# gonewest818/raytrace-clj

Measured on NVIDIA B200. Metric: samples_per_sec, higher is better.
Workload: dtype f32

## Files before the change

### raytrace_clj_b200/csrc/rt_api.cu

```cuda
#include "../../include/raytrace_b200.h"

#include <cuda_runtime.h>
#include <dlfcn.h>
#include <math_constants.h>
#include <nccl.h>

#include <algorithm>
#include <cmath>
#include <cstdio>
#include <cstdlib>
#include <cstring>
#include <atomic>
#include <mutex>
#include <thread>
#include <string>
#include <vector>

#include "rt_bvh_build.cuh"
#include "rt_kernels.cuh"

using namespace rt;

namespace {

constexpr int kR = 4;
constexpr int kBlock = 256;
constexpr int kMinBlocks = 1;
constexpr int kTileCap = 4096;

thread_local std::string g_create_error;

struct DeviceBuffers {
    int dev = 0;
    cudaStream_t stream = nullptr;
    cudaEvent_t ev0 = nullptr, ev1 = nullptr, ev_done = nullptr;
    void* scene_blob = nullptr;
    void* scene_stage = nullptr;
    size_t scene_bytes = 0;
    DevScene sc{};
    float* d_sum = nullptr;
    float* d_mean = nullptr;
    uint8_t* d_rgb8 = nullptr;
    size_t frame_px = 0;
    unsigned long long* d_counters = nullptr;
    struct WaveLane {
        float4* queue = nullptr;
        unsigned long long* best = nullptr;
        uint2* pairs = nullptr;
        uint2* cands = nullptr;
        double* cand_t = nullptr;
        unsigned* cand_count = nullptr;
        WaveState* state = nullptr;
        LaneStatus* h_status = nullptr;
        LaneStatus* d_status = nullptr;
        cudaEvent_t ev_done = nullptr;
        cudaStream_t stream = nullptr;
        cudaStream_t stage_stream = nullptr;
        cudaEvent_t ev_culled = nullptr, ev_shaded = nullptr;
        size_t entries = 0;
        bool best_clean = false;
    } lanes[kMaxLanes];
    cudaEvent_t ev_lane_start = nullptr;
    TraceRec* d_trace = nullptr;
    struct TraceMeta { const char* kernel; int lane, iter; };
    std::vector<TraceMeta> trace_meta;
    void* scratch = nullptr;
    size_t scratch_bytes = 0;
    int sm_count = 0, clock_khz = 0;
    char name[64] = {0};
    float last_ms = 0.f;
    bool timed = false;
    float4* bvh_nodes = nullptr;
    size_t bvh_cap = 0;
    int bvh_builder = 0, bvh_depth = 0;
    long long bvh_build_ns = 0;
    void* bvh_scratch = nullptr;
    size_t bvh_scratch_bytes = 0;
    int* h_bvh_depth = nullptr;
    cudaEvent_t ev_b0 = nullptr, ev_b1 = nullptr;
    void* h_stage = nullptr;
    size_t h_stage_bytes = 0;
    cudaEvent_t ev_r0 = nullptr, ev_r1 = nullptr;
    cudaEvent_t ev_chunk[4] = {};
};

struct NcclApi {
    void* handle = nullptr;
    ncclResult_t (*CommInitAll)(ncclComm_t*, int, const int*) = nullptr;
    ncclResult_t (*CommDestroy)(ncclComm_t) = nullptr;
    ncclResult_t (*Reduce)(const void*, void*, size_t, ncclDataType_t, ncclRedOp_t, int, ncclComm_t, cudaStream_t) = nullptr;
    ncclResult_t (*GroupStart)() = nullptr;
    ncclResult_t (*GroupEnd)() = nullptr;
    const char* (*GetErrorString)(ncclResult_t) = nullptr;
    std::vector<ncclComm_t> comms;
};

}

struct Options {
    int wave_lanes = 2;
    long long wave_capacity = 1ll << 24;
    int cull_claims = 2;
    int cull_ctas_per_sm = 4;
    int cull_shape = 0;
    int light_block = 128;
    long long tail_entries = 1 << 19;
    int tail_ctas_per_sm = 0;
    int tile_records = 1024;
    int direct_spheres = 1;
    int common_origin = 1;
    int reduce = 0;
    int rows = 0;
    int tail_block = 256;
    int tail_rays = 1;
    int tail_solo = 24;
    int tail_lpp = 32;
    int mega_regcap = 0;
    int wave_depth = 2;
    int cull_tc = 1;
    int tc_tiles_per_cta = 0;
    int tc_ctas = 0;
    int bvh_build = 1;
};

struct rt_ctx {
    std::mutex mu;
    std::string err;
    std::vector<DeviceBuffers> devs;
    Options opt;
    bool has_scene = false, has_cam = false;
    int n_spheres = 0;
    int n_total = 0;
    int n_list = 0, n_cull = 0;
    int cull_cap = 0, preloaded = 0;
    int tc_tiles = 0;
    std::vector<std::vector<float>> tc_scratch_rows;
    std::vector<int> tc_row_k;
    int generic = 0;
    int accel = RT_ACCEL_BRUTE_FORCE;
    bool bvh_dirty = true;
    double win_lo = 0.0, win_hi = 0.0;
    std::vector<float> h_c0r, h_c1, h_t0t1;
    std::vector<unsigned> h_flags;
    std::vector<double> h_bs_c0, h_bs_c1, h_bs_r;
    DevCamera cam{};
    std::atomic<uint64_t> n_launches{0};
    std::mutex err_mu;
    bool profile = false;
    double stage_ms[4] = {0, 0, 0, 0};
    double reduce_ms = 0.0;
    std::vector<bool> peer_ok;
    NcclApi nccl;
};

namespace {

int fail(rt_ctx* ctx, int code, const std::string& msg) {
    if (ctx) {
        std::lock_guard<std::mutex> lk(ctx->err_mu);
        ctx->err = msg;
    } else {
        g_create_error = msg;
    }
    return code;
}

#define RT_CUDA(ctx, expr)                                                                          \
    do {                                                                                            \
        cudaError_t e__ = (expr);                                                                   \
        if (e__ != cudaSuccess)                                                                     \
            return fail(ctx, RT_ERR_CUDA, std::string(#expr) + ": " + cudaGetErrorString(e__));     \
    } while (0)

int ensure_scratch(rt_ctx* ctx, DeviceBuffers& d, size_t bytes) {
    if (d.scratch_bytes >= bytes) return RT_OK;
    if (d.scratch) cudaFree(d.scratch);
    d.scratch = nullptr;
    d.scratch_bytes = 0;
    RT_CUDA(ctx, cudaMalloc(&d.scratch, bytes));
    d.scratch_bytes = bytes;
    return RT_OK;
}

int ensure_frame(rt_ctx* ctx, DeviceBuffers& d, size_t px) {
    if (d.frame_px >= px) return RT_OK;
    if (d.d_sum) cudaFree(d.d_sum);
    if (d.d_mean) cudaFree(d.d_mean);
    if (d.d_rgb8) cudaFree(d.d_rgb8);
    d.d_sum = d.d_mean = nullptr;
    d.d_rgb8 = nullptr;
    d.frame_px = 0;
    RT_CUDA(ctx, cudaMalloc(&d.d_sum, px * 3 * sizeof(float)));
    RT_CUDA(ctx, cudaMalloc(&d.d_mean, px * 3 * sizeof(float)));
    RT_CUDA(ctx, cudaMalloc(&d.d_rgb8, px * 3));
    d.frame_px = px;
    return RT_OK;
}


void free_lane(DeviceBuffers::WaveLane& L) {
    if (L.queue) cudaFree(L.queue);
    if (L.best) cudaFree(L.best);
    if (L.pairs) cudaFree(L.pairs);
    if (L.cands) cudaFree(L.cands);
    if (L.cand_t) cudaFree(L.cand_t);
    if (L.cand_count) cudaFree(L.cand_count);
    L.queue = nullptr; L.best = nullptr; L.pairs = nullptr; L.cands = nullptr; L.cand_t = nullptr; L.cand_count = nullptr;
    L.entries = 0;
}

void free_wave(DeviceBuffers& d) {
    for (auto& L : d.lanes) {
        free_lane(L);
        if (L.state) cudaFree(L.state);
        if (L.h_status) cudaFreeHost(L.h_status);
        if (L.ev_done) cudaEventDestroy(L.ev_done);
        if (L.stream) cudaStreamDestroy(L.stream);
        if (L.stage_stream) cudaStreamDestroy(L.stage_stream);
        if (L.ev_culled) cudaEventDestroy(L.ev_culled);
        if (L.ev_shaded) cudaEventDestroy(L.ev_shaded);
        L = DeviceBuffers::WaveLane();
    }
    if (d.ev_lane_start) cudaEventDestroy(d.ev_lane_start);
    d.ev_lane_start = nullptr;
    if (d.d_trace) cudaFree(d.d_trace);
    d.d_trace = nullptr;
}

int ensure_lane(rt_ctx* ctx, DeviceBuffers& d, int lane, size_t entries) {
    DeviceBuffers::WaveLane& L = d.lanes[lane];
    if (!L.state) {
        RT_CUDA(ctx, cudaMalloc(&L.state, sizeof(WaveState)));
        RT_CUDA(ctx, cudaHostAlloc(&L.h_status, sizeof(LaneStatus), cudaHostAllocMapped));
        RT_CUDA(ctx, cudaHostGetDevicePointer((void**)&L.d_status, L.h_status, 0));
        RT_CUDA(ctx, cudaEventCreateWithFlags(&L.ev_done, cudaEventDisableTiming));
        if (lane > 0) RT_CUDA(ctx, cudaStreamCreateWithFlags(&L.stream, cudaStreamNonBlocking));
        int prio_least = 0, prio_greatest = 0;
        RT_CUDA(ctx, cudaDeviceGetStreamPriorityRange(&prio_least, &prio_greatest));
        RT_CUDA(ctx, cudaStreamCreateWithPriority(&L.stage_stream, cudaStreamNonBlocking, prio_greatest));
        RT_CUDA(ctx, cudaEventCreateWithFlags(&L.ev_culled, cudaEventDisableTiming));
        RT_CUDA(ctx, cudaEventCreateWithFlags(&L.ev_shaded, cudaEventDisableTiming));
        if (!d.ev_lane_start) RT_CUDA(ctx, cudaEventCreateWithFlags(&d.ev_lane_start, cudaEventDisableTiming));
    }
    if (L.entries >= entries) return RT_OK;
    free_lane(L);
    RT_CUDA(ctx, cudaMalloc(&L.queue, entries * 2 * 3 * sizeof(float4)));
    RT_CUDA(ctx, cudaMalloc(&L.best, entries * 2 * sizeof(unsigned long long)));
    RT_CUDA(ctx, cudaMalloc(&L.pairs, entries * kPairsPerEntry * sizeof(uint2)));
    const size_t cand_slots = entries * kPairsPerEntry + (size_t)d.sm_count * 8 * 8 * 32;
    RT_CUDA(ctx, cudaMalloc(&L.cands, cand_slots * sizeof(uint2)));
    RT_CUDA(ctx, cudaMalloc(&L.cand_t, cand_slots * sizeof(double)));
    RT_CUDA(ctx, cudaMalloc(&L.cand_count, (size_t)d.sm_count * 8 * 8 * sizeof(unsigned)));
    L.entries = entries;
    L.best_clean = false;
    return RT_OK;
}

size_t align_up(size_t x, size_t a) { return (x + a - 1) / a * a; }

float round_up_f32(double x) {
    float f = (float)x;
    if ((double)f < x) f = nextafterf(f, INFINITY);
    return f;
}

size_t mega_smem_bytes(int cull_cap) { return (size_t)cull_cap * sizeof(float4) + Culler<kR, kBlock>::LIST_BYTES; }

template <typename Kern>
int configure_kernel(rt_ctx* ctx, Kern kern, size_t smem, int* blocks_per_sm) {
    RT_CUDA(ctx, cudaFuncSetAttribute(kern, cudaFuncAttributeMaxDynamicSharedMemorySize, (int)smem));
    int b = 0;
    RT_CUDA(ctx, cudaOccupancyMaxActiveBlocksPerMultiprocessor(&b, kern, kBlock, smem));
    if (b < 1) return fail(ctx, RT_ERR_CUDA, "kernel does not fit on an SM");
    *blocks_per_sm = b;
    return RT_OK;
}

long long env_ll(const char* name, long long dflt) {
    const char* v = getenv(name);
    return (v && *v) ? atoll(v) : dflt;
}
int env_int(const char* name, int dflt) { return (int)env_ll(name, dflt); }

Options options_from_env() {
    Options o;
    o.wave_lanes = env_int("RT_WAVE_LANES", o.wave_lanes);
    o.wave_capacity = env_ll("RT_WAVE_CAPACITY", o.wave_capacity);
    o.cull_claims = env_int("RT_CULL_CLAIMS", o.cull_claims);
    o.cull_ctas_per_sm = env_int("RT_CULL_CTAS_PER_SM", o.cull_ctas_per_sm);
    const char* shape = getenv("RT_CULL_SHAPE");
    if (shape && !strcmp(shape, "128x6")) o.cull_shape = 1;
    if (shape && !strcmp(shape, "256x2")) o.cull_shape = 2;
    o.light_block = env_int("RT_LIGHT_BLOCK", o.light_block);
    o.tail_entries = env_ll("RT_TAIL_ENTRIES", o.tail_entries);
    o.tail_ctas_per_sm = env_int("RT_TAIL_CTAS_PER_SM", o.tail_ctas_per_sm);
    o.tile_records = env_int("RT_TILE_RECORDS", o.tile_records);
    o.direct_spheres = env_int("RT_DIRECT_SPHERES", o.direct_spheres);
    o.common_origin = env_int("RT_COMMON_ORIGIN", o.common_origin);
    o.reduce = env_int("RT_REDUCE", o.reduce);
    o.rows = env_int("RT_ROWS", o.rows);
    o.wave_depth = env_int("RT_WAVE_DEPTH", o.wave_depth);
    o.tail_rays = env_int("RT_TAIL_RAYS", o.tail_rays);
    o.tail_solo = env_int("RT_TAIL_SOLO", o.tail_solo);
    o.tail_lpp = env_int("RT_TAIL_LPP", o.tail_lpp);
    o.tail_block = env_int("RT_TAIL_BLOCK", o.tail_block);
    o.cull_tc = env_int("RT_CULL_TC", o.cull_tc);
    o.tc_tiles_per_cta = env_int("RT_TC_TILES_PER_CTA", o.tc_tiles_per_cta);
    o.tc_ctas = env_int("RT_TC_CTAS", o.tc_ctas);
    o.bvh_build = env_int("RT_BVH_BUILD", o.bvh_build);
    return o;
}

template <int BLOCK, int MINB>
int cull_config(rt_ctx* ctx, size_t* smem, int* bps, void (**kern)(const WaveParams)) {
    *kern = wf_cull<kR, BLOCK, MINB>;
    *smem = (ctx->preloaded ? 2 : 1) * (size_t)ctx->cull_cap * sizeof(float4) + Culler<kR, BLOCK>::LIST_BYTES;
    RT_CUDA(ctx, cudaFuncSetAttribute(*kern, cudaFuncAttributeMaxDynamicSharedMemorySize, (int)*smem));
    RT_CUDA(ctx, cudaOccupancyMaxActiveBlocksPerMultiprocessor(bps, *kern, BLOCK, *smem));
    if (*bps < 1) return fail(ctx, RT_ERR_CUDA, "cull kernel does not fit on an SM");
    return RT_OK;
}

int launch_wave(rt_ctx* ctx, DeviceBuffers& d, const RenderParams& P, unsigned long long, cudaStream_t stream) {
    const Options& opt = ctx->opt;
    void (*cull)(const WaveParams) = nullptr;
    size_t smem = 0;
    int bps = 0, cull_block = 256, rc;
    if (opt.cull_shape == 2) rc = cull_config<256, 2>(ctx, &smem, &bps, &cull);
    else if (opt.cull_shape == 1) { rc = cull_config<128, 6>(ctx, &smem, &bps, &cull); cull_block = 128; }
    else { rc = cull_config<128, 5>(ctx, &smem, &bps, &cull); cull_block = 128; }
    if (rc) return rc;
    const int cull_ctas_env = opt.cull_ctas_per_sm;
    if (cull_ctas_env > 0) bps = std::min(bps, cull_ctas_env);
    const size_t cap_env = (size_t)std::max<long long>(64, opt.wave_capacity);
    const int lanes_env = std::max(1, std::min(kMaxLanes, opt.wave_lanes));
    const int n_lanes = (ctx->profile || P.total_work < 65536) ? 1 : lanes_env;
    const size_t capacity = align_up((size_t)std::min<unsigned long long>(cap_env / n_lanes, (P.total_work + n_lanes - 1) / n_lanes), 32);

    bool done[kMaxLanes] = {};
    const unsigned tail_entries = (unsigned)std::max<long long>(0, opt.tail_entries);
    const bool gen = ctx->generic != 0;
    const bool tail4 = opt.tail_rays == 4;
    const int tail_block = (gen || tail4) ? 256 : (opt.tail_block == 32 || opt.tail_block == 64 || opt.tail_block == 128 ? opt.tail_block : 256);
    const size_t tail_smem = (size_t)ctx->cull_cap * sizeof(float4) +
                             (tail4 ? Culler<4, 256>::LIST_BYTES : (size_t)Culler<1, 256>::LIST_WORDS * tail_block * sizeof(uint32_t));
    int tail_bps = 0;
    void (*k_tail)(const WaveParams) = gen ? wf_tail<256, true, 1> : (tail4 ? wf_tail<256, false, 4> : wf_tail<256, false, 1>);
    if (tail_block == 128) k_tail = wf_tail<128, false, 1>;
    if (tail_block == 64) k_tail = wf_tail<64, false, 1>;
    if (tail_block == 32) k_tail = wf_tail<32, false, 1>;
    void (*k_refine)(const WaveParams) = gen ? wf_refine<true> : wf_refine<false>;
    void (*k_shade)(const WaveParams) = gen ? wf_shade<true> : wf_shade<false>;
    RT_CUDA(ctx, cudaFuncSetAttribute(k_tail, cudaFuncAttributeMaxDynamicSharedMemorySize, (int)tail_smem));
    RT_CUDA(ctx, cudaOccupancyMaxActiveBlocksPerMultiprocessor(&tail_bps, k_tail, tail_block, tail_smem));
    const int tail_auto = (n_lanes > 1 ? 1 : std::max(1, std::min((int)(tail_bps * tail_block / 256), 2))) * (256 / tail_block);
    const int tail_grid = d.sm_count * (opt.tail_ctas_per_sm > 0 ? opt.tail_ctas_per_sm : tail_auto);
    const bool bvh = ctx->accel == RT_ACCEL_BVH;
    void (*k_bvh)(const WaveParams) = gen ? wf_bvh<true> : wf_bvh<false>;
    const bool tail_ok = tail_bps >= 1 && tail_entries > 0 && !ctx->profile && !bvh;
    const bool use_tc = opt.cull_tc != 0 && ctx->tc_tiles > 0 && !bvh && ((ctx->n_list >= tc::MIN_LEAVES && !ctx->generic) || opt.cull_tc == 3);
    const int tc_launch_tiles = std::min(ctx->tc_tiles, (int)tc::MAX_TILES);
    const int tc_slots = tc::slots_for(tc_launch_tiles, 227 * 1024);
    const size_t tc_smem = tc::smem_bytes(tc_launch_tiles, tc_slots);
    if (use_tc) RT_CUDA(ctx, cudaFuncSetAttribute(wf_cull_tc, cudaFuncAttributeMaxDynamicSharedMemorySize, (int)tc_smem));
    const int tc_per_cta = std::max(0, opt.tc_tiles_per_cta);
    const int tc_grid = opt.tc_ctas > 0 ? std::min(opt.tc_ctas, 4 * d.sm_count) : d.sm_count;
    auto launch_tc = [&](const WaveParams& Wl, int per_cta, unsigned ctas, cudaStream_t s_) {
        WaveParams Wt = Wl;
        Wt.claims_per_warp = per_cta;
        Wt.tc_slots = tc_slots;
        for (int t0 = 0, pass = 0; t0 < ctx->tc_tiles; t0 += tc::MAX_TILES, ++pass) {
            Wt.tc_tile0 = t0;
            Wt.tc_launch_tiles = std::min((int)tc::MAX_TILES, ctx->tc_tiles - t0);
            Wt.tc_pass = pass;
            wf_cull_tc<<<ctas, tc::THREADS, tc_smem, s_>>>(Wt);
            if (pass) ctx->n_launches += 1;
        }
    };

    const int light_block = std::max(64, std::min(256, opt.light_block / 32 * 32));
    const int light_grid = d.sm_count * 8 * 256 / light_block;
    const int cull_grid = d.sm_count * bps;
    const int claims_env = std::max(0, opt.cull_claims);
    const int claims = (ctx->profile || !ctx->preloaded || n_lanes < 2 || bvh) ? 0 : claims_env;
    const int cull_warps = cull_block / 32, resident_warps = cull_grid * cull_warps;
    unsigned n_bound[kMaxLanes];
    WaveParams W[kMaxLanes];
    cudaStream_t st[kMaxLanes];
    unsigned long long first = 0;
    for (int l = 0; l < n_lanes; ++l) {
        if ((rc = ensure_lane(ctx, d, l, capacity))) return rc;
        DeviceBuffers::WaveLane& L = d.lanes[l];
        W[l] = WaveParams{};
        W[l].base = P;
        W[l].queue[0] = L.queue;
        W[l].queue[1] = L.queue + 3 * capacity;
        W[l].best_t = L.best;
        W[l].best_key = L.best + L.entries;
        W[l].pairs = L.pairs;
        W[l].cands = L.cands;
        W[l].cand_t = L.cand_t;
        W[l].cand_count = L.cand_count;
        W[l].st = L.state;
        W[l].capacity = (int)capacity;
        W[l].pair_cap = (unsigned)std::min<size_t>(capacity * kPairsPerEntry, 0xfffffff0u);
        W[l].cur = 0;
        W[l].claims_per_warp = claims;
        W[l].resident_warps = claims ? resident_warps : 0;
        W[l].tail_solo = (unsigned)std::max(0, opt.tail_solo);
        W[l].tail_lpp = opt.tail_lpp == 8 ? 8u : (opt.tail_lpp == 16 ? 16u : 32u);
        st[l] = l == 0 ? stream : L.stream;
    }
    static const char* trace_path = getenv("RT_TRACE");
    constexpr int kTraceMax = 8192;
    const bool tracing = trace_path && *trace_path;
    if (tracing) {
        if (!d.d_trace) RT_CUDA(ctx, cudaMalloc(&d.d_trace, kTraceMax * sizeof(TraceRec)));
        static const std::vector<TraceRec> init((size_t)kTraceMax, TraceRec{~0ull, 0ull});
        RT_CUDA(ctx, cudaMemcpyAsync(d.d_trace, init.data(), init.size() * sizeof(TraceRec), cudaMemcpyHostToDevice, stream));
        d.trace_meta.clear();
    }
    auto trace_slot = [&](const char* kernel, int lane, int iter) -> TraceRec* {
        if (!tracing || (int)d.trace_meta.size() >= kTraceMax) return nullptr;
        d.trace_meta.push_back({kernel, lane, iter});
        return d.d_trace + (d.trace_meta.size() - 1);
    };
    int iter_no[kMaxLanes] = {};
    static const bool debug_sync = getenv("RT_DEBUG_SYNC") && *getenv("RT_DEBUG_SYNC") == '1';
    auto dbg = [&](const char* what, int lane, int it) -> int {
        if (!debug_sync) return RT_OK;
        cudaError_t e = cudaDeviceSynchronize();
        if (e != cudaSuccess) return fail(ctx, RT_ERR_CUDA, std::string(what) + " (lane " + std::to_string(lane) + ", iteration " + std::to_string(it) + "): " + cudaGetErrorString(e));
        return RT_OK;
    };
    unsigned count0[kMaxLanes];
    unsigned long long total0 = 0;
    for (int l = 0; l < n_lanes; ++l) {
        count0[l] = (unsigned)std::min<unsigned long long>(capacity, P.total_work - total0);
        total0 += count0[l];
        n_bound[l] = count0[l];
    }
    InitParams I{};
    I.n_lanes = n_lanes;
    I.work_counter = P.work_counter;
    I.counters = P.counters;
    I.total0 = total0;
    I.total_work = P.total_work;
    for (int l = 0; l < n_lanes; ++l) {
        DeviceBuffers::WaveLane& L = d.lanes[l];
        I.st[l] = L.state;
        I.first[l] = first;
        I.count[l] = count0[l];
        first += count0[l];
        if (!L.best_clean) {
            wf_fill_best<<<d.sm_count * 4, 256, 0, stream>>>(L.best, L.best + L.entries, L.entries);
            ctx->n_launches += 1;
        }
        L.best_clean = false;
    }
    wf_init<<<1, 1, 0, stream>>>(I);
    ctx->n_launches += 1;
    RT_CUDA(ctx, cudaGetLastError());
    RT_CUDA(ctx, cudaEventRecord(d.ev_lane_start, stream));
    for (int l = 1; l < n_lanes; ++l) RT_CUDA(ctx, cudaStreamWaitEvent(st[l], d.ev_lane_start, 0));

    const int depth = std::max(1, std::min(16, opt.wave_depth));
    int enq[kMaxLanes] = {}, seen[kMaxLanes] = {};
    bool tailed[kMaxLanes] = {};
    for (int l = 0; l < n_lanes; ++l) {
        DeviceBuffers::WaveLane& L = d.lanes[l];
        memset(L.h_status, 0, sizeof(LaneStatus));
        W[l].status = L.d_status;
        if (count0[l] == 0) done[l] = true;
    }
    std::vector<cudaEvent_t> evs;
    unsigned idle_spins = 0;
    for (;;) {
        bool progressed = false, all_done = true;
        for (int l = 0; l < n_lanes; ++l) {
            if (done[l]) continue;
            all_done = false;
            DeviceBuffers::WaveLane& L = d.lanes[l];
            while (!tailed[l] && enq[l] - seen[l] < depth) {
                cudaEvent_t e[5] = {nullptr, nullptr, nullptr, nullptr, nullptr};
                if (ctx->profile)
                    for (auto& x : e) { RT_CUDA(ctx, cudaEventCreate(&x)); evs.push_back(x); }
                if (ctx->profile) cudaEventRecord(e[0], st[l]);
                W[l].iter = (unsigned)(enq[l] + 1);
                const bool tc_now = use_tc && !(enq[l] == 0 && P.common_origin && opt.cull_tc == 2);
                if (bvh) {
                    W[l].trace = trace_slot("bvh", l, iter_no[l]);
                    k_bvh<<<light_grid, 128, 0, st[l]>>>(W[l]);
                    if (ctx->profile) { cudaEventRecord(e[1], st[l]); cudaEventRecord(e[2], st[l]); cudaEventRecord(e[3], st[l]); }
                    W[l].trace = trace_slot("shade", l, iter_no[l]);
                    k_shade<<<light_grid, light_block, 0, st[l]>>>(W[l]);
                    if (ctx->profile) cudaEventRecord(e[4], st[l]);
                    ctx->n_launches -= 2;
                } else if (claims) {
                    W[l].trace = trace_slot("cull", l, iter_no[l]);
                    if (debug_sync) {
                        WaveState hs{};
                        cudaMemcpy(&hs, W[l].st, sizeof hs, cudaMemcpyDeviceToHost);
                        fprintf(stderr, "lane %d iteration %d cur %d: in flight %u fresh %u | other queue %u %u | mode %u exhausted %u npairs %u\n", l, enq[l], W[l].cur,
                                hs.cnt[W[l].cur][0], hs.cnt[W[l].cur][1], hs.cnt[W[l].cur ^ 1][0], hs.cnt[W[l].cur ^ 1][1], hs.mode, hs.exhausted, hs.npairs);
                    }
                    if (tc_now) {
                        const unsigned tiles = (n_bound[l] + tc::TILE_M - 1) / tc::TILE_M;
                        const unsigned ctas = tc_per_cta ? (tiles + (unsigned)tc_per_cta - 1u) / (unsigned)tc_per_cta : (unsigned)tc_grid;
                        launch_tc(W[l], tc_per_cta, std::max(1u, ctas), st[l]);
                    } else {
                    const unsigned items = n_bound[l] / (32u * kR) + 2u * (unsigned)resident_warps + 8u;
                    const unsigned ctas = (items + (unsigned)(cull_warps * claims) - 1u) / (unsigned)(cull_warps * claims);
                    cull<<<ctas, cull_block, smem, st[l]>>>(W[l]);
                    }
                    if ((rc = dbg(tc_now ? "wf_cull_tc" : "wf_cull", l, enq[l]))) return rc;
                    RT_CUDA(ctx, cudaEventRecord(L.ev_culled, st[l]));
                    RT_CUDA(ctx, cudaStreamWaitEvent(L.stage_stream, L.ev_culled, 0));
                    W[l].trace = trace_slot("refine", l, iter_no[l]);
                    k_refine<<<light_grid, light_block, 0, L.stage_stream>>>(W[l]);
                    if ((rc = dbg("wf_refine", l, enq[l]))) return rc;
                    W[l].trace = trace_slot("tiebreak", l, iter_no[l]);
                    wf_tiebreak<<<light_grid, light_block, 0, L.stage_stream>>>(W[l]);
                    if ((rc = dbg("wf_tiebreak", l, enq[l]))) return rc;
                    W[l].trace = trace_slot("shade", l, iter_no[l]);
                    k_shade<<<light_grid, light_block, 0, L.stage_stream>>>(W[l]);
                    if ((rc = dbg("wf_shade", l, enq[l]))) return rc;
                    RT_CUDA(ctx, cudaEventRecord(L.ev_shaded, L.stage_stream));
                    RT_CUDA(ctx, cudaStreamWaitEvent(st[l], L.ev_shaded, 0));
                } else {
                    W[l].trace = trace_slot("cull", l, iter_no[l]);
                    if (tc_now) {
                        launch_tc(W[l], 0, (unsigned)tc_grid, st[l]);
                    } else {
                        cull<<<cull_grid, cull_block, smem, st[l]>>>(W[l]);
                    }
                    if (ctx->profile) cudaEventRecord(e[1], st[l]);
                    W[l].trace = trace_slot("refine", l, iter_no[l]);
                    k_refine<<<light_grid, light_block, 0, st[l]>>>(W[l]);
                    if (ctx->profile) cudaEventRecord(e[2], st[l]);
                    W[l].trace = trace_slot("tiebreak", l, iter_no[l]);
                    wf_tiebreak<<<light_grid, light_block, 0, st[l]>>>(W[l]);
                    if (ctx->profile) cudaEventRecord(e[3], st[l]);
                    W[l].trace = trace_slot("shade", l, iter_no[l]);
                    k_shade<<<light_grid, light_block, 0, st[l]>>>(W[l]);
                    if (ctx->profile) cudaEventRecord(e[4], st[l]);
                }
                RT_CUDA(ctx, cudaGetLastError());
                W[l].cur ^= 1;
                ++iter_no[l];
                ctx->n_launches += 4;
                ++enq[l];
                progressed = true;
            }
        }
        if (all_done) break;
        for (int l = 0; l < n_lanes; ++l) {
            if (done[l]) continue;
            DeviceBuffers::WaveLane& L = d.lanes[l];
            const volatile LaneStatus* hs = L.h_status;
            const unsigned seq = hs->seq;
            if ((int)seq == seen[l] && hs->mode != MODE_DONE) continue;
            std::atomic_thread_fence(std::memory_order_acquire);
            const unsigned n_next = hs->n_next, n_fresh = hs->n_fresh, exhausted = hs->exhausted, mode = hs->mode;
            if (hs->seq != seq) continue;
            seen[l] = (int)seq;
            progressed = true;
            if (exhausted) n_bound[l] = std::min(n_bound[l], n_next);
            if (mode == MODE_DONE) { done[l] = true; continue; }
            if (tail_ok && !tailed[l] && exhausted && n_fresh == 0 && n_next <= tail_entries) {
                W[l].iter = (unsigned)(enq[l] + 1);
                W[l].trace = trace_slot("tail", l, iter_no[l]);
                k_tail<<<tail_grid, tail_block, tail_smem, st[l]>>>(W[l]);
                if ((rc = dbg("wf_tail", l, enq[l]))) return rc;
                RT_CUDA(ctx, cudaGetLastError());
                ctx->n_launches += 1;
                tailed[l] = true;
            }
        }
        if (!progressed) {
            if (++idle_spins > 200) {
                if (cudaSuccess != cudaPeekAtLastError()) RT_CUDA(ctx, cudaGetLastError());
                if (idle_spins > 20000 && (idle_spins % 1000) == 0) {
                    for (int l = 0; l < n_lanes; ++l)
                        if (!done[l] && cudaStreamQuery(st[l]) == cudaSuccess && d.lanes[l].h_status->seq == (unsigned)seen[l] &&
                            enq[l] > seen[l])
                            return fail(ctx, RT_ERR_CUDA, "wavefront lane finished its queue without reporting status");
                }
                std::this_thread::yield();
            }
        } else {
            idle_spins = 0;
        }
    }
    for (int l = 1; l < n_lanes; ++l) {
        RT_CUDA(ctx, cudaEventRecord(d.lanes[l].ev_done, st[l]));
        RT_CUDA(ctx, cudaStreamWaitEvent(stream, d.lanes[l].ev_done, 0));
    }
    for (int l = 0; l < n_lanes; ++l) d.lanes[l].best_clean = true;
    if (ctx->profile) {
        RT_CUDA(ctx, cudaStreamSynchronize(stream));
        for (size_t i = 0; i + 4 < evs.size(); i += 5)
            for (int sgi = 0; sgi < 4; ++sgi) {
                float ms = 0.f;
                if (cudaEventElapsedTime(&ms, evs[i + sgi], evs[i + sgi + 1]) == cudaSuccess) ctx->stage_ms[sgi] += ms;
            }
        for (auto x : evs) cudaEventDestroy(x);
    }
    return RT_OK;
}

int launch_params(rt_ctx* ctx, DeviceBuffers& d, RenderParams& P, int variant, cudaStream_t stream);

int launch_render(rt_ctx* ctx, DeviceBuffers& d, int nx, int ny, int sample_begin, int sample_count, int row_offset,
                  int row_stride, int max_depth, uint64_t seed, int variant, float* d_sum, cudaStream_t stream) {
    RenderParams P{};
    P.sc = d.sc;
    P.cam = ctx->cam;
    P.nx = nx;
    P.ny = ny;
    P.sample_begin = sample_begin;
    P.sample_count = sample_count;
    P.row_offset = row_offset;
    P.row_stride = row_stride;
    P.rows_in_shard = (ny - row_offset + row_stride - 1) / row_stride;
    P.max_depth = max_depth;
    P.key = make_uint2((uint32_t)seed, (uint32_t)(seed >> 32));
    P.sum = d_sum;
    P.counters = d.d_counters;
    P.work_counter = d.d_counters + DC_COUNT;
    P.total_work = (unsigned long long)sample_count * (unsigned long long)nx * (unsigned long long)P.rows_in_shard;
    if ((sample_begin + sample_count) >= (1 << 24)) return fail(ctx, RT_ERR_ARG, "sample index must stay below 2^24");
    return launch_params(ctx, d, P, variant, stream);
}

int launch_params(rt_ctx* ctx, DeviceBuffers& d, RenderParams& P, int variant, cudaStream_t stream) {
    if (variant != RT_VARIANT_MEGAKERNEL && variant != RT_VARIANT_WAVEFRONT)
        return fail(ctx, RT_ERR_ARG, "unknown render variant");
    if (variant == RT_VARIANT_WAVEFRONT && P.max_depth > 255)
        return fail(ctx, RT_ERR_ARG, "the wavefront variant packs the depth in 8 bits: max_depth <= 255");
    P.sc = d.sc;
    P.cam = ctx->cam;
    P.counters = d.d_counters;
    P.work_counter = d.d_counters + DC_COUNT;
    P.cull_cap = ctx->cull_cap;
    P.preloaded = ctx->preloaded;
    P.common_origin = (ctx->opt.common_origin && (ctx->cam.type == CAM_PINHOLE || ctx->cam.lens_radius == 0.f)) ? 1 : 0;
    RT_CUDA(ctx, cudaMemsetAsync(P.work_counter, 0, sizeof(unsigned long long), stream));
    if (P.total_work == 0) return RT_OK;
    size_t smem = mega_smem_bytes(ctx->cull_cap);
    unsigned long long want = (P.total_work + (unsigned long long)kBlock * kR - 1) / ((unsigned long long)kBlock * kR);
    int bps = 0;
    if (variant == RT_VARIANT_MEGAKERNEL) {
        void (*kern)(const RenderParams) = ctx->generic ? mega_kernel<kR, kBlock, kMinBlocks, true>
                                           : (ctx->opt.mega_regcap ? mega_kernel<kR, kBlock, 2, false> : mega_kernel<kR, kBlock, kMinBlocks, false>);
        int rc = configure_kernel(ctx, kern, smem, &bps);
        if (rc) return rc;
        int grid = (int)std::min<unsigned long long>((unsigned long long)d.sm_count * bps, want);
        if (grid < 1) grid = 1;
        kern<<<grid, kBlock, smem, stream>>>(P);
        RT_CUDA(ctx, cudaGetLastError());
        ctx->n_launches += 1;
        return RT_OK;
    }
    return launch_wave(ctx, d, P, want, stream);
}

void build_cull_records(rt_ctx* ctx, double win_lo, double win_hi, float* cull_all, float* tc_out) {
    const double eps = std::ldexp(1.0, -20), u = std::ldexp(1.0, -24);
    for (int i = 0; i < ctx->n_spheres; ++i) {
        float* cull_a = i < ctx->n_list ? cull_all : cull_all + 4 * (size_t)(ctx->n_cull - ctx->n_list);
        double r = std::fabs(ctx->h_bs_r[(size_t)i]);
        double mid[3], half2 = 0.0, cmax = 0.0;
        const bool moving = (ctx->h_flags[i] & RT_SPHERE_MOVING) != 0;
        for (int c = 0; c < 3; ++c) {
            double p0 = ctx->h_bs_c0[3 * (size_t)i + c];
            if (moving) {
                double p1 = ctx->h_bs_c1[3 * (size_t)i + c], t0 = ctx->h_t0t1[2 * i], t1 = ctx->h_t0t1[2 * i + 1];
                double fa = (win_lo - t0) / (t1 - t0), fb = (win_hi - t0) / (t1 - t0);
                double pa = p0 * (1.0 - fa) + p1 * fa, pb = p0 * (1.0 - fb) + p1 * fb;
                mid[c] = 0.5 * (pa + pb);
                half2 += 0.25 * (pb - pa) * (pb - pa);
            } else {
                mid[c] = p0;
            }
            cmax = std::max(cmax, std::fabs(mid[c]));
        }
        double rb = r + std::sqrt(half2);
        double e = (moving || ctx->generic) ? std::ldexp(1.0, -21) * (cmax + rb) : 0.0;
        double cc = 0.0;
        for (int c = 0; c < 3; ++c) {
            const float neg = (float)(-mid[c]);
            cull_a[4 * i + c] = neg;
            cc += (double)neg * (double)neg;
        }
        double re = rb + e;
        double r2i = re * re * (1.0 + eps) + 48.0 * u * cc + 8.0 * u * re * re;
        cull_a[4 * i + 3] = round_up_f32(r2i - cc);
        if (tc_out && i < ctx->n_list) {
            const double c[3] = {-(double)cull_a[4 * i], -(double)cull_a[4 * i + 1], -(double)cull_a[4 * i + 2]};
            const double Wtc = re * re * (1.0 + eps) + 96.0 * u * cc + 24.0 * u * re * re - cc;
            float row[tc::KTOT];
            tc::sphere_slots(c, Wtc, row);
            ctx->tc_scratch_rows[(size_t)i].assign(row, row + tc::KTOT);
        }
    }
    for (int k = ctx->n_list; k < ctx->n_cull; ++k) {
        cull_all[4 * k] = cull_all[4 * k + 1] = cull_all[4 * k + 2] = 0.f;
        cull_all[4 * k + 3] = -INFINITY;
    }
    if (tc_out) {
        float pad[tc::KTOT];
        tc::padding_slots(pad);
        for (int p = 0; p < ctx->tc_tiles * tc::TILE_N; ++p) {
            const int k = ctx->tc_row_k[(size_t)p];
            const float* row = k >= 0 ? ctx->tc_scratch_rows[(size_t)k].data() : pad;
            float* tile = tc_out + (size_t)(p / tc::TILE_N) * (tc::B_TILE_BYTES / 4);
            for (int q = 0; q < tc::KTOT; ++q) tile[tc::canon_off(tc::TILE_N, p % tc::TILE_N, q) / 4] = row[q];
        }
    }
}

int ensure_window(rt_ctx* ctx, double lo, double hi) {
    if (lo >= ctx->win_lo && hi <= ctx->win_hi) return RT_OK;
    if (!(lo <= hi) || !std::isfinite(lo) || !std::isfinite(hi)) return fail(ctx, RT_ERR_ARG, "ray time is not finite");
    ctx->win_lo = std::min(ctx->win_lo, lo);
    ctx->win_hi = std::max(ctx->win_hi, hi);
    bool any_moving = false;
    for (unsigned f : ctx->h_flags) any_moving |= (f & RT_SPHERE_MOVING) != 0;
    if (!any_moving) return RT_OK;
    ctx->bvh_dirty = true;
    std::vector<float> cull((size_t)(ctx->n_cull + ctx->n_spheres - ctx->n_list) * 4);
    std::vector<float> tcr((size_t)ctx->tc_tiles * (tc::B_TILE_BYTES / 4));
    build_cull_records(ctx, ctx->win_lo, ctx->win_hi, cull.data(), tcr.empty() ? nullptr : tcr.data());
    if (cull.empty()) return RT_OK;
    for (auto& d : ctx->devs) {
        RT_CUDA(ctx, cudaSetDevice(d.dev));
        RT_CUDA(ctx, cudaDeviceSynchronize());
        RT_CUDA(ctx, cudaMemcpy((void*)d.sc.cull_a, cull.data(), cull.size() * sizeof(float), cudaMemcpyHostToDevice));
        if (!tcr.empty()) RT_CUDA(ctx, cudaMemcpy((void*)d.sc.cull_tc, tcr.data(), tcr.size() * sizeof(float), cudaMemcpyHostToDevice));
    }
    cudaSetDevice(ctx->devs[0].dev);
    return RT_OK;
}

struct BuildLeaf {
    float lo[3], hi[3];
    float c[3];
    int k;
};
int bvh_build_node(std::vector<BuildLeaf>& L, int begin, int end, std::vector<float>& nodes, float lo[3], float hi[3], int depth,
                   int* max_depth) {
    if (end - begin == 1) {
        for (int a = 0; a < 3; ++a) { lo[a] = L[(size_t)begin].lo[a]; hi[a] = L[(size_t)begin].hi[a]; }
        *max_depth = std::max(*max_depth, depth);
        return ~L[(size_t)begin].k;
    }
    float cmin[3] = {INFINITY, INFINITY, INFINITY}, cmax[3] = {-INFINITY, -INFINITY, -INFINITY};
    for (int i = begin; i < end; ++i)
        for (int a = 0; a < 3; ++a) { cmin[a] = std::min(cmin[a], L[(size_t)i].c[a]); cmax[a] = std::max(cmax[a], L[(size_t)i].c[a]); }
    int axis = 0;
    for (int a = 1; a < 3; ++a) if (cmax[a] - cmin[a] > cmax[axis] - cmin[axis]) axis = a;
    const int mid = begin + (end - begin + 1) / 2;
    std::nth_element(L.begin() + begin, L.begin() + mid, L.begin() + end,
                     [axis](const BuildLeaf& x, const BuildLeaf& y) { return x.c[axis] < y.c[axis]; });
    const size_t me = nodes.size() / 16;
    nodes.resize(nodes.size() + 16, 0.f);
    float llo[3], lhi[3], rlo[3], rhi[3];
    const int left = bvh_build_node(L, begin, mid, nodes, llo, lhi, depth + 1, max_depth);
    const int right = bvh_build_node(L, mid, end, nodes, rlo, rhi, depth + 1, max_depth);
    float* N = nodes.data() + 16 * me;
    N[0] = llo[0]; N[1] = llo[1]; N[2] = llo[2]; N[3] = lhi[0]; N[4] = lhi[1]; N[5] = lhi[2];
    N[6] = rlo[0]; N[7] = rlo[1]; N[8] = rlo[2]; N[9] = rhi[0]; N[10] = rhi[1]; N[11] = rhi[2];
    memcpy(&N[12], &left, 4);
    memcpy(&N[13], &right, 4);
    for (int a = 0; a < 3; ++a) { lo[a] = std::min(llo[a], rlo[a]); hi[a] = std::max(lhi[a], rhi[a]); }
    return (int)me;
}

int ensure_bvh_nodes(rt_ctx* ctx, DeviceBuffers& d, size_t bytes) {
    if (d.bvh_cap >= bytes) return RT_OK;
    if (d.bvh_nodes) cudaFree(d.bvh_nodes);
    d.bvh_nodes = nullptr;
    d.bvh_cap = 0;
    RT_CUDA(ctx, cudaMalloc(&d.bvh_nodes, bytes));
    d.bvh_cap = bytes;
    return RT_OK;
}

int bvh_build_host(rt_ctx* ctx) {
    const int n = ctx->n_list;
    std::vector<BuildLeaf> L((size_t)n);
    for (int k = 0; k < n; ++k) {
        BuildLeaf& b = L[(size_t)k];
        b.k = k;
        const bool moving = (ctx->h_flags[(size_t)k] & RT_SPHERE_MOVING) != 0;
        const double r = std::fabs(ctx->h_bs_r[(size_t)k]);
        for (int a = 0; a < 3; ++a) {
            double pa = ctx->h_bs_c0[3 * (size_t)k + a], pb = pa;
            if (moving) {
                const double p0 = ctx->h_bs_c0[3 * (size_t)k + a], p1 = ctx->h_bs_c1[3 * (size_t)k + a];
                const double t0 = ctx->h_t0t1[2 * k], t1 = ctx->h_t0t1[2 * k + 1];
                const double fa = (ctx->win_lo - t0) / (t1 - t0), fb = (ctx->win_hi - t0) / (t1 - t0);
                pa = p0 * (1.0 - fa) + p1 * fa;
                pb = p0 * (1.0 - fb) + p1 * fb;
            }
            const double lo = std::min(pa, pb) - r, hi = std::max(pa, pb) + r;
            const double m = 1e-6 * (std::fabs(lo) + std::fabs(hi) + r) + 1e-30;
            b.lo[a] = nextafterf((float)(lo - m), -INFINITY);
            b.hi[a] = nextafterf((float)(hi + m), INFINITY);
            b.c[a] = (float)(0.5 * (lo + hi));
        }
    }
    std::vector<float> nodes;
    nodes.reserve(16 * (size_t)std::max(1, n));
    float lo[3], hi[3];
    int depth = 1;
    if (n == 1) {
        nodes.assign(16, 0.f);
        for (int a = 0; a < 3; ++a) { nodes[(size_t)a] = nodes[6 + (size_t)a] = L[0].lo[a]; nodes[3 + (size_t)a] = nodes[9 + (size_t)a] = L[0].hi[a]; }
        const int leaf = ~0;
        memcpy(&nodes[12], &leaf, 4);
        memcpy(&nodes[13], &leaf, 4);
    } else {
        const int root = bvh_build_node(L, 0, n, nodes, lo, hi, 0, &depth);
        if (root != 0) return fail(ctx, RT_ERR_STATE, "BVH build: the root is not node 0");
    }
    for (auto& d : ctx->devs) {
        RT_CUDA(ctx, cudaSetDevice(d.dev));
        RT_CUDA(ctx, cudaDeviceSynchronize());
        const size_t bytes = nodes.size() * sizeof(float);
        if (int rc = ensure_bvh_nodes(ctx, d, bytes)) return rc;
        RT_CUDA(ctx, cudaMemcpy(d.bvh_nodes, nodes.data(), bytes, cudaMemcpyHostToDevice));
        d.sc.bvh = d.bvh_nodes;
        d.sc.bvh_nodes = (int)(nodes.size() / 16);
        d.bvh_builder = 0;
        d.bvh_depth = depth;
        d.bvh_build_ns = 0;
    }
    cudaSetDevice(ctx->devs[0].dev);
    return RT_OK;
}

int bvh_enqueue_device(rt_ctx* ctx, DeviceBuffers& d) {
    const int n = ctx->n_list;
    const int n_nodes = std::max(1, n - 1);
    RT_CUDA(ctx, cudaSetDevice(d.dev));
    RT_CUDA(ctx, cudaDeviceSynchronize());
    if (int rc = ensure_bvh_nodes(ctx, d, (size_t)n_nodes * 4 * sizeof(float4))) return rc;
    size_t sort_bytes = 0;
    RT_CUDA(ctx, cub::DeviceRadixSort::SortPairs(nullptr, sort_bytes, (const unsigned long long*)nullptr, (unsigned long long*)nullptr,
                                                 (const int*)nullptr, (int*)nullptr, n, 0, 3 * (int)kMortonAxisBits, d.stream));
    size_t off = 0;
    auto take = [&](size_t bytes) { const size_t o = off; off = align_up(off + bytes, 256); return o; };
    const size_t n_ = (size_t)n;
    const size_t o_c0 = take(n_ * 3 * 8), o_c1 = take(n_ * 3 * 8), o_r = take(n_ * 8), o_t = take(n_ * 2 * 4), o_fl = take(n_ * 4);
    const size_t o_box = take(n_ * 6 * 4), o_cb = take(6 * 4), o_code = take(n_ * 8), o_code2 = take(n_ * 8);
    const size_t o_leaf = take(n_ * 4), o_leaf2 = take(n_ * 4), o_par = take((2 * n_ - 1) * 4), o_arr = take((size_t)n_nodes * 4);
    const size_t o_h = take((size_t)n_nodes * 4), o_depth = take(4), o_sort = take(sort_bytes);
    if (d.bvh_scratch_bytes < off) {
        if (d.bvh_scratch) cudaFree(d.bvh_scratch);
        d.bvh_scratch = nullptr;
        d.bvh_scratch_bytes = 0;
        RT_CUDA(ctx, cudaMalloc(&d.bvh_scratch, off));
        d.bvh_scratch_bytes = off;
    }
    if (!d.h_bvh_depth) {
        RT_CUDA(ctx, cudaHostAlloc(&d.h_bvh_depth, sizeof(int), cudaHostAllocDefault));
        RT_CUDA(ctx, cudaEventCreate(&d.ev_b0));
        RT_CUDA(ctx, cudaEventCreate(&d.ev_b1));
    }
    char* S = (char*)d.bvh_scratch;
    const cudaStream_t st = d.stream;
    BvhLeafInput in{(const double*)(S + o_c0), (const double*)(S + o_c1), (const double*)(S + o_r), (const float*)(S + o_t),
                    (const unsigned*)(S + o_fl)};
    float* boxes = (float*)(S + o_box);
    unsigned* cb = (unsigned*)(S + o_cb);
    int* depth = (int*)(S + o_depth);
    RT_CUDA(ctx, cudaEventRecord(d.ev_b0, st));
    RT_CUDA(ctx, cudaMemcpyAsync(S + o_c0, ctx->h_bs_c0.data(), n_ * 3 * 8, cudaMemcpyHostToDevice, st));
    RT_CUDA(ctx, cudaMemcpyAsync(S + o_c1, ctx->h_bs_c1.data(), n_ * 3 * 8, cudaMemcpyHostToDevice, st));
    RT_CUDA(ctx, cudaMemcpyAsync(S + o_r, ctx->h_bs_r.data(), n_ * 8, cudaMemcpyHostToDevice, st));
    RT_CUDA(ctx, cudaMemcpyAsync(S + o_t, ctx->h_t0t1.data(), n_ * 2 * 4, cudaMemcpyHostToDevice, st));
    RT_CUDA(ctx, cudaMemcpyAsync(S + o_fl, ctx->h_flags.data(), n_ * 4, cudaMemcpyHostToDevice, st));
    RT_CUDA(ctx, cudaMemsetAsync(cb, 0xff, 3 * 4, st));
    RT_CUDA(ctx, cudaMemsetAsync(cb + 3, 0, 3 * 4, st));
    const int grid = (n + 255) / 256;
    bvh_leaf_boxes<<<grid, 256, 0, st>>>(in, n, ctx->win_lo, ctx->win_hi, boxes, cb);
    if (n == 1) {
        bvh_single_leaf<<<1, 32, 0, st>>>(boxes, d.bvh_nodes, depth);
    } else {
        unsigned long long* code = (unsigned long long*)(S + o_code);
        unsigned long long* code2 = (unsigned long long*)(S + o_code2);
        int* leaf = (int*)(S + o_leaf);
        int* leaf2 = (int*)(S + o_leaf2);
        int* parent = (int*)(S + o_par);
        bvh_morton<<<grid, 256, 0, st>>>(boxes, n, cb, code, leaf);
        RT_CUDA(ctx, cub::DeviceRadixSort::SortPairs(S + o_sort, sort_bytes, code, code2, leaf, leaf2, n, 0, 3 * (int)kMortonAxisBits, st));
        RT_CUDA(ctx, cudaMemsetAsync(S + o_arr, 0, (size_t)n_nodes * 4, st));
        bvh_hierarchy<<<(n - 1 + 255) / 256, 256, 0, st>>>(code2, leaf2, n, d.bvh_nodes, parent);
        bvh_fit<<<grid, 256, 0, st>>>(boxes, parent, n, d.bvh_nodes, (unsigned*)(S + o_arr), (int*)(S + o_h), depth);
    }
    RT_CUDA(ctx, cudaGetLastError());
    RT_CUDA(ctx, cudaMemcpyAsync(d.h_bvh_depth, depth, sizeof(int), cudaMemcpyDeviceToHost, st));
    RT_CUDA(ctx, cudaEventRecord(d.ev_b1, st));
    d.sc.bvh_nodes = n_nodes;
// ... 751 lines not shown
        int bad = RT_OK;
        for (int g = 0; g < G; ++g)
            if (rcs[(size_t)g] && !bad) bad = rcs[(size_t)g];
        if (bad) {
            for (auto& dv : ctx->devs) { cudaSetDevice(dv.dev); cudaDeviceSynchronize(); }
            cudaSetDevice(ctx->devs[0].dev);
            return bad;
        }
    }
    DeviceBuffers& root = ctx->devs[0];
    RT_CUDA(ctx, cudaSetDevice(root.dev));
    ResolveParams P{};
    P.sum = root.d_sum; P.n_peers = 0; P.nx = nx; P.ny = ny; P.nr = nsamples;
    P.rgb8 = out_rgb8 ? root.d_rgb8 : nullptr;
    P.mean = out_linear_rgb ? root.d_mean : nullptr;
    P.sum_out = nullptr;
    const int total = nx * ny * 3;
    if (use_nccl) {
        NcclApi& N = ctx->nccl;
        for (int g = 1; g < G; ++g) RT_CUDA(ctx, cudaStreamWaitEvent(root.stream, ctx->devs[g].ev_done, 0));
        RT_CUDA(ctx, cudaEventRecord(root.ev_r0, root.stream));
        ncclResult_t nr = N.GroupStart();
        for (int g = 0; g < G && nr == ncclSuccess; ++g)
            nr = N.Reduce(ctx->devs[g].d_sum, ctx->devs[g].d_sum, (size_t)total, ncclFloat, ncclSum, 0, N.comms[(size_t)g], ctx->devs[g].stream);
        const ncclResult_t ge = N.GroupEnd();
        if (nr == ncclSuccess) nr = ge;
        if (nr != ncclSuccess) {
            for (auto& dv : ctx->devs) { cudaSetDevice(dv.dev); cudaDeviceSynchronize(); }
            cudaSetDevice(root.dev);
            return fail(ctx, RT_ERR_NCCL, std::string("ncclReduce: ") + N.GetErrorString(nr));
        }
        RT_CUDA(ctx, cudaSetDevice(root.dev));
        RT_CUDA(ctx, cudaEventRecord(root.ev_r1, root.stream));
        resolve_kernel<<<(total + 255) / 256, 256, 0, root.stream>>>(P);
    } else {
        for (int g = 1; g < G; ++g) {
            DeviceBuffers& d = ctx->devs[g];
            RT_CUDA(ctx, cudaStreamWaitEvent(root.stream, d.ev_done, 0));
            if (ctx->peer_ok[g]) {
                P.peers[P.n_peers++] = d.d_sum;
            } else {
                if ((rc = ensure_scratch(ctx, root, (size_t)(G - 1) * px * 3 * sizeof(float)))) return rc;
                float* stage = (float*)root.scratch + (size_t)(g - 1) * px * 3;
                RT_CUDA(ctx, cudaMemcpyPeerAsync(stage, root.dev, d.d_sum, d.dev, px * 3 * sizeof(float), root.stream));
                P.peers[P.n_peers++] = stage;
            }
        }
        RT_CUDA(ctx, cudaEventRecord(root.ev_r0, root.stream));
        resolve_kernel<<<(total + 255) / 256, 256, 0, root.stream>>>(P);
        RT_CUDA(ctx, cudaEventRecord(root.ev_r1, root.stream));
    }
    RT_CUDA(ctx, cudaGetLastError());
    ctx->n_launches += 1;
    auto host_pinned = [](const void* p) {
        cudaPointerAttributes at{};
        if (cudaPointerGetAttributes(&at, p) != cudaSuccess) { cudaGetLastError(); return false; }
        return at.type == cudaMemoryTypeHost;
    };
    const size_t b_lin = out_linear_rgb ? align_up(px * 3 * sizeof(float), 256) : 0, b_rgb = out_rgb8 ? px * 3 : 0;
    if (b_lin + b_rgb) {
        if ((rc = ensure_stage(ctx, root, b_lin + b_rgb))) return rc;
        constexpr int NCH = 4;
        for (auto& e : root.ev_chunk)
            if (!e) RT_CUDA(ctx, cudaEventCreateWithFlags(&e, cudaEventDisableTiming));
        struct Part { char* dst; const char* src; char* stage; size_t bytes; };
        const Part parts[2] = {{(char*)out_linear_rgb, (const char*)root.d_mean, (char*)root.h_stage, out_linear_rgb ? px * 3 * sizeof(float) : 0},
                               {(char*)out_rgb8, (const char*)root.d_rgb8, (char*)root.h_stage + b_lin, b_rgb}};
        for (const Part& pt : parts) {
            if (!pt.bytes) continue;
            if (host_pinned(pt.dst)) {
                RT_CUDA(ctx, cudaMemcpyAsync(pt.dst, pt.src, pt.bytes, cudaMemcpyDeviceToHost, root.stream));
                continue;
            }
            const size_t step = align_up((pt.bytes + NCH - 1) / NCH, 4096);
            for (int c = 0; c < NCH; ++c) {
                const size_t off = std::min(pt.bytes, (size_t)c * step), len = std::min(pt.bytes - off, step);
                if (len) RT_CUDA(ctx, cudaMemcpyAsync(pt.stage + off, pt.src + off, len, cudaMemcpyDeviceToHost, root.stream));
                RT_CUDA(ctx, cudaEventRecord(root.ev_chunk[c], root.stream));
            }
            for (int c = 0; c < NCH; ++c) {
                const size_t off = std::min(pt.bytes, (size_t)c * step), len = std::min(pt.bytes - off, step);
                RT_CUDA(ctx, cudaEventSynchronize(root.ev_chunk[c]));
                if (len) memcpy(pt.dst + off, pt.stage + off, len);
            }
        }
    }
    RT_CUDA(ctx, cudaStreamSynchronize(root.stream));
    for (int g = 1; g < G; ++g) {
        RT_CUDA(ctx, cudaSetDevice(ctx->devs[g].dev));
        RT_CUDA(ctx, cudaStreamSynchronize(ctx->devs[g].stream));
    }
    cudaSetDevice(root.dev);
    if (G > 1) {
        float ms = 0.f;
        if (cudaEventElapsedTime(&ms, root.ev_r0, root.ev_r1) == cudaSuccess) ctx->reduce_ms += ms;
        cudaGetLastError();
    }
    return RT_OK;
}

int rt_host_alloc(rt_ctx* ctx, size_t bytes, void** out) {
    if (!out || bytes == 0) return ctx ? fail(ctx, RT_ERR_ARG, "rt_host_alloc: bad arguments") : RT_ERR_ARG;
    *out = nullptr;
    if (ctx && !ctx->devs.empty()) cudaSetDevice(ctx->devs[0].dev);
    const cudaError_t e = cudaHostAlloc(out, bytes, cudaHostAllocPortable);
    if (e != cudaSuccess) {
        cudaGetLastError();
        return fail(ctx, RT_ERR_CUDA, std::string("cudaHostAlloc: ") + cudaGetErrorString(e));
    }
    return RT_OK;
}

int rt_host_free(rt_ctx* ctx, void* p) {
    if (!p) return RT_OK;
    const cudaError_t e = cudaFreeHost(p);
    if (e != cudaSuccess) {
        cudaGetLastError();
        return fail(ctx, RT_ERR_CUDA, std::string("cudaFreeHost: ") + cudaGetErrorString(e));
    }
    return RT_OK;
}

int rt_trace_paths(rt_ctx* ctx, int nx, int ny, int n, const int32_t* pixel, const int32_t* sample, int max_depth, uint64_t seed,
                   int variant, float* out_radiance, int32_t* out_nrays, int32_t* out_term, int log_bounces, rt_path_bounce* out_log) {
    int rc = check_ready(ctx);
    if (rc) return rc;
    std::lock_guard<std::mutex> lk(ctx->mu);
    if ((rc = check_camera_times(ctx))) return rc;
    if (nx <= 0 || ny <= 0 || n < 0 || max_depth < 0 || log_bounces < 0 || (n > 0 && (!pixel || !sample || !out_radiance || !out_nrays || !out_term)) ||
        (log_bounces > 0 && n > 0 && !out_log))
        return fail(ctx, RT_ERR_ARG, "bad trace_paths arguments");
    if ((long long)nx * ny > 0x7fffffffLL / 3) return fail(ctx, RT_ERR_ARG, "image too large");
    if (n == 0) return RT_OK;
    for (int q = 0; q < n; ++q)
        if (pixel[q] < 0 || pixel[q] >= nx * ny || sample[q] < 0 || sample[q] >= (1 << 24))
            return fail(ctx, RT_ERR_ARG, "pixel / sample index out of range");
    static_assert(sizeof(rt_path_bounce) == sizeof(PathBounce) && sizeof(PathBounce) == 40, "rt_path_bounce layout");
    DeviceBuffers& d = ctx->devs[0];
    RT_CUDA(ctx, cudaSetDevice(d.dev));
    const size_t b_i = align_up((size_t)n * 4, 256), b_f = align_up((size_t)n * 12, 256), b_l = align_up((size_t)n * log_bounces * sizeof(PathBounce), 256);
    char* buf = nullptr;
    RT_CUDA(ctx, cudaMalloc(&buf, 4 * b_i + b_f + b_l + 256));
    int* d_pix = (int*)buf;
    int* d_smp = (int*)(buf + b_i);
    int* d_nr = (int*)(buf + 2 * b_i);
    int* d_term = (int*)(buf + 3 * b_i);
    float* d_rad = (float*)(buf + 4 * b_i);
    PathBounce* d_log = log_bounces > 0 ? (PathBounce*)(buf + 4 * b_i + b_f) : nullptr;
    auto cleanup = [&](int code) { cudaStreamSynchronize(d.stream); cudaFree(buf); return code; };
    cudaError_t e;
    if ((e = cudaMemcpyAsync(d_pix, pixel, (size_t)n * 4, cudaMemcpyHostToDevice, d.stream)) != cudaSuccess ||
        (e = cudaMemcpyAsync(d_smp, sample, (size_t)n * 4, cudaMemcpyHostToDevice, d.stream)) != cudaSuccess ||
        (e = cudaMemsetAsync(d_nr, 0, 2 * b_i + b_f, d.stream)) != cudaSuccess ||
        (d_log && (e = cudaMemsetAsync(d_log, 0xff, (size_t)n * log_bounces * sizeof(PathBounce), d.stream)) != cudaSuccess))
        return cleanup(fail(ctx, RT_ERR_CUDA, std::string("trace_paths upload: ") + cudaGetErrorString(e)));
    RenderParams P{};
    P.nx = nx; P.ny = ny;
    P.sample_begin = 0; P.sample_count = 1;
    P.row_offset = 0; P.row_stride = 1; P.rows_in_shard = ny;
    P.max_depth = max_depth;
    P.key = make_uint2((uint32_t)seed, (uint32_t)(seed >> 32));
    P.sum = d_rad;
    P.total_work = (unsigned long long)n;
    P.path_pixel = d_pix; P.path_sample = d_smp; P.path_nrays = d_nr; P.path_term = d_term;
    P.path_log = d_log; P.path_log_n = log_bounces;
    if ((rc = launch_params(ctx, d, P, variant, d.stream))) return cleanup(rc);
    if ((e = cudaMemcpyAsync(out_radiance, d_rad, (size_t)n * 12, cudaMemcpyDeviceToHost, d.stream)) != cudaSuccess ||
        (e = cudaMemcpyAsync(out_nrays, d_nr, (size_t)n * 4, cudaMemcpyDeviceToHost, d.stream)) != cudaSuccess ||
        (e = cudaMemcpyAsync(out_term, d_term, (size_t)n * 4, cudaMemcpyDeviceToHost, d.stream)) != cudaSuccess ||
        (d_log && (e = cudaMemcpyAsync(out_log, d_log, (size_t)n * log_bounces * sizeof(PathBounce), cudaMemcpyDeviceToHost, d.stream)) != cudaSuccess) ||
        (e = cudaStreamSynchronize(d.stream)) != cudaSuccess)
        return cleanup(fail(ctx, RT_ERR_CUDA, std::string("trace_paths: ") + cudaGetErrorString(e)));
    if (out_log)
        for (size_t q = 0; q < (size_t)n * log_bounces; ++q)
            if (out_log[q].hit_id == -1 && std::isnan(out_log[q].t)) { memset(&out_log[q], 0, sizeof(rt_path_bounce)); out_log[q].hit_id = -2; }
    d.timed = false;
    return cleanup(RT_OK);
}

int rt_sample_device(rt_ctx* ctx, int kind, int n, uint64_t seed, float* out) {
    if (!ctx) return RT_ERR_ARG;
    std::lock_guard<std::mutex> lk(ctx->mu);
    if ((kind != 0 && kind != 1) || n < 0 || (n > 0 && !out)) return fail(ctx, RT_ERR_ARG, "bad sample_device arguments");
    if (n == 0) return RT_OK;
    DeviceBuffers& d = ctx->devs[0];
    RT_CUDA(ctx, cudaSetDevice(d.dev));
    const int dim = kind == 0 ? 3 : 2;
    int rc;
    if ((rc = ensure_scratch(ctx, d, (size_t)n * dim * 4))) return rc;
    sampler_kernel<<<(n + 255) / 256, 256, 0, d.stream>>>(kind, n, make_uint2((uint32_t)seed, (uint32_t)(seed >> 32)), (float*)d.scratch);
    RT_CUDA(ctx, cudaGetLastError());
    RT_CUDA(ctx, cudaMemcpyAsync(out, d.scratch, (size_t)n * dim * 4, cudaMemcpyDeviceToHost, d.stream));
    RT_CUDA(ctx, cudaStreamSynchronize(d.stream));
    return RT_OK;
}

int rt_trace_primary(rt_ctx* ctx, int n, const float* origins, const float* dirs, const float* times, double tmin,
                     double tmax, double* out_t, int32_t* out_id) {
    int rc = check_ready(ctx);
    if (rc) return rc;
    std::lock_guard<std::mutex> lk(ctx->mu);
    if (n < 0 || (n > 0 && (!origins || !dirs || !out_t || !out_id))) return fail(ctx, RT_ERR_ARG, "bad trace arguments");
    if (!(tmin >= 0.0)) return fail(ctx, RT_ERR_ARG, "tmin must be >= 0: the cull discards spheres behind the origin");
    if (n == 0) return RT_OK;
    {
        double lo = 0.0, hi = 0.0;
        if (times) {
            lo = INFINITY; hi = -INFINITY;
            for (int i = 0; i < n; ++i) { lo = std::min(lo, (double)times[i]); hi = std::max(hi, (double)times[i]); }
        }
        if ((rc = ensure_window(ctx, lo, hi))) return rc;
    }
    DeviceBuffers& d = ctx->devs[0];
    RT_CUDA(ctx, cudaSetDevice(d.dev));
    size_t b_o = align_up((size_t)n * 12, 256), b_t = align_up((size_t)n * 4, 256), b_ot = align_up((size_t)n * 8, 256);
    if ((rc = ensure_scratch(ctx, d, 2 * b_o + 2 * b_t + b_ot))) return rc;
    char* base = (char*)d.scratch;
    float* d_o = (float*)base;
    float* d_d = (float*)(base + b_o);
    float* d_tm = (float*)(base + 2 * b_o);
    int* d_id = (int*)(base + 2 * b_o + b_t);
    double* d_t = (double*)(base + 2 * b_o + 2 * b_t);
    RT_CUDA(ctx, cudaMemcpyAsync(d_o, origins, (size_t)n * 12, cudaMemcpyHostToDevice, d.stream));
    RT_CUDA(ctx, cudaMemcpyAsync(d_d, dirs, (size_t)n * 12, cudaMemcpyHostToDevice, d.stream));
    if (times) RT_CUDA(ctx, cudaMemcpyAsync(d_tm, times, (size_t)n * 4, cudaMemcpyHostToDevice, d.stream));
    if (ctx->accel == RT_ACCEL_BVH) {
        if ((rc = ensure_bvh(ctx))) return rc;
        TraceParamsB B{};
        B.sc = d.sc; B.n = n; B.origins = d_o; B.dirs = d_d; B.times = times ? d_tm : nullptr;
        B.tmin = tmin; B.tmax = tmax; B.out_t = d_t; B.out_id = d_id;
        B.stats = nullptr;
        if (ctx->generic) trace_bvh_kernel<true><<<(n + 127) / 128, 128, 0, d.stream>>>(B);
        else trace_bvh_kernel<false><<<(n + 127) / 128, 128, 0, d.stream>>>(B);
        RT_CUDA(ctx, cudaGetLastError());
        RT_CUDA(ctx, cudaMemcpyAsync(out_t, d_t, (size_t)n * 8, cudaMemcpyDeviceToHost, d.stream));
        RT_CUDA(ctx, cudaMemcpyAsync(out_id, d_id, (size_t)n * 4, cudaMemcpyDeviceToHost, d.stream));
        RT_CUDA(ctx, cudaStreamSynchronize(d.stream));
        return RT_OK;
    }
    TraceParams P{};
    P.sc = d.sc; P.n = n; P.origins = d_o; P.dirs = d_d; P.times = times ? d_tm : nullptr;
    P.tmin = tmin; P.tmax = tmax; P.out_t = d_t; P.out_id = d_id; P.cull_cap = ctx->cull_cap; P.preloaded = ctx->preloaded;
    void (*kern)(const TraceParams) = ctx->generic ? trace_kernel<kR, kBlock, true> : trace_kernel<kR, kBlock, false>;
    size_t smem = mega_smem_bytes(ctx->cull_cap);
    int bps = 0;
    if ((rc = configure_kernel(ctx, kern, smem, &bps))) return rc;
    int want = (int)(((long long)n + kBlock * kR - 1) / (kBlock * kR));
    int grid = std::max(1, std::min(d.sm_count * bps, want));
    kern<<<grid, kBlock, smem, d.stream>>>(P);
    RT_CUDA(ctx, cudaGetLastError());
    RT_CUDA(ctx, cudaMemcpyAsync(out_t, d_t, (size_t)n * 8, cudaMemcpyDeviceToHost, d.stream));
    RT_CUDA(ctx, cudaMemcpyAsync(out_id, d_id, (size_t)n * 4, cudaMemcpyDeviceToHost, d.stream));
    RT_CUDA(ctx, cudaStreamSynchronize(d.stream));
    return RT_OK;
}

int rt_cull_check(rt_ctx* ctx, int n, const float* origins, const float* dirs, const float* times, double tmin, double tmax,
                  uint64_t out[3]) {
    int rc = check_ready(ctx);
    if (rc) return rc;
    std::lock_guard<std::mutex> lk(ctx->mu);
    if (n < 0 || !out || (n > 0 && (!origins || !dirs))) return fail(ctx, RT_ERR_ARG, "bad cull_check arguments");
    if (!(tmin >= 0.0)) return fail(ctx, RT_ERR_ARG, "tmin must be >= 0: the cull discards spheres behind the origin");
    out[0] = out[1] = out[2] = 0;
    if (n == 0) return RT_OK;
    {
        double lo = 0.0, hi = 0.0;
        if (times) {
            lo = INFINITY; hi = -INFINITY;
            for (int i = 0; i < n; ++i) { lo = std::min(lo, (double)times[i]); hi = std::max(hi, (double)times[i]); }
        }
        if ((rc = ensure_window(ctx, lo, hi))) return rc;
    }
    DeviceBuffers& d = ctx->devs[0];
    RT_CUDA(ctx, cudaSetDevice(d.dev));
    size_t b_o = align_up((size_t)n * 12, 256), b_t = align_up((size_t)n * 4, 256);
    if ((rc = ensure_scratch(ctx, d, 2 * b_o + b_t + 256))) return rc;
    char* base = (char*)d.scratch;
    float* d_o = (float*)base;
    float* d_d = (float*)(base + b_o);
    float* d_tm = (float*)(base + 2 * b_o);
    unsigned long long* d_out = (unsigned long long*)(base + 2 * b_o + b_t);
    RT_CUDA(ctx, cudaMemcpyAsync(d_o, origins, (size_t)n * 12, cudaMemcpyHostToDevice, d.stream));
    RT_CUDA(ctx, cudaMemcpyAsync(d_d, dirs, (size_t)n * 12, cudaMemcpyHostToDevice, d.stream));
    if (times) RT_CUDA(ctx, cudaMemcpyAsync(d_tm, times, (size_t)n * 4, cudaMemcpyHostToDevice, d.stream));
    RT_CUDA(ctx, cudaMemsetAsync(d_out, 0, 3 * sizeof(unsigned long long), d.stream));
    if (ctx->opt.cull_tc && ctx->tc_tiles > 0) {
        const size_t cap = align_up(std::max<size_t>((size_t)n, 1u << 18), 128);
        if ((rc = ensure_lane(ctx, d, 0, cap))) return rc;
        DeviceBuffers::WaveLane& L = d.lanes[0];
        L.best_clean = false;
        const int words = (ctx->n_cull + 31) / 32;
        unsigned* d_mask = nullptr;
        RT_CUDA(ctx, cudaMalloc(&d_mask, (size_t)n * words * sizeof(unsigned)));
        RT_CUDA(ctx, cudaMemsetAsync(d_mask, 0, (size_t)n * words * sizeof(unsigned), d.stream));
        WaveParams W{};
        W.base.sc = d.sc;
        W.base.cam = ctx->cam;
        W.base.counters = d.d_counters;
        W.base.work_counter = d.d_counters + DC_COUNT;
        W.base.max_depth = 1;
        W.queue[0] = L.queue;
        W.queue[1] = L.queue + 3 * L.entries;
        W.best_t = L.best;
        W.best_key = L.best + L.entries;
        W.pairs = L.pairs;
        W.cands = L.cands;
        W.cand_t = L.cand_t;
        W.cand_count = L.cand_count;
        W.st = L.state;
        W.capacity = (int)L.entries;
        W.pair_cap = (unsigned)std::min<size_t>(L.entries * kPairsPerEntry, 0xfffffff0u);
        wf_fill_best<<<d.sm_count * 4, 256, 0, d.stream>>>(L.best, L.best + L.entries, L.entries);
#ifdef RT_TC_CHECK
        RT_CUDA(ctx, cudaMemsetAsync(L.pairs, 0xDD, (size_t)W.pair_cap * sizeof(uint2), d.stream));
#endif
        tc_check_fill<<<(n + 127) / 128, 128, 0, d.stream>>>(W, n, d_o, d_d, times ? d_tm : nullptr);
        const int launch_tiles = std::min(ctx->tc_tiles, (int)tc::MAX_TILES);
        W.tc_slots = tc::slots_for(launch_tiles, 227 * 1024);
        const size_t tc_smem = tc::smem_bytes(launch_tiles, W.tc_slots);
        RT_CUDA(ctx, cudaFuncSetAttribute(wf_cull_tc, cudaFuncAttributeMaxDynamicSharedMemorySize, (int)tc_smem));
        for (int t0 = 0, pass = 0; t0 < ctx->tc_tiles; t0 += tc::MAX_TILES, ++pass) {
            W.tc_tile0 = t0;
            W.tc_launch_tiles = std::min((int)tc::MAX_TILES, ctx->tc_tiles - t0);
            W.tc_pass = pass;
            wf_cull_tc<<<d.sm_count, tc::THREADS, tc_smem, d.stream>>>(W);
        }
        tc_check_mark<<<d.sm_count * 4, 256, 0, d.stream>>>(W, d_mask, words);
        tc_check_compare<<<(n + 127) / 128, 128, 0, d.stream>>>(W, n, tmin, tmax, d_mask, words, d_out);
        cudaError_t e = cudaStreamSynchronize(d.stream);
        cudaFree(d_mask);
        if (e != cudaSuccess) return fail(ctx, RT_ERR_CUDA, std::string("tensor-core cull check: ") + cudaGetErrorString(e));
    } else {
        cull_check_kernel<<<(n + 127) / 128, 128, 0, d.stream>>>(d.sc, n, d_o, d_d, times ? d_tm : nullptr, tmin, tmax, d_out);
    }
    RT_CUDA(ctx, cudaGetLastError());
    unsigned long long h[3];
    RT_CUDA(ctx, cudaMemcpyAsync(h, d_out, sizeof(h), cudaMemcpyDeviceToHost, d.stream));
    RT_CUDA(ctx, cudaStreamSynchronize(d.stream));
    for (int i = 0; i < 3; ++i) out[i] = h[i];
    return RT_OK;
}

int rt_generate_rays(rt_ctx* ctx, int n, int nx, int ny, const int32_t* ij, const int32_t* s, uint64_t seed,
                     float* out_origin, float* out_dir, float* out_time, float* out_rand) {
    if (!ctx) return RT_ERR_ARG;
    std::lock_guard<std::mutex> lk(ctx->mu);
    if (!ctx->has_cam) return fail(ctx, RT_ERR_STATE, "rt_set_camera has not been called");
    if (n < 0 || nx <= 0 || ny <= 0 || (n > 0 && (!ij || !s || !out_origin || !out_dir || !out_time)))
        return fail(ctx, RT_ERR_ARG, "bad generate_rays arguments");
    if (n == 0) return RT_OK;
    DeviceBuffers& d = ctx->devs[0];
    RT_CUDA(ctx, cudaSetDevice(d.dev));
    size_t b_ij = align_up((size_t)n * 8, 256), b_s = align_up((size_t)n * 4, 256), b_v = align_up((size_t)n * 12, 256),
           b_r = align_up((size_t)n * 20, 256);
    int rc;
    if ((rc = ensure_scratch(ctx, d, b_ij + 2 * b_s + 2 * b_v + b_r))) return rc;
    char* base = (char*)d.scratch;
    int* d_ij = (int*)base;
    int* d_s = (int*)(base + b_ij);
    float* d_o = (float*)(base + b_ij + b_s);
    float* d_d = (float*)(base + b_ij + b_s + b_v);
    float* d_t = (float*)(base + b_ij + b_s + 2 * b_v);
    float* d_r = (float*)(base + b_ij + 2 * b_s + 2 * b_v);
    RT_CUDA(ctx, cudaMemcpyAsync(d_ij, ij, (size_t)n * 8, cudaMemcpyHostToDevice, d.stream));
    RT_CUDA(ctx, cudaMemcpyAsync(d_s, s, (size_t)n * 4, cudaMemcpyHostToDevice, d.stream));
    genrays_kernel<<<(n + 255) / 256, 256, 0, d.stream>>>(ctx->cam, n, nx, ny, d_ij, d_s,
                                                         make_uint2((uint32_t)seed, (uint32_t)(seed >> 32)), d_o, d_d, d_t,
                                                         out_rand ? d_r : nullptr);
    RT_CUDA(ctx, cudaGetLastError());
    RT_CUDA(ctx, cudaMemcpyAsync(out_origin, d_o, (size_t)n * 12, cudaMemcpyDeviceToHost, d.stream));
    RT_CUDA(ctx, cudaMemcpyAsync(out_dir, d_d, (size_t)n * 12, cudaMemcpyDeviceToHost, d.stream));
    RT_CUDA(ctx, cudaMemcpyAsync(out_time, d_t, (size_t)n * 4, cudaMemcpyDeviceToHost, d.stream));
    if (out_rand) RT_CUDA(ctx, cudaMemcpyAsync(out_rand, d_r, (size_t)n * 20, cudaMemcpyDeviceToHost, d.stream));
    RT_CUDA(ctx, cudaStreamSynchronize(d.stream));
    return RT_OK;
}

int rt_shade_batch(rt_ctx* ctx, int n, const float* origins, const float* dirs, const float* times, const int32_t* hit_id,
                   const double* hit_t, const float* ball, const float* u01v, float* out_origin, float* out_dir,
                   float* out_atten, float* out_emitted, int32_t* out_flags) {
    int rc = check_ready(ctx);
    if (rc) return rc;
    std::lock_guard<std::mutex> lk(ctx->mu);
    if (n < 0 || (n > 0 && (!origins || !dirs || !hit_id || !hit_t || !ball || !u01v || !out_origin || !out_dir ||
                            !out_atten || !out_emitted || !out_flags)))
        return fail(ctx, RT_ERR_ARG, "bad shade_batch arguments");
    if (n == 0) return RT_OK;
    DeviceBuffers& d = ctx->devs[0];
    RT_CUDA(ctx, cudaSetDevice(d.dev));
    size_t b3 = align_up((size_t)n * 12, 256), b1 = align_up((size_t)n * 4, 256), b8 = align_up((size_t)n * 8, 256);
    if ((rc = ensure_scratch(ctx, d, 7 * b3 + 4 * b1 + b8))) return rc;
    char* p = (char*)d.scratch;
    float* d_o = (float*)p; p += b3;
    float* d_d = (float*)p; p += b3;
    float* d_ball = (float*)p; p += b3;
    float* d_oo = (float*)p; p += b3;
    float* d_od = (float*)p; p += b3;
    float* d_oa = (float*)p; p += b3;
    float* d_oe = (float*)p; p += b3;
    float* d_tm = (float*)p; p += b1;
    float* d_u = (float*)p; p += b1;
    int* d_id = (int*)p; p += b1;
    int* d_fl = (int*)p; p += b1;
    double* d_ht = (double*)p;
    RT_CUDA(ctx, cudaMemcpyAsync(d_o, origins, (size_t)n * 12, cudaMemcpyHostToDevice, d.stream));
    RT_CUDA(ctx, cudaMemcpyAsync(d_d, dirs, (size_t)n * 12, cudaMemcpyHostToDevice, d.stream));
    RT_CUDA(ctx, cudaMemcpyAsync(d_ball, ball, (size_t)n * 12, cudaMemcpyHostToDevice, d.stream));
    if (times) RT_CUDA(ctx, cudaMemcpyAsync(d_tm, times, (size_t)n * 4, cudaMemcpyHostToDevice, d.stream));
    RT_CUDA(ctx, cudaMemcpyAsync(d_u, u01v, (size_t)n * 4, cudaMemcpyHostToDevice, d.stream));
    RT_CUDA(ctx, cudaMemcpyAsync(d_id, hit_id, (size_t)n * 4, cudaMemcpyHostToDevice, d.stream));
    RT_CUDA(ctx, cudaMemcpyAsync(d_ht, hit_t, (size_t)n * 8, cudaMemcpyHostToDevice, d.stream));
    shade_kernel<<<(n + 255) / 256, 256, 0, d.stream>>>(d.sc, n, d_o, d_d, times ? d_tm : nullptr, d_id, d_ht, d_ball, d_u,
                                                       d_oo, d_od, d_oa, d_oe, d_fl);
    RT_CUDA(ctx, cudaGetLastError());
    RT_CUDA(ctx, cudaMemcpyAsync(out_origin, d_oo, (size_t)n * 12, cudaMemcpyDeviceToHost, d.stream));
    RT_CUDA(ctx, cudaMemcpyAsync(out_dir, d_od, (size_t)n * 12, cudaMemcpyDeviceToHost, d.stream));
    RT_CUDA(ctx, cudaMemcpyAsync(out_atten, d_oa, (size_t)n * 12, cudaMemcpyDeviceToHost, d.stream));
    RT_CUDA(ctx, cudaMemcpyAsync(out_emitted, d_oe, (size_t)n * 12, cudaMemcpyDeviceToHost, d.stream));
    RT_CUDA(ctx, cudaMemcpyAsync(out_flags, d_fl, (size_t)n * 4, cudaMemcpyDeviceToHost, d.stream));
    RT_CUDA(ctx, cudaStreamSynchronize(d.stream));
    return RT_OK;
}

int rt_measure_fp32_peak(rt_ctx* ctx, double* out_ffma_tflops, double* out_ffma2_tflops) {
    if (!ctx) return RT_ERR_ARG;
    std::lock_guard<std::mutex> lk(ctx->mu);
    DeviceBuffers& d = ctx->devs[0];
    RT_CUDA(ctx, cudaSetDevice(d.dev));
    const int blocks = d.sm_count * 8, threads = 256, iters = 1 << 15;
    int rc;
    if ((rc = ensure_scratch(ctx, d, (size_t)blocks * threads * 4))) return rc;
    float* out = (float*)d.scratch;
    double best[2] = {0, 0};
    for (int variant = 0; variant < 2; ++variant) {
        for (int rep = 0; rep < 4; ++rep) {
            RT_CUDA(ctx, cudaEventRecord(d.ev0, d.stream));
            if (variant == 0) ffma_peak_kernel<false><<<blocks, threads, 0, d.stream>>>(out, iters, 1.0000001f, 1e-7f);
            else ffma_peak_kernel<true><<<blocks, threads, 0, d.stream>>>(out, iters, 1.0000001f, 1e-7f);
            RT_CUDA(ctx, cudaGetLastError());
            RT_CUDA(ctx, cudaEventRecord(d.ev1, d.stream));
            RT_CUDA(ctx, cudaEventSynchronize(d.ev1));
            float ms = 0;
            RT_CUDA(ctx, cudaEventElapsedTime(&ms, d.ev0, d.ev1));
            double flops = 2.0 * 16.0 * (double)iters * (double)blocks * threads;
            if (rep > 0) best[variant] = std::max(best[variant], flops / (ms * 1e-3) / 1e12);
        }
    }
    if (out_ffma_tflops) *out_ffma_tflops = best[0];
    if (out_ffma2_tflops) *out_ffma2_tflops = best[1];
    d.timed = false;
    return RT_OK;
}

int rt_get_counters(rt_ctx* ctx, uint64_t out[RT_CTR_COUNT]) {
    if (!ctx || !out) return RT_ERR_ARG;
    std::lock_guard<std::mutex> lk(ctx->mu);
    unsigned long long dc[DC_COUNT];
    uint64_t total[DC_COUNT] = {0};
    float max_ms = 0.f;
    for (auto& d : ctx->devs) {
        RT_CUDA(ctx, cudaSetDevice(d.dev));
        RT_CUDA(ctx, cudaDeviceSynchronize());
        RT_CUDA(ctx, cudaMemcpy(dc, d.d_counters, sizeof(dc), cudaMemcpyDeviceToHost));
        for (int i = 0; i < DC_COUNT; ++i) total[i] += dc[i];
        if (!d.trace_meta.empty() && d.d_trace && getenv("RT_TRACE")) {
            std::vector<TraceRec> rec(d.trace_meta.size());
            RT_CUDA(ctx, cudaMemcpy(rec.data(), d.d_trace, rec.size() * sizeof(TraceRec), cudaMemcpyDeviceToHost));
            unsigned long long t0 = ~0ull;
            for (auto& r : rec) if (r.t_end) t0 = std::min(t0, r.t_start);
            if (FILE* f = fopen(getenv("RT_TRACE"), "a")) {
                fprintf(f, "# device %d, %zu launches: kernel lane iteration start_us end_us duration_us (%%globaltimer, relative to the first kernel)\n", d.dev, rec.size());
                for (size_t i = 0; i < rec.size(); ++i) {
                    if (!rec[i].t_end) continue;
                    fprintf(f, "%-9s %d %3d %10.1f %10.1f %9.1f\n", d.trace_meta[i].kernel, d.trace_meta[i].lane, d.trace_meta[i].iter,
                            (rec[i].t_start - t0) * 1e-3, (rec[i].t_end - t0) * 1e-3, (rec[i].t_end - rec[i].t_start) * 1e-3);
                }
                fclose(f);
            }
            d.trace_meta.clear();
        }
        if (d.timed) {
            float ms = 0.f;
            if (cudaEventElapsedTime(&ms, d.ev0, d.ev1) == cudaSuccess) d.last_ms = ms;
            cudaGetLastError();
        }
        max_ms = std::max(max_ms, d.last_ms);
    }
    cudaSetDevice(ctx->devs[0].dev);
    memset(out, 0, sizeof(uint64_t) * RT_CTR_COUNT);
    out[RT_CTR_RAYS] = total[DC_RAYS];
    out[RT_CTR_SPHERE_TESTS] = total[DC_RAYS] * (uint64_t)ctx->n_spheres;
    out[RT_CTR_SAMPLES] = total[DC_SAMPLES];
    out[RT_CTR_TERM_LIGHT] = total[DC_TERM_LIGHT];
    out[RT_CTR_TERM_ABSORB] = total[DC_TERM_ABSORB];
    out[RT_CTR_TERM_DEPTH] = total[DC_TERM_DEPTH];
    out[RT_CTR_TERM_MISS] = total[DC_TERM_MISS];
    out[RT_CTR_KERNEL_NS] = (uint64_t)((double)max_ms * 1e6);
    out[RT_CTR_CANDIDATES] = total[DC_CANDIDATES];
    out[RT_CTR_DIRECT_TESTS] = total[DC_DIRECT];
    out[RT_CTR_BVH_NODE_TESTS] = total[DC_BVH_NODES];
    if (ctx->accel == RT_ACCEL_BVH) out[RT_CTR_SPHERE_TESTS] = total[DC_CANDIDATES] + total[DC_DIRECT];
    out[RT_CTR_KERNEL_LAUNCHES] = ctx->n_launches.load();
    out[RT_CTR_CULL_NS] = (uint64_t)(ctx->stage_ms[0] * 1e6);
    out[RT_CTR_REFINE_NS] = (uint64_t)(ctx->stage_ms[1] * 1e6);
    out[RT_CTR_TIEBREAK_NS] = (uint64_t)(ctx->stage_ms[2] * 1e6);
    out[RT_CTR_SHADE_NS] = (uint64_t)(ctx->stage_ms[3] * 1e6);
    out[RT_CTR_REDUCE_NS] = (uint64_t)(ctx->reduce_ms * 1e6);
    return RT_OK;
}

int rt_reset_counters(rt_ctx* ctx) {
    if (!ctx) return RT_ERR_ARG;
    std::lock_guard<std::mutex> lk(ctx->mu);
    for (auto& d : ctx->devs) {
        RT_CUDA(ctx, cudaSetDevice(d.dev));
        RT_CUDA(ctx, cudaDeviceSynchronize());
        RT_CUDA(ctx, cudaMemset(d.d_counters, 0, (DC_COUNT + 1) * sizeof(unsigned long long)));
    }
    cudaSetDevice(ctx->devs[0].dev);
    ctx->n_launches = 0;
    for (double& x : ctx->stage_ms) x = 0.0;
    ctx->reduce_ms = 0.0;
    return RT_OK;
}

int rt_set_profile(rt_ctx* ctx, int on) {
    if (!ctx) return RT_ERR_ARG;
    std::lock_guard<std::mutex> lk(ctx->mu);
    ctx->profile = on != 0;
    return RT_OK;
}

}
```

### raytrace_clj_b200/csrc/rt_cull_tc.cuh

```cuda

namespace tc {

constexpr int EW = 16;
constexpr int PG = 1;
constexpr int PW = 4 * PG;
constexpr int THREADS = (EW + 1 + PW) * 32;
constexpr int MAX_SLOTS = 4;
constexpr int TILE_M = 128;
constexpr int TILE_N = 256;
constexpr int KTOT = 32;
constexpr int A_BYTES = TILE_M * KTOT * 4;
constexpr int B_TILE_BYTES = TILE_N * KTOT * 4;
constexpr int MAX_TILES = 4;
constexpr int MIN_LEAVES = 160;
constexpr int CAND_CAP = 256;
constexpr int PAIR_CHUNK = 64;
constexpr float RAY_DEFLATE = 1.0f - 5.0e-6f;
constexpr float DEAD = -1.0e30f;

__host__ __device__ inline size_t canon_off(int rows, int r, int k) {
    return (size_t)(k / 4) * ((size_t)rows * 16) + (size_t)(r / 8) * 128 + (size_t)(r % 8) * 16 + (size_t)(k % 4) * 4;
}
inline size_t smem_bytes(int tiles, int slots) {
    return (size_t)tiles * B_TILE_BYTES + (size_t)tiles * TILE_N * (16 + 4) + (size_t)slots * (A_BYTES + TILE_M * 32) + (size_t)EW * CAND_CAP * 4 + 1024;
}
inline int slots_for(int tiles, size_t smem_limit) {
    int s = MAX_SLOTS;
    while (s > 2 && smem_bytes(tiles, s) > smem_limit) --s;
    return s;
}

__device__ __forceinline__ uint32_t smem_u32(const void* p) { return (uint32_t)__cvta_generic_to_shared(p); }
__device__ __forceinline__ void mbar_init(uint64_t* bar, int count) {
    asm volatile("mbarrier.init.shared::cta.b64 [%0], %1;" ::"r"(smem_u32(bar)), "r"(count) : "memory");
}
__device__ __forceinline__ void mbar_arrive(uint64_t* bar) {
    asm volatile("mbarrier.arrive.shared::cta.b64 _, [%0];" ::"r"(smem_u32(bar)) : "memory");
}
__device__ __forceinline__ bool mbar_try_wait(uint64_t* bar, uint32_t parity) {
    uint32_t ok;
    asm volatile("{\n .reg .pred p;\n mbarrier.try_wait.parity.shared::cta.b64 p, [%1], %2;\n selp.u32 %0, 1, 0, p;\n}"
                 : "=r"(ok) : "r"(smem_u32(bar)), "r"(parity) : "memory");
    return ok != 0;
}
__device__ __forceinline__ void mbar_wait(uint64_t* bar, uint32_t parity) {
    for (unsigned spin = 0; spin < 0x40000000u; ++spin)
        if (mbar_try_wait(bar, parity)) return;
    __trap();
}
__device__ __forceinline__ uint64_t make_desc(uint32_t saddr, uint32_t lbo_bytes, uint32_t sbo_bytes) {
    return (uint64_t)((saddr >> 4) & 0x3fffu) | ((uint64_t)((lbo_bytes >> 4) & 0x3fffu) << 16) | ((uint64_t)((sbo_bytes >> 4) & 0x3fffu) << 32) |
           (1ull << 46);
}
#ifndef RT_TC_NBLK
#define RT_TC_NBLK 1
#endif
constexpr int NBLK = RT_TC_NBLK;
constexpr int BLOCK_N = TILE_N / NBLK;
constexpr int BLOCK_WARPS = EW / NBLK;
constexpr uint32_t IDESC = (1u << 4) | (2u << 7) | (2u << 10) | ((uint32_t)(BLOCK_N >> 3) << 17) | ((uint32_t)(TILE_M >> 4) << 24);
__device__ __forceinline__ void mma_tf32(uint32_t d_tmem, uint64_t adesc, uint64_t bdesc, uint32_t accumulate) {
    asm volatile("{\n .reg .pred p;\n setp.ne.b32 p, %4, 0;\n tcgen05.mma.cta_group::1.kind::tf32 [%0], %1, %2, %3, p;\n}"
                 ::"r"(d_tmem), "l"(adesc), "l"(bdesc), "r"(IDESC), "r"(accumulate) : "memory");
}
__device__ __forceinline__ void mma_commit(uint64_t* bar) {
    asm volatile("tcgen05.commit.cta_group::1.mbarrier::arrive::one.shared::cluster.b64 [%0];" ::"r"(smem_u32(bar)) : "memory");
}
#define RT_TMEM_LD32(taddr, v)                                                                                                \
    asm volatile("tcgen05.ld.sync.aligned.32x32b.x32.b32 "                                                                   \
                 "{%0, %1, %2, %3, %4, %5, %6, %7, %8, %9, %10, %11, %12, %13, %14, %15, "                                   \
                 "%16, %17, %18, %19, %20, %21, %22, %23, %24, %25, %26, %27, %28, %29, %30, %31}, [%32];"                   \
                 : "=r"(v[0]), "=r"(v[1]), "=r"(v[2]), "=r"(v[3]), "=r"(v[4]), "=r"(v[5]), "=r"(v[6]), "=r"(v[7]),           \
                   "=r"(v[8]), "=r"(v[9]), "=r"(v[10]), "=r"(v[11]), "=r"(v[12]), "=r"(v[13]), "=r"(v[14]), "=r"(v[15]),     \
                   "=r"(v[16]), "=r"(v[17]), "=r"(v[18]), "=r"(v[19]), "=r"(v[20]), "=r"(v[21]), "=r"(v[22]), "=r"(v[23]),   \
                   "=r"(v[24]), "=r"(v[25]), "=r"(v[26]), "=r"(v[27]), "=r"(v[28]), "=r"(v[29]), "=r"(v[30]), "=r"(v[31])    \
                 : "r"(taddr))
__device__ __forceinline__ void tmem_wait_ld() { asm volatile("tcgen05.wait::ld.sync.aligned;" ::: "memory"); }
__device__ __forceinline__ void fence_before() { asm volatile("tcgen05.fence::before_thread_sync;" ::: "memory"); }
__device__ __forceinline__ void fence_after() { asm volatile("tcgen05.fence::after_thread_sync;" ::: "memory"); }
__device__ __forceinline__ void fence_async_smem() { asm volatile("fence.proxy.async.shared::cta;" ::: "memory"); }

__host__ __device__ inline float tf32_rn(float x) {
#ifdef __CUDA_ARCH__
    return __uint_as_float((__float_as_uint(x) + 0x1000u) & 0xffffe000u);
#else
    uint32_t b; memcpy(&b, &x, 4); b = (b + 0x1000u) & 0xffffe000u; memcpy(&x, &b, 4); return x;
#endif
}
__device__ __forceinline__ void split2(float x, float& hi, float& lo) {
    hi = tf32_rn(x);
    lo = tf32_rn(x - hi);
}

inline void sphere_slots(const double c[3], double W, float out[KTOT]) {
    auto sp2 = [](double x, float& hi, float& lo) { hi = tf32_rn((float)x); lo = tf32_rn((float)(x - (double)hi)); };
    float wh = tf32_rn((float)W), wl = tf32_rn((float)(W - (double)wh)), wl2 = tf32_rn((float)(W - (double)wh - (double)wl));
    float ch[3], cl[3], dh[3], dl[3], eh[3], el[3];
    for (int i = 0; i < 3; ++i) { sp2(c[i], ch[i], cl[i]); sp2(c[i] * c[i], dh[i], dl[i]); }
    sp2(2.0 * c[0] * c[1], eh[0], el[0]); sp2(2.0 * c[0] * c[2], eh[1], el[1]); sp2(2.0 * c[1] * c[2], eh[2], el[2]);
    const float s[KTOT] = {1.f, 1.f, wh, wl, ch[0], cl[0], ch[0], wl2, ch[1], cl[1], ch[1], el[2], ch[2], cl[2], ch[2], eh[2],
                           dh[0], dl[0], dh[0], dh[1], dl[1], dh[1], dh[2], dl[2], dh[2], eh[0], el[0], eh[0], eh[1], el[1], eh[1], eh[2]};
    for (int k = 0; k < KTOT; ++k) out[k] = s[k];
}
inline void padding_slots(float out[KTOT]) {
    for (int k = 0; k < KTOT; ++k) out[k] = 0.f;
    out[0] = 1.f;
    out[2] = DEAD;
}

struct Smem {
    float* B;
    float4* rec;
    int* row_k;
    unsigned char* A0;
    float4* ray0;
    uint32_t* cand;
    uint64_t* a_ready;
    uint64_t* a_free;
    uint64_t* ray_free;
    uint64_t* d_full;
    uint64_t* d_empty;
    int* tile_of;
    uint32_t* tmem_base;
    unsigned* cand_n;
    __device__ __forceinline__ float* A(unsigned s) const { return reinterpret_cast<float*>(A0 + (size_t)s * A_BYTES); }
    __device__ __forceinline__ float4* ray(unsigned s) const { return ray0 + (size_t)s * TILE_M * 2; }
};
__device__ __forceinline__ Smem carve(unsigned char* base, int tiles, int slots) {
    Smem S;
    S.B = reinterpret_cast<float*>(base);
    unsigned char* p = base + (size_t)tiles * B_TILE_BYTES;
    S.rec = reinterpret_cast<float4*>(p);
    p += (size_t)tiles * TILE_N * 16;
    S.row_k = reinterpret_cast<int*>(p);
    p += (size_t)tiles * TILE_N * 4;
    S.A0 = p;
    p += (size_t)slots * A_BYTES;
    S.ray0 = reinterpret_cast<float4*>(p);
    p += (size_t)slots * TILE_M * 32;
    S.cand = reinterpret_cast<uint32_t*>(p);
    p += (size_t)EW * CAND_CAP * 4;
    uint64_t* bars = reinterpret_cast<uint64_t*>(p);
    S.a_ready = bars; S.a_free = bars + MAX_SLOTS; S.ray_free = bars + 2 * MAX_SLOTS;
    S.d_full = bars + 3 * MAX_SLOTS; S.d_empty = bars + 3 * MAX_SLOTS + 2 * NBLK;
    int* ints = reinterpret_cast<int*>(bars + 3 * MAX_SLOTS + 4 * NBLK);
    S.tile_of = ints;
    S.tmem_base = reinterpret_cast<uint32_t*>(ints + MAX_SLOTS);
    S.cand_n = reinterpret_cast<unsigned*>(ints + MAX_SLOTS + 4);
    return S;
}

}

#ifdef RT_TC_CHECK
#define TC_CHECK(cond, what, a, b) do { if (!(cond)) { printf("wf_cull_tc check failed: %s (%u, %u) block %u thread %u\n", what, (unsigned)(a), (unsigned)(b), blockIdx.x, threadIdx.x); __trap(); } } while (0)
#else
#define TC_CHECK(cond, what, a, b)
#endif

__device__ __forceinline__ void tc_produce_ray(const WaveParams& W, const tc::Smem& S, int slot, int rl, bool live, unsigned v, unsigned n_g,
                                               unsigned p0, unsigned long long gen_base, int cur) {
    const RenderParams& P = W.base;
    float f[tc::KTOT];
    float4 r0, r1;
    if (live) {
        float4* qc = cur ? W.queue[1] : W.queue[0];
        float4 a, b;
        if (v >= n_g && W.tc_pass != 0) {
            const size_t e = (size_t)(p0 + (v - n_g));
            a = qc[3 * e];
            b = qc[3 * e + 1];
        } else if (v >= n_g) {
            float4 c;
            float4* q = qc + 3 * (size_t)(p0 + (v - n_g));
            TC_CHECK(p0 + (v - n_g) < (unsigned)W.capacity, "fresh entry", p0 + (v - n_g), W.capacity);
            TC_CHECK(gen_base + (v - n_g) < P.total_work, "work item", (unsigned)(gen_base + (v - n_g)), (unsigned)P.total_work);
            make_path(P, gen_base + (v - n_g), a, b, c);
            q[0] = a; q[1] = b; q[2] = c;
        } else {
            TC_CHECK(v < (unsigned)W.capacity, "entry in flight", v, W.capacity);
            a = qc[3 * (size_t)v];
            b = qc[3 * (size_t)v + 1];
        }
        const float aa = fmaf(b.z, b.z, fmaf(b.y, b.y, b.x * b.x));
        const float inv = rsqrtf(aa);
        const float qq = fmaf(a.z, a.z, fmaf(a.y, a.y, a.x * a.x));
        {
            const float s = inv * ((1.0f + 0.5f * CULL_EPS) * 0.70710678118654752f);
            const float hx = b.x * s, hy = b.y * s, hz = b.z * s;
            r0 = make_float4(hx, hy, hz, fmaf(a.z, hz, fmaf(a.y, hy, a.x * hx)));
            r1 = make_float4(-2.0f * a.x, -2.0f * a.y, -2.0f * a.z, qq * RAY_DEFLATE);
        }
        const float s = inv * (1.0f + 0.5f * CULL_EPS);
        const float hx = b.x * s, hy = b.y * s, hz = b.z * s;
        const float Pd = fmaf(a.z, hz, fmaf(a.y, hy, a.x * hx));
        const float g0 = fmaf(Pd, Pd, -(qq * tc::RAY_DEFLATE));
        const float gx = 2.0f * fmaf(-Pd, hx, a.x), gy = 2.0f * fmaf(-Pd, hy, a.y), gz = 2.0f * fmaf(-Pd, hz, a.z);
        float h_, l_;
        tc::split2(g0, h_, l_); f[0] = h_; f[1] = l_;
        f[2] = 1.f; f[3] = 1.f; f[7] = 1.f;
        tc::split2(gx, h_, l_); f[4] = h_; f[5] = h_; f[6] = l_;
        tc::split2(gy, h_, l_); f[8] = h_; f[9] = h_; f[10] = l_;
        tc::split2(gz, h_, l_); f[12] = h_; f[13] = h_; f[14] = l_;
        tc::split2(hx * hx, h_, l_); f[16] = h_; f[17] = h_; f[18] = l_;
        tc::split2(hy * hy, h_, l_); f[19] = h_; f[20] = h_; f[21] = l_;
        tc::split2(hz * hz, h_, l_); f[22] = h_; f[23] = h_; f[24] = l_;
        tc::split2(hx * hy, h_, l_); f[25] = h_; f[26] = h_; f[27] = l_;
        tc::split2(hx * hz, h_, l_); f[28] = h_; f[29] = h_; f[30] = l_;
        tc::split2(hy * hz, h_, l_); f[31] = h_; f[11] = h_; f[15] = l_;
    } else {
#pragma unroll
        for (int k = 0; k < tc::KTOT; ++k) f[k] = 0.f;
        f[0] = tc::DEAD;
        f[2] = 1.f;
        r0 = make_float4(1.f, 0.f, 0.f, 0.f);
        r1 = make_float4(0.f, 0.f, 0.f, CUDART_INF_F);
    }
    unsigned char* Ab = reinterpret_cast<unsigned char*>(S.A((unsigned)slot)) + (size_t)(rl >> 3) * 128 + (size_t)(rl & 7) * 16;
#pragma unroll
    for (int kc = 0; kc < tc::KTOT / 4; ++kc)
        *reinterpret_cast<float4*>(Ab + (size_t)kc * (tc::TILE_M * 16)) = make_float4(f[4 * kc], f[4 * kc + 1], f[4 * kc + 2], f[4 * kc + 3]);
    S.ray((unsigned)slot)[2 * rl] = r0;
    S.ray((unsigned)slot)[2 * rl + 1] = r1;
}

struct TcEmit {
    unsigned pos, end;
    unsigned next;
    bool ahead;
    unsigned pads;
};
__device__ __forceinline__ void tc_pad(const WaveParams& W, TcEmit& E, unsigned from, unsigned to, unsigned lane) {
    TC_CHECK(to <= W.pair_cap, "pad", from, to);
#ifdef RT_TC_CHECK
    for (unsigned i = from + lane; i < to; i += 32) W.pairs[i] = make_uint2(PAIR_NULL, (blockIdx.x << 8) | (threadIdx.x >> 5));
#else
    for (unsigned i = from + lane; i < to; i += 32) W.pairs[i] = make_uint2(PAIR_NULL, 0u);
#endif
    if (to > from) E.pads += to - from;
}
__device__ __forceinline__ void tc_request(const WaveParams& W, TcEmit& E, unsigned lane) {
    unsigned b = 0;
    if (lane == 0) b = atomicAdd(&W.st->npairs, (unsigned)tc::PAIR_CHUNK);
    E.next = b;
    E.ahead = true;
}

__device__ __forceinline__ void tc_emit(const WaveParams& W, TcEmit& E, bool emit, unsigned entry, unsigned k, unsigned lane) {
    const unsigned bal = __ballot_sync(0xffffffffu, emit);
    const unsigned total = __popc(bal);
    if (total == 0) return;
    if (E.pos + total > E.end) {
        tc_pad(W, E, E.pos, E.end, lane);
        if (!E.ahead) tc_request(W, E, lane);
        const unsigned b = __shfl_sync(0xffffffffu, E.next, 0);
        E.pos = min(b, W.pair_cap);
        E.end = min(b + (unsigned)tc::PAIR_CHUNK, W.pair_cap);
        tc_request(W, E, lane);
    }
    if (emit) {
        const unsigned w = E.pos + __popc(bal & ((1u << lane) - 1u));
        TC_CHECK(entry < (unsigned)W.capacity && k < (unsigned)W.base.sc.n_list, "pair", entry, k);
        if (w < E.end) W.pairs[w] = make_uint2(entry, k);
        else W.best_key[entry] = BEST_KEY_OVERFLOW;
    }
    E.pos = min(E.pos + total, E.end);
}

__device__ __forceinline__ bool tc_confirm(const tc::Smem& S, float4 r0, float4 r1, unsigned row, int& kk) {
    const float4 R = S.rec[row];
    kk = S.row_k[row];
    const float cc = fmaf(R.x, r0.x, fmaf(R.y, r0.y, fmaf(R.z, r0.z, r0.w)));
    const float s = fmaf(R.x, r1.x, fmaf(R.y, r1.y, fmaf(R.z, r1.z, R.w)));
    const float key = fmaf(-cc, fabsf(cc), fmaf(cc, cc, s - r1.w));
    return (__float_as_uint(key) >> 31) == 0u && kk >= 0;
}

__device__ __noinline__ void tc_redo_fp32(const WaveParams& W, const tc::Smem& S, int slot, unsigned tile, unsigned n, unsigned n_g, unsigned n_p,
                                          int tiles, unsigned cb, unsigned rl) {
    if (tile * tc::TILE_M + rl >= n) return;
    const float4 r0 = S.ray((unsigned)slot)[2 * rl], r1 = S.ray((unsigned)slot)[2 * rl + 1];
    const unsigned entry = wf_entry(tile * tc::TILE_M + rl, n_g, n_p, (unsigned)W.capacity);
    for (int j = 0; j < tiles; ++j)
        for (unsigned q = 0; q < 64u; ++q) {
            int kk;
            if (!tc_confirm(S, r0, r1, (unsigned)j * tc::TILE_N + cb * 64u + q, kk)) continue;
            const unsigned w = atomicAdd(&W.st->npairs, 1u);
            if (w < W.pair_cap) W.pairs[w] = make_uint2(entry, (unsigned)kk);
            else W.best_key[entry] = BEST_KEY_OVERFLOW;
        }
}

__device__ __forceinline__ void tc_drain(const WaveParams& W, const tc::Smem& S, int slot, unsigned tile, unsigned n_g, unsigned n_p,
                                         const uint32_t* cand, unsigned ncand, TcEmit& E, unsigned lane) {
    for (unsigned base = 0; base < ncand; base += 32) {
        const unsigned idx = base + lane;
        bool emit = false;
        unsigned k = 0, entry = 0;
        if (idx < ncand) {
            const uint32_t c = cand[idx];
            const unsigned rl = c >> 20, row = c & 0xfffffu;
            TC_CHECK(rl < 128u && row < (unsigned)W.tc_launch_tiles * 256u, "candidate", c, ncand);
            int kk;
            emit = tc_confirm(S, S.ray((unsigned)slot)[2 * rl], S.ray((unsigned)slot)[2 * rl + 1], row, kk);
            k = (unsigned)kk;
            entry = wf_entry(tile * tc::TILE_M + rl, n_g, n_p, (unsigned)W.capacity);
        }
        tc_emit(W, E, emit, entry, k, lane);
    }
}

#ifdef RT_TC_TIMING
#define TC_T(var) const long long var = clock64()
#define TC_ACC(slot, since) tacc[slot] += clock64() - (since)
#else
#define TC_T(var)
#define TC_ACC(slot, since)
#endif
__global__ void __launch_bounds__(tc::THREADS, 1) wf_cull_tc(const __grid_constant__ WaveParams W) {
    TraceScope trace(W.trace);
    const RenderParams& P = W.base;
    extern __shared__ __align__(1024) unsigned char tc_smem[];
    if (W.st->mode != MODE_RUN) return;
    const unsigned n_g = W.st->cnt[W.cur][0], n_p = W.st->cnt[W.cur][1], n = n_g + n_p;
    if (n == 0) return;
    const unsigned long long gen_base = W.st->gen_base[W.cur];
    const unsigned p0 = (unsigned)W.capacity - n_p;
    const int tiles = W.tc_launch_tiles;
    const unsigned slots = (unsigned)W.tc_slots;
    const tc::Smem S = tc::carve(tc_smem, tiles, (int)slots);
    const unsigned tid = threadIdx.x, warp = tid >> 5, lane = tid & 31u;
    if (blockIdx.x == 0 && tid == 0 && W.tc_pass == 0) atomicAdd(&P.counters[DC_RAYS], (unsigned long long)n);

    const unsigned total_tiles = (n + tc::TILE_M - 1) / tc::TILE_M;
    const unsigned per_cta = W.claims_per_warp > 0 ? (unsigned)W.claims_per_warp : (total_tiles + gridDim.x - 1) / gridDim.x;
    const unsigned first = blockIdx.x * per_cta, last = min(first + per_cta, total_tiles);
    if (first >= last) return;

    if (tid == 0) {
        for (unsigned i = 0; i < slots; ++i) {
            tc::mbar_init(&S.a_ready[i], tc::TILE_M);
            tc::mbar_init(&S.a_free[i], 1);
            tc::mbar_init(&S.ray_free[i], tc::EW);
        }
        for (int i = 0; i < 2 * tc::NBLK; ++i) {
            tc::mbar_init(&S.d_full[i], 1);
            tc::mbar_init(&S.d_empty[i], tc::BLOCK_WARPS);
        }
        asm volatile("fence.mbarrier_init.release.cluster;" ::: "memory");
    }
    if (warp == tc::EW) {
        asm volatile("tcgen05.alloc.cta_group::1.sync.aligned.shared::cta.b32 [%0], %1;" ::"r"(tc::smem_u32(S.tmem_base)), "r"(512) : "memory");
        asm volatile("tcgen05.relinquish_alloc_permit.cta_group::1.sync.aligned;" ::: "memory");
    }
    if (tid < tc::EW) S.cand_n[tid] = 0u;
    {
        const float4* src = reinterpret_cast<const float4*>(P.sc.cull_tc) + (size_t)W.tc_tile0 * (tc::B_TILE_BYTES / 16);
        float4* dst = reinterpret_cast<float4*>(S.B);
        const int n4 = tiles * (tc::B_TILE_BYTES / 16);
        for (int i = (int)tid; i < n4; i += tc::THREADS) dst[i] = __ldg(&src[i]);
        for (int i = (int)tid; i < tiles * tc::TILE_N; i += tc::THREADS) {
            const int k = __ldg(&P.sc.tc_row_k[(size_t)W.tc_tile0 * tc::TILE_N + i]);
            S.row_k[i] = k;
            S.rec[i] = k >= 0 ? __ldg(&P.sc.cull_a[k]) : make_float4(0.f, 0.f, 0.f, -CUDART_INF_F);
        }
    }
    tc::fence_async_smem();
    tc::fence_before();
    __syncthreads();
    tc::fence_after();
    const uint32_t tmem = *S.tmem_base;
    const unsigned n_it = last - first;
#ifdef RT_TC_TIMING
    long long tacc[6] = {0, 0, 0, 0, 0, 0};
    const long long t_begin = clock64();
#endif

    if (warp > tc::EW) {
        const unsigned pt = tid - (tc::EW + 1) * 32, rl = pt & (tc::TILE_M - 1), q = pt / tc::TILE_M;
        for (unsigned it = q; it <= n_it; it += tc::PG) {
            const unsigned s = it % slots, ph = (it / slots) & 1u;
            TC_T(t0);
            if (it >= slots) {
                tc::mbar_wait(&S.a_free[s], ph ^ 1u);
                TC_ACC(0, t0);
                TC_T(t1);
                tc::mbar_wait(&S.ray_free[s], ph ^ 1u);
                TC_ACC(1, t1);
            }
            TC_T(t2);
            if (it < n_it) {
                const unsigned v = (first + it) * tc::TILE_M + rl;
                tc_produce_ray(W, S, (int)s, (int)rl, v < n, v, n_g, p0, gen_base, W.cur);
            }
            TC_ACC(2, t2);
            if (rl == 0) S.tile_of[s] = it < n_it ? (int)(first + it) : -1;
            tc::fence_async_smem();
            tc::mbar_arrive(&S.a_ready[s]);
        }
    } else if (warp == tc::EW) {
        if (lane == 0) {
            const unsigned total = n_it * (unsigned)tiles;
            unsigned gi[tc::NBLK];
#pragma unroll
            for (int c = 0; c < tc::NBLK; ++c) gi[c] = 0;
            unsigned ready_tiles = 0, freed_tiles = 0;
            const uint32_t b_base = tc::smem_u32(S.B);
            for (unsigned idle = 0;;) {
                bool left = false, progressed = false;
#pragma unroll
                for (int c = 0; c < tc::NBLK; ++c) {
                    const unsigned gq = gi[c];
                    if (gq >= total) continue;
                    left = true;
                    const unsigned it = gq / (unsigned)tiles, jt = gq - it * (unsigned)tiles, s = it % slots, b = gq & 1u;
                    if (it >= ready_tiles) {
                        if (!tc::mbar_try_wait(&S.a_ready[s], (it / slots) & 1u)) continue;
                        ready_tiles = it + 1;
                    }
                    if (!tc::mbar_try_wait(&S.d_empty[b * tc::NBLK + c], ((gq >> 1) & 1u) ^ 1u)) continue;
                    tc::fence_after();
                    const uint32_t a_addr = tc::smem_u32(S.A(s));
                    const uint32_t b_addr = b_base + jt * tc::B_TILE_BYTES + (uint32_t)c * (tc::BLOCK_N / 8) * 128;
#pragma unroll
                    for (int kk = 0; kk < tc::KTOT / 8; ++kk)
                        tc::mma_tf32(tmem + b * tc::TILE_N + (uint32_t)c * tc::BLOCK_N, tc::make_desc(a_addr + kk * 2 * tc::TILE_M * 16, tc::TILE_M * 16, 128),
                                     tc::make_desc(b_addr + kk * 2 * tc::TILE_N * 16, tc::TILE_N * 16, 128), kk > 0);
                    tc::mma_commit(&S.d_full[b * tc::NBLK + c]);
                    gi[c] = gq + 1;
                    progressed = true;
                }
                unsigned mn = gi[0];
#pragma unroll
                for (int c = 1; c < tc::NBLK; ++c) mn = min(mn, gi[c]);
                for (const unsigned done = mn / (unsigned)tiles; freed_tiles < done; ++freed_tiles) tc::mma_commit(&S.a_free[freed_tiles % slots]);
                if (!left) break;
                if (progressed) idle = 0;
                else if (++idle > 0x20000000u) __trap();
            }
            tc::mbar_wait(&S.a_free[(n_it - 1) % slots], ((n_it - 1) / slots) & 1u);
        }
        __syncwarp();
    } else {
        const unsigned rl = (warp & 3u) * 32u + lane;
        const unsigned cb = warp >> 2;
        const unsigned blk = warp / tc::BLOCK_WARPS;
        const uint32_t t_lane = ((warp & 3u) * 32u) << 16;
        uint32_t* cand = S.cand + warp * tc::CAND_CAP;
        unsigned* cand_n = S.cand_n + warp;
        TcEmit E{0u, 0u, 0u, false, 0u};
        unsigned g = 0;
        for (unsigned it = 0; it < n_it; ++it) {
            const unsigned s = it % slots, a_ph = (it / slots) & 1u, tile = first + it;
            for (int j = 0; j < tiles; ++j, ++g) {
                const unsigned b = g & 1u;
                TC_T(t0);
                tc::mbar_wait(&S.d_full[b * tc::NBLK + blk], (g >> 1) & 1u);
                TC_ACC(0, t0);
                tc::fence_after();
                const uint32_t taddr = tmem + t_lane + b * tc::TILE_N + cb * 64u;
                unsigned m0, m1;
                TC_T(t1);
                {
                    uint32_t v0[32], v1[32];
                    RT_TMEM_LD32(taddr, v0);
                    RT_TMEM_LD32(taddr + 32u, v1);
                    tc::tmem_wait_ld();
                    tc::fence_before();
                    __syncwarp();
                    if (lane == 0) tc::mbar_arrive(&S.d_empty[b * tc::NBLK + blk]);
                    unsigned w0 = 0u, w1 = 0u;
#pragma unroll
                    for (int q = 0; q < 32; ++q) { w0 = __funnelshift_l(v0[q], w0, 1); w1 = __funnelshift_l(v1[q], w1, 1); }
                    const bool live_ray = tile * tc::TILE_M + rl < n;
                    m0 = live_ray ? ~w0 : 0u; m1 = live_ray ? ~w1 : 0u;
                }
                TC_ACC(1, t1);
                TC_T(t2);
                const unsigned row0 = (unsigned)j * tc::TILE_N + cb * 64u;
#ifdef RT_TC_CHECK
                {
                    const unsigned char* Ab = reinterpret_cast<const unsigned char*>(S.A(s));
                    const unsigned char* Bb = reinterpret_cast<const unsigned char*>(S.B) + (size_t)j * tc::B_TILE_BYTES;
                    for (int q = 0; q < 64; ++q) {
                        double acc = 0.0, mag = 0.0;
                        for (int k = 0; k < tc::KTOT; ++k) {
                            const double x = (double)*reinterpret_cast<const float*>(Ab + tc::canon_off(tc::TILE_M, (int)rl, k)) *
                                             (double)*reinterpret_cast<const float*>(Bb + tc::canon_off(tc::TILE_N, (int)(cb * 64u) + q, k));
                            acc += x; mag += fabs(x);
                        }
                        const unsigned culled = ((q < 32 ? ~m0 : ~m1) >> (31 - (q & 31))) & 1u;
                        if (acc > 1e-4 * mag && culled && mag < 1e20)
                            printf("TMEM mismatch: tile %u ray %u col %u (row %u) double %g (mag %g) but sign bit set; block %u warp %u buffer %u g %u\n", tile, rl, (unsigned)q, row0 + q,
                                   acc, mag, blockIdx.x, warp, b, g);
                        if (acc < -1e-4 * mag && !culled)
                            printf("TMEM mismatch: tile %u ray %u col %u (row %u) double %g (mag %g) but sign bit clear; block %u warp %u buffer %u g %u\n", tile, rl, (unsigned)q, row0 + q,
                                   acc, mag, blockIdx.x, warp, b, g);
                    }
                }
#endif
#pragma unroll
                for (int h = 0; h < 2; ++h) {
                    unsigned mm = h ? m1 : m0;
                    while (mm != 0u) {
                        const int bit = 31 - __clz((int)mm);
                        mm &= ~(1u << bit);
                        const unsigned pos = atomicAdd(cand_n, 1u);
                        if (pos < (unsigned)tc::CAND_CAP) cand[pos] = (rl << 20) | (row0 + (unsigned)h * 32u + (unsigned)(31 - bit));
                    }
                }
                TC_ACC(2, t2);
            }
            TC_T(t3);
            __syncwarp();
            const unsigned raw = *cand_n;
            const bool overflowed = raw > (unsigned)tc::CAND_CAP;
            const unsigned ncand = overflowed ? 0u : raw;
            if (overflowed) {
                tc::mbar_wait(&S.a_ready[s], a_ph);
                tc_redo_fp32(W, S, (int)s, tile, n, n_g, n_p, tiles, cb, rl);
                __syncwarp();
            }
#ifdef RT_TC_CHECK
            if (lane == 0 && ncand > 48u && n < 300u)
                printf("big candidate list: block %u warp %u tile %u it %u ncand %u raw %u first %x %x %x %x last %x\n", blockIdx.x, warp, tile, it, ncand, raw, cand[0], cand[1], cand[2], cand[3], cand[ncand - 1]);
#endif
            if (ncand) {
                tc::mbar_wait(&S.a_ready[s], a_ph);
                tc_drain(W, S, (int)s, tile, n_g, n_p, cand, ncand, E, lane);
            }
            __syncwarp();
            if (lane == 0) {
                *cand_n = 0u;
                tc::mbar_arrive(&S.ray_free[s]);
            }
            __syncwarp();
            TC_ACC(3, t3);
        }
        tc_pad(W, E, E.pos, E.end, lane);
        if (E.ahead) {
            const unsigned b = __shfl_sync(0xffffffffu, E.next, 0);
            tc_pad(W, E, min(b, W.pair_cap), min(b + (unsigned)tc::PAIR_CHUNK, W.pair_cap), lane);
            if (lane == 0 && E.pads) atomicAdd(&W.st->pad, E.pads);
        }
    }
#ifdef RT_TC_TIMING
    if (blockIdx.x == 0 && lane == 0 && n_it > 8)
        printf("tc warp %2u (%s) tiles %u total %lld : %lld %lld %lld %lld cycles per tile\n", warp, warp < tc::EW ? "epi: d_full wait, ld+shf, cand, drain" : (warp == tc::EW ? "mma: a_ready wait, d_empty wait, issue" : "prod: a_free wait, ray_free wait, produce"),
               n_it, (clock64() - t_begin) / n_it, tacc[0] / n_it, tacc[1] / n_it, tacc[2] / n_it, tacc[3] / n_it);
#endif
    tc::fence_before();
    __syncthreads();
    if (warp == tc::EW) asm volatile("tcgen05.dealloc.cta_group::1.sync.aligned.b32 %0, %1;" ::"r"(tmem), "r"(512) : "memory");
}

__global__ void tc_check_fill(const __grid_constant__ WaveParams W, int n, const float* origins, const float* dirs, const float* times) {
    const int i = blockIdx.x * blockDim.x + threadIdx.x;
    if (i == 0) {
        WaveState* st = W.st;
        st->cnt[0][0] = (unsigned)n; st->cnt[0][1] = 0; st->cnt[1][0] = 0; st->cnt[1][1] = 0;
        st->gen_base[0] = 0; st->gen_base[1] = 0;
        st->batch = 0; st->npairs = 0; st->exhausted = 1; st->done = 0; st->mode = MODE_RUN; st->pad = 0;
    }
    if (i >= n) return;
    float4* q = W.queue[0] + 3 * (size_t)i;
    q[0] = make_float4(origins[3 * i], origins[3 * i + 1], origins[3 * i + 2], times ? times[i] : 0.f);
    q[1] = make_float4(dirs[3 * i], dirs[3 * i + 1], dirs[3 * i + 2], 0.f);
    q[2] = make_float4(0.f, 0.f, 0.f, 0.f);
}
__global__ void tc_check_mark(const __grid_constant__ WaveParams W, unsigned* mask, int words) {
    const unsigned npairs = min(W.st->npairs, W.pair_cap);
#ifdef RT_TC_CHECK
    if (blockIdx.x == 0 && threadIdx.x == 0 && W.st->cnt[0][0] < 300u) {
        for (unsigned c0 = 0; c0 < npairs; c0 += 64) {
            unsigned never = 0, real = 0, tag0 = 0xffffffffu, tags = 0;
            for (unsigned i = c0; i < min(c0 + 64u, npairs); ++i) {
                const uint2 pr = W.pairs[i];
                if (pr.x == 0xddddddddu) ++never;
                else if (pr.x == PAIR_NULL) { if (pr.y != tag0) { ++tags; tag0 = pr.y; } }
                else ++real;
            }
            if (never || tags > 1 || real)
                printf("chunk %u: never written %u, real %u, pad-tag changes %u (last tag block %u warp %u)  first entries (%x %x) (%x %x) (%x %x) ... (%x %x)\n", c0, never, real, tags,
                       tag0 >> 8, tag0 & 255u, W.pairs[c0].x, W.pairs[c0].y, W.pairs[c0 + 1].x, W.pairs[c0 + 1].y, W.pairs[c0 + 2].x, W.pairs[c0 + 2].y, W.pairs[c0 + 63].x, W.pairs[c0 + 63].y);
        }
        printf("npairs %u pad counter %u\n", W.st->npairs, W.st->pad);
    }
#endif
    for (unsigned i = blockIdx.x * blockDim.x + threadIdx.x; i < npairs; i += gridDim.x * blockDim.x) {
        const uint2 pr = W.pairs[i];
        if (pr.x != PAIR_NULL && pr.x < (unsigned)W.capacity) atomicOr(&mask[(size_t)pr.x * words + (pr.y >> 5)], 1u << (pr.y & 31u));
    }
}
__global__ void __launch_bounds__(128) tc_check_compare(const __grid_constant__ WaveParams W, int n, double tmin, double tmax, const unsigned* mask,
                                                        int words, unsigned long long* out) {
    const DevScene& sc = W.base.sc;
    const int idx = blockIdx.x * blockDim.x + threadIdx.x;
    unsigned long long lost = 0, surv = 0, cand = 0;
    if (idx < n) {
        const float4 a = W.queue[0][3 * (size_t)idx], b = W.queue[0][3 * (size_t)idx + 1];
        const bool overflow = W.best_key[idx] == BEST_KEY_OVERFLOW;
        for (int k = 0; k < sc.n_list; ++k) {
            const bool kept = overflow || ((mask[(size_t)idx * words + (k >> 5)] >> (k & 31)) & 1u);
            const double t = sc.generic ? refine_leaf<true>(&W.base.sc, k, a.x, a.y, a.z, b.x, b.y, b.z, a.w, tmin, tmax, false, make_uint2(0u, 0u), 0u, 0u, 0u)
                                        : refine_leaf<false>(&W.base.sc, k, a.x, a.y, a.z, b.x, b.y, b.z, a.w, tmin, tmax, false, make_uint2(0u, 0u), 0u, 0u, 0u);
            surv += kept ? 1u : 0u;
            if (t < CUDART_INF) {
                cand++;
                lost += kept ? 0u : 1u;
#ifdef RT_TC_CHECK
                if (!kept) printf("lost pair: ray %d leaf %d t %.9g  o (%.9g %.9g %.9g) d (%.9g %.9g %.9g)\n", idx, k, t, a.x, a.y, a.z, b.x, b.y, b.z);
#endif
            }
        }
    }
    if (lost) atomicAdd(&out[0], lost);
    if (surv) atomicAdd(&out[1], surv);
    if (cand) atomicAdd(&out[2], cand);
}
```

### raytrace_clj_b200/csrc/rt_kernels.cuh

```cuda
#pragma once

#include "rt_device.cuh"

namespace rt {

#define RT_FOR_R _Pragma("unroll") for (int r = 0; r < R; ++r)

struct PathBounce {
    float o[3];
    float time;
    float d[3];
    int hit_id;
    double t;
};

struct RenderParams {
    DevScene sc;
    DevCamera cam;
    int nx, ny;
    int sample_begin, sample_count;
    int row_offset, row_stride, rows_in_shard;
    int max_depth;
    uint2 key;
    float* sum;
// ... 29 lines not shown
        P.path_term[slot] = reason;
    }
}

template <bool GEN>
__device__ __forceinline__ double refine_leaf(const DevScene* sc, int k, float ox, float oy, float oz, float dx, float dy, float dz,
                                              float time, double tmin, double tmax, bool has_ctx, uint2 key, uint32_t pixel,
                                              uint32_t sample, uint32_t bounce) {
    if (!GEN)
        return refine_candidate(sc->ex_c0r, sc->ex_c1, sc->ex_t0t1, sc->flags, k, ox, oy, oz, dx, dy, dz, time, tmin, tmax);
    float mu = 0.5f;
    if (has_ctx && __ldg(&sc->prim_type[k]) == PRIM_MEDIUM) mu = medium_uniform(key, pixel, sample, bounce, __ldg(&sc->orig_id[k]));
    return refine_generic(sc, k, ox, oy, oz, dx, dy, dz, time, tmin, tmax, mu);
}

__device__ __forceinline__ float4 lds128(unsigned addr) {
    float4 v;
    asm("ld.shared.v4.f32 {%0, %1, %2, %3}, [%4];" : "=f"(v.x), "=f"(v.y), "=f"(v.z), "=f"(v.w) : "r"(addr));
    return v;
}
__device__ __forceinline__ unsigned smem_addr(const void* p) {
    unsigned a = (unsigned)__cvta_generic_to_shared(p);
    asm volatile("" : "+r"(a));
    return a;
}

__device__ __forceinline__ int slice_lo(int n, int part, int parts) { return (int)(((long long)n * part) / parts); }

constexpr int GROUP = 32;
constexpr int CHUNK_GROUPS = 16;
constexpr int CHUNK = GROUP * CHUNK_GROUPS;
constexpr int CULL_PAD = 8;
constexpr float RAY_DEFLATE = 1.0f - 3.2e-6f;

template <int R, int BLOCK, bool COMMON = false>
struct Culler {
    float hx[R], hy[R], hz[R];
    float mx[R], my[R], mz[R];
    float P[R];
    float Q[R];
    float cox, coy, coz;

    static constexpr int LIST_WORDS = CHUNK_GROUPS * R;
    static constexpr size_t LIST_BYTES = (size_t)LIST_WORDS * BLOCK * sizeof(uint32_t);

    __device__ __forceinline__ void set_ray(int r, float o_x, float o_y, float o_z, float d_x, float d_y, float d_z) {
        float a = fmaf(d_z, d_z, fmaf(d_y, d_y, d_x * d_x));
        float s = rsqrtf(a) * ((1.0f + 0.5f * CULL_EPS) * 0.70710678118654752f);
        hx[r] = d_x * s; hy[r] = d_y * s; hz[r] = d_z * s;
        mx[r] = -2.0f * o_x; my[r] = -2.0f * o_y; mz[r] = -2.0f * o_z;
        P[r] = fmaf(o_z, hz[r], fmaf(o_y, hy[r], o_x * hx[r]));
        Q[r] = fmaf(o_z, o_z, fmaf(o_y, o_y, o_x * o_x)) * RAY_DEFLATE;
    }
    __device__ __forceinline__ void kill(int r) {
        hx[r] = 1.f; hy[r] = 0.f; hz[r] = 0.f;
        mx[r] = my[r] = mz[r] = 0.f;
        P[r] = 0.f;
        Q[r] = CUDART_INF_F;
    }

    __device__ __forceinline__ void pin() {
        if (COMMON) {
            RT_FOR_R asm volatile("" : "+f"(hx[r]), "+f"(hy[r]), "+f"(hz[r]), "+f"(P[r]));
        } else {
            RT_FOR_R asm volatile("" : "+f"(hx[r]), "+f"(hy[r]), "+f"(hz[r]), "+f"(mx[r]), "+f"(my[r]), "+f"(mz[r]), "+f"(P[r]), "+f"(Q[r]));
        }
    }

    static __device__ __forceinline__ unsigned list_begin(const uint32_t* list) {
        return (unsigned)__cvta_generic_to_shared(list + threadIdx.x);
    }
    static __device__ __forceinline__ unsigned word(const uint32_t* list, int g, int r) {
        return list[(g * R + r) * BLOCK + threadIdx.x];
    }

    static __device__ __forceinline__ float4 common_record(float4 S, float o_x, float o_y, float o_z) {
        const float m_x = -2.0f * o_x, m_y = -2.0f * o_y, m_z = -2.0f * o_z;
        const float q = fmaf(o_z, o_z, fmaf(o_y, o_y, o_x * o_x)) * RAY_DEFLATE;
        S.w = fmaf(S.x, m_x, fmaf(S.y, m_y, fmaf(S.z, m_z, S.w))) - q;
        return S;
    }

    __device__ __forceinline__ unsigned key_bits(const float4 S, int r) const {
        float c = fmaf(S.x, hx[r], fmaf(S.y, hy[r], fmaf(S.z, hz[r], P[r])));
        if (COMMON) return __float_as_uint(fmaf(-c, fabsf(c), fmaf(c, c, S.w)));
        float s = fmaf(S.x, mx[r], fmaf(S.y, my[r], fmaf(S.z, mz[r], S.w)));
        return __float_as_uint(fmaf(-c, fabsf(c), fmaf(c, c, s - Q[r])));
    }

    __device__ __forceinline__ unsigned long long cull_chunk(unsigned sa, int count, uint32_t* list) const {
        unsigned la = list_begin(list);
        unsigned nzr[R];
        RT_FOR_R nzr[r] = 0u;
        const int full = count / GROUP;
        for (int g = 0; g < full; ++g, la += R * BLOCK * 4) {
            unsigned acc[R];
            RT_FOR_R acc[r] = 0u;
#pragma unroll 8
            for (int u = 0; u < GROUP; ++u, sa += 16) {
                const float4 S = lds128(sa);
                RT_FOR_R acc[r] = __funnelshift_l(key_bits(S, r), acc[r], 1);
            }
            RT_FOR_R {
                asm volatile("st.shared.u32 [%0], %1;" ::"r"(la + (unsigned)(r * BLOCK * 4)), "r"(acc[r]) : "memory");
                nzr[r] |= (acc[r] != 0xffffffffu ? 1u : 0u) << g;
            }
        }
        const int rem = count - full * GROUP;
        if (rem) {
            unsigned acc[R];
            RT_FOR_R acc[r] = 0xffffffffu;
            for (int u = 0; u < rem; u += CULL_PAD) {
#pragma unroll
                for (int v = 0; v < CULL_PAD; ++v, sa += 16) {
                    const float4 S = lds128(sa);
                    RT_FOR_R acc[r] = __funnelshift_l(key_bits(S, r), acc[r], 1);
                }
            }
            RT_FOR_R {
                asm volatile("st.shared.u32 [%0], %1;" ::"r"(la + (unsigned)(r * BLOCK * 4)), "r"(acc[r]) : "memory");
                nzr[r] |= (acc[r] != 0xffffffffu ? 1u : 0u) << full;
            }
        }
        unsigned long long nz = 0ull;
        RT_FOR_R nz |= (unsigned long long)nzr[r] << (16 * r);
        return nz;
    }

    template <class Sink>
    __device__ __forceinline__ void run_range(const float4* s_cull, int s0, int s1, int kbase, uint32_t* list, Sink& sink) {
        for (int c0 = s0; c0 < s1; c0 += CHUNK) {
            const int cc = min(CHUNK, s1 - c0);
            const unsigned long long nz = cull_chunk(smem_addr(s_cull + c0), cc, list);
            sink.flush(list, nz, cc, kbase + c0);
        }
    }

    template <class Sink>
    __device__ __forceinline__ void run(const DevScene& sc, float4* s_cull, int cap, bool preloaded, uint32_t* list,
                                        Sink& sink) {
        pin();
        for (int base = 0; base < sc.n_cull; base += cap) {
            const int count = min(cap, sc.n_cull - base);
            if (!preloaded) {
                __syncthreads();
                for (int i = threadIdx.x; i < count; i += BLOCK) {
                    float4 S = __ldg(&sc.cull_a[base + i]);
                    if (COMMON) S = common_record(S, cox, coy, coz);
                    s_cull[i] = S;
                }
                __syncthreads();
            }
            run_range(s_cull, 0, count, base, list, sink);
        }
    }

    template <class Sink>
    __device__ __forceinline__ void run_slice(const DevScene& sc, float4* s_cull, uint32_t* list, Sink& sink, int part,
                                              int parts) {
        pin();
        const int groups = (sc.n_cull + GROUP - 1) / GROUP;
        const int s0 = slice_lo(groups, part, parts) * GROUP, s1 = min(slice_lo(groups, part + 1, parts) * GROUP, sc.n_cull);
        run_range(s_cull, s0, s1, 0, list, sink);
    }
};

__device__ __forceinline__ void preload_scene(const DevScene& sc, float4* s_cull, int block) {
    for (int i = threadIdx.x; i < sc.n_cull; i += block) s_cull[i] = __ldg(&sc.cull_a[i]);
    __syncthreads();
}

template <int R, int BLOCK>
struct SurvivorIter {
    unsigned long long z;
    unsigned sv;
    int g, r, m, full, rem;
    __device__ __forceinline__ void begin(unsigned long long nz, int count) {
        z = nz; sv = 0u; g = 0; r = 0; m = 0;
        full = count / GROUP; rem = count - full * GROUP;
    }
    __device__ __forceinline__ bool next(const uint32_t* list, int& ray, int& k) {
        if (sv == 0u) {
            if (z == 0ull) return false;
            const int i = __ffsll((long long)z) - 1;
            z &= z - 1ull;
            r = i >> 4;
            g = i & 15;
            m = g < full ? GROUP : rem;
            sv = ~Culler<R, BLOCK>::word(list, g, r);
        }
        const int bit = __ffs(sv) - 1;
        sv &= sv - 1u;
        ray = r;
        k = g * GROUP + (m - 1 - bit);
        return true;
    }
};

template <int R, int BLOCK, bool GEN = false>
struct RefineSink {
    float ox[R], oy[R], oz[R];
    float dx[R], dy[R], dz[R];
    float tm[R];
    double best_t[R];
    int best_k[R];
    unsigned best_tie[R];
    unsigned ncand;
    double tmin, tmax;
    const DevScene* sc;
    bool has_ctx;
    uint2 key;
    uint32_t pix[R], smp[R], bounce[R];

    __device__ __forceinline__ void begin() {
        RT_FOR_R {
            best_t[r] = CUDART_INF;
            best_k[r] = -1;
            best_tie[r] = 0xffffffffu;
        }
    }

    __device__ __forceinline__ void refine(int r, int k) {
        float sox = ox[0], soy = oy[0], soz = oz[0], sdx = dx[0], sdy = dy[0], sdz = dz[0], stm = tm[0];
        uint32_t spix = 0, ssmp = 0, sb = 0;
        if (has_ctx) { spix = pix[0]; ssmp = smp[0]; sb = bounce[0]; }
#pragma unroll
        for (int q = 1; q < R; ++q)
            if (r == q) {
                sox = ox[q]; soy = oy[q]; soz = oz[q]; sdx = dx[q]; sdy = dy[q]; sdz = dz[q]; stm = tm[q];
                if (has_ctx) { spix = pix[q]; ssmp = smp[q]; sb = bounce[q]; }
            }
        const double t = refine_leaf<GEN>(sc, k, sox, soy, soz, sdx, sdy, sdz, stm, tmin, tmax, has_ctx, key, spix, ssmp, sb);
        ncand++;
        if (t < CUDART_INF) {
            const unsigned tie = __ldg(&sc->tie_hi[k]);
#pragma unroll
            for (int q = 0; q < R; ++q)
                if (r == q && (t < best_t[q] || (t == best_t[q] && tie < best_tie[q]))) {
                    best_t[q] = t;
                    best_k[q] = k;
                    best_tie[q] = tie;
                }
        }
    }

    __device__ __forceinline__ void flush(const uint32_t* list, unsigned long long nz, int count, int kbase) {
        SurvivorIter<R, BLOCK> it;
        it.begin(nz, count);
        int r, k;
        while (it.next(list, r, k)) refine(r, kbase + k);
    }

    __device__ __forceinline__ unsigned direct(unsigned live) {
        unsigned nd = 0;
        for (int k = sc->n_list; k < sc->n; ++k)
            for (int r = 0; r < R; ++r)
                if ((live >> r) & 1u) { refine(r, k); ++nd; }
        ncand -= nd;
        return nd;
    }
};

struct alignas(8) WaveState {
    unsigned cnt[2][2];
    unsigned long long gen_base[2];
    unsigned batch;
    unsigned npairs;
    unsigned exhausted;
    unsigned done;
    unsigned mode;
    unsigned pad;
};
enum { MODE_RUN = 0, MODE_DONE = 2 };
struct LaneStatus {
    unsigned n_next;
    unsigned n_fresh;
    unsigned exhausted;
    unsigned mode;
    unsigned seq;
    unsigned pad[3];
};
__device__ __forceinline__ unsigned wf_entry(unsigned i, unsigned n_g, unsigned n_p, unsigned capacity) {
    return i < n_g ? i : capacity - n_p + (i - n_g);
}

struct TraceRec {
    unsigned long long t_start, t_end;
};
__device__ __forceinline__ unsigned long long global_timer_ns() {
    unsigned long long t;
    asm volatile("mov.u64 %0, %globaltimer;" : "=l"(t));
    return t;
}
struct TraceScope {
    TraceRec* rec;
    __device__ __forceinline__ explicit TraceScope(TraceRec* r) : rec(r) {
        if (rec && threadIdx.x == 0) atomicMin(&rec->t_start, global_timer_ns());
    }
    __device__ __forceinline__ ~TraceScope() {
        if (rec && threadIdx.x == 0) atomicMax(&rec->t_end, global_timer_ns());
    }
};

struct WaveParams {
    RenderParams base;
    float4* queue[2];
    unsigned long long* best_t;
    unsigned long long* best_key;
    uint2* pairs;
    uint2* cands;
    double* cand_t;
    unsigned* cand_count;
    WaveState* st;
    int capacity;
    unsigned pair_cap;
    int cur;
    int claims_per_warp;
    int resident_warps;
    volatile LaneStatus* status;
    unsigned iter;
    TraceRec* trace;
    int tc_slots;
    int tc_tile0, tc_launch_tiles;
    int tc_pass;
    unsigned tail_solo;
    unsigned tail_lpp;
};
__device__ __forceinline__ void publish_status(const WaveParams& W, unsigned n_next, unsigned n_fresh, unsigned exhausted, unsigned mode,
                                               unsigned seq) {
    if (!W.status) return;
    W.status->n_next = n_next;
    W.status->n_fresh = n_fresh;
    W.status->exhausted = exhausted;
    W.status->mode = mode;
    __threadfence_system();
    W.status->seq = seq;
}

constexpr unsigned long long BEST_T_INIT = 0x7ff0000000000000ull;
constexpr unsigned long long BEST_KEY_MISS = ~0ull;
constexpr unsigned long long BEST_KEY_OVERFLOW = 0ull;
constexpr unsigned PAIR_NULL = 0xffffffffu;

__device__ __forceinline__ unsigned warp_claim(unsigned* counter, bool pred, unsigned lane) {
    unsigned m = __ballot_sync(0xffffffffu, pred);
    unsigned base = 0;
    if (m) {
        int leader = __ffs(m) - 1;
        if ((int)lane == leader) base = atomicAdd(counter, (unsigned)__popc(m));
        base = __shfl_sync(0xffffffffu, base, leader);
    }
    return base + __popc(m & ((1u << lane) - 1u));
}

__device__ __forceinline__ void make_path(const RenderParams& P, unsigned long long w, float4& a, float4& b, float4& c) {
    const unsigned pshard = (unsigned)P.nx * (unsigned)P.rows_in_shard;
    unsigned s_local, q;
    if (P.total_work <= 0xffffffffull) {
        s_local = (unsigned)w / pshard;
        q = (unsigned)w - s_local * pshard;
    } else {
        s_local = (unsigned)(w / pshard);
        q = (unsigned)(w - (unsigned long long)s_local * pshard);
    }
    int row_local = (int)(q / (unsigned)P.nx);
    int i = (int)(q - (unsigned)row_local * (unsigned)P.nx);
    int j = P.row_offset + row_local * P.row_stride;
    uint32_t pix = (uint32_t)j * (uint32_t)P.nx + (uint32_t)i;
    uint32_t smp = (uint32_t)(P.sample_begin + (int)s_local);
    uint32_t slot = pix;
    if (P.path_pixel) {
        pix = (uint32_t)__ldg(&P.path_pixel[w]);
        smp = (uint32_t)__ldg(&P.path_sample[w]);
        j = (int)(pix / (uint32_t)P.nx);
        i = (int)(pix - (uint32_t)j * (uint32_t)P.nx);
        slot = (uint32_t)w;
    }
    float3 o, d;
    float tmv;
    generate_ray(P.cam, P.nx, P.ny, i, j, pix, smp, P.key, o, d, tmv, nullptr);
    a = make_float4(o.x, o.y, o.z, tmv);
    b = make_float4(d.x, d.y, d.z, __uint_as_float(slot));
    c = make_float4(1.f, 1.f, 1.f, __uint_as_float((smp << 8) | (uint32_t)P.max_depth));
}

constexpr int kMaxLanes = 2;
struct InitParams {
    WaveState* st[kMaxLanes];
    unsigned long long first[kMaxLanes];
    unsigned count[kMaxLanes];
    int n_lanes;
    unsigned long long* work_counter;
    unsigned long long* counters;
    unsigned long long total0, total_work;
};
__global__ void wf_init(const InitParams I) {
    for (int l = 0; l < I.n_lanes; ++l) {
        WaveState* st = I.st[l];
        st->cnt[0][0] = 0; st->cnt[0][1] = I.count[l];
        st->cnt[1][0] = 0; st->cnt[1][1] = 0;
        st->gen_base[0] = I.first[l]; st->gen_base[1] = 0;
        st->batch = 0; st->npairs = 0; st->done = 0; st->mode = I.count[l] ? MODE_RUN : MODE_DONE; st->pad = 0;
        st->exhausted = I.total0 >= I.total_work ? 1u : 0u;
    }
    *I.work_counter = I.total0;
    atomicAdd(&I.counters[DC_SAMPLES], I.total0);
}
__global__ void wf_fill_best(unsigned long long* best_t, unsigned long long* best_key, size_t n) {
    for (size_t i = blockIdx.x * (size_t)blockDim.x + threadIdx.x; i < n; i += (size_t)gridDim.x * blockDim.x) {
        best_t[i] = 0x7ff0000000000000ull;
        best_key[i] = ~0ull;
    }
}

template <int R, int BLOCK>
struct PairSink {
    unsigned idx0;
    unsigned n;
    unsigned n_g, p0;
    __device__ __forceinline__ unsigned entry(unsigned v) const { return v < n_g ? v : p0 + (v - n_g); }
    unsigned long long live;
    uint2* pairs;
    unsigned pair_cap;
    unsigned long long* best_key;
    WaveState* st;

    __device__ __forceinline__ void flush(const uint32_t* list, unsigned long long nz, int count, int kbase) {
        nz &= live;
        if (!__any_sync(0xffffffffu, nz != 0ull)) return;
        const unsigned lane = threadIdx.x & 31u;
        unsigned np = 0;
        for (unsigned long long z = nz; z; z &= z - 1ull) {
            const int i = __ffsll((long long)z) - 1;
            np += __popc(~Culler<R, BLOCK>::word(list, i & 15, i >> 4));
        }
        unsigned incl = np;
#pragma unroll
        for (int d = 1; d < 32; d <<= 1) {
            unsigned v = __shfl_up_sync(0xffffffffu, incl, d);
            if ((int)lane >= d) incl += v;
        }
        const unsigned total = __shfl_sync(0xffffffffu, incl, 31);
        unsigned base = 0;
        if (lane == 0) base = atomicAdd(&st->npairs, total);
        base = __shfl_sync(0xffffffffu, base, 0);
        const bool fits = base + total <= pair_cap;
        unsigned w = base + incl - np;
        SurvivorIter<R, BLOCK> it;
        it.begin(nz, count);
        int r, k;
        while (it.next(list, r, k)) {
            const unsigned v = idx0 + 32u * (unsigned)r;
            if (fits) {
                pairs[w] = make_uint2(entry(v), (unsigned)(kbase + k));
            } else {
                if (w < pair_cap) pairs[w] = make_uint2(PAIR_NULL, 0u);
                if (v < n) best_key[entry(v)] = BEST_KEY_OVERFLOW;
            }
            ++w;
        }
    }
};

constexpr unsigned ITEM_NONE = 0xffffffffu;
constexpr unsigned ITEM_STOP = 0xfffffffeu;
struct Scope {
    unsigned bid, nblk;
};
__device__ __forceinline__ Scope grid_scope() { return Scope{blockIdx.x, gridDim.x}; }
template <int R, int BLOCK, bool COMMON>
__device__ __forceinline__ unsigned wf_cull_batches(const WaveParams& W, Scope sc_, int cur, unsigned e0, unsigned e1, unsigned n_g,
                                                    unsigned p0, unsigned long long gen0, int parts, unsigned item0, unsigned claimed,
                                                    int& budget, float4* s_cull, uint32_t* s_list) {
    if (claimed == ITEM_STOP) return ITEM_STOP;
    const RenderParams& P = W.base;
    const unsigned lane = threadIdx.x & 31u, warp = threadIdx.x >> 5, warps = BLOCK / 32;
    const unsigned n_batches = (e1 - e0 + 32 * R - 1) / (32 * R);
    const unsigned n_items = n_batches * (unsigned)parts;
    Culler<R, BLOCK, COMMON> K;
    K.cox = P.cam.origin.x; K.coy = P.cam.origin.y; K.coz = P.cam.origin.z;
    PairSink<R, BLOCK> sink;
    sink.n = e1;
    sink.n_g = n_g;
    sink.p0 = p0;
    sink.pairs = W.pairs;
    sink.pair_cap = W.pair_cap;
    sink.best_key = W.best_key;
    sink.st = W.st;
    unsigned item = sc_.bid * warps + warp;
    const unsigned uniform_end = (n_items + warps - 1) / warps * warps;
    for (;;) {
        if (P.preloaded) {
            if (claimed != ITEM_NONE) {
                item = claimed;
                claimed = ITEM_NONE;
            } else {
                unsigned b = 0;
                if (lane == 0) b = atomicAdd(&W.st->batch, 1u);
                item = __shfl_sync(0xffffffffu, b, 0);
            }
            if (item >= item0 + n_items) return item;
            item -= item0;
        } else {
            if (item - warp >= uniform_end) break;
        }
        const unsigned batch = item / (unsigned)parts, part = item - batch * (unsigned)parts;
        sink.idx0 = e0 + batch * (32 * R) + lane;
        sink.live = 0ull;
        RT_FOR_R {
            const unsigned v = sink.idx0 + 32 * r;
            if (v < e1 && batch < n_batches) {
                float4* qc = cur ? W.queue[1] : W.queue[0];
                float4 a, b;
                if (v >= n_g) {
                    float4 c;
                    float4* q = qc + 3 * (size_t)(p0 + (v - n_g));
                    make_path(P, gen0 + (v - n_g), a, b, c);
                    if (part == 0) { q[0] = a; q[1] = b; q[2] = c; }
                } else {
                    a = qc[3 * (size_t)v];
                    b = qc[3 * (size_t)v + 1];
                }
                K.set_ray(r, a.x, a.y, a.z, b.x, b.y, b.z);
                sink.live |= 0xffffull << (16 * r);
            } else {
                K.kill(r);
            }
        }
        if (parts > 1) K.run_slice(P.sc, s_cull, s_list, sink, (int)part, parts);
        else           K.run(P.sc, s_cull, P.cull_cap, P.preloaded != 0, s_list, sink);
        item += sc_.nblk * warps;
        if (P.preloaded && budget > 0 && --budget == 0) return ITEM_STOP;
    }
    return ITEM_NONE;
}

template <int R, int BLOCK>
__device__ __forceinline__ void wf_cull_body(const WaveParams& W, Scope sc_, int cur, unsigned n_g, unsigned n_p, unsigned long long gen_base,
                                             float4* s_cull, float4* s_cullc, uint32_t* s_list) {
    const RenderParams& P = W.base;
    const unsigned n = n_g + n_p, p0 = (unsigned)W.capacity - n_p;
    if (sc_.bid == 0 && threadIdx.x == 0) atomicAdd(&P.counters[DC_RAYS], (unsigned long long)n);
    const unsigned grid_warps = W.resident_warps > 0 ? (unsigned)W.resident_warps : sc_.nblk * (BLOCK / 32);
    int budget = W.claims_per_warp;
    const unsigned n_c = P.common_origin ? n_p : 0u, n_v = n - n_c;
    const unsigned long long genC = gen_base - p0;
    if (R > 1 && !P.preloaded) {
        if (n_c) wf_cull_batches<R, BLOCK, true>(W, sc_, cur, p0, p0 + n_c, 0u, 0u, genC + 0u, 1, 0u, ITEM_NONE, budget, s_cull, s_list);
        if (n_v) wf_cull_batches<R, BLOCK, false>(W, sc_, cur, 0u, n_v, n_g, p0, gen_base, 1, 0u, ITEM_NONE, budget, s_cull, s_list);
    } else if (R > 1 && n >= grid_warps * 64u) {
        const unsigned tail = grid_warps * 64u, per = 32u * R;
        const unsigned g_rest0 = min(n_v, tail), p_rest0 = min(n_c, tail - g_rest0);
        const unsigned g_bulk = (n_v - g_rest0) / per * per, p_bulk = (n_c - p_rest0) / per * per;
        unsigned items = 0;
        unsigned next = wf_cull_batches<R, BLOCK, true>(W, sc_, cur, p0, p0 + p_bulk, 0u, 0u, genC, 1, items, ITEM_NONE, budget, s_cullc, s_list);
        items += p_bulk / per;
        next = wf_cull_batches<R, BLOCK, false>(W, sc_, cur, 0u, g_bulk, n_g, p0, gen_base, 1, items, next, budget, s_cull, s_list);
        items += g_bulk / per;
        next = wf_cull_batches<1, BLOCK, true>(W, sc_, cur, p0 + p_bulk, p0 + n_c, 0u, 0u, genC, 1, items, next, budget, s_cullc, s_list);
        items += (n_c - p_bulk + 31u) / 32u;
        wf_cull_batches<1, BLOCK, false>(W, sc_, cur, g_bulk, n_v, n_g, p0, gen_base, 1, items, next, budget, s_cull, s_list);
    } else {
        const unsigned b1 = (n + 31) / 32;
        int parts = 1;
        if (P.preloaded)
            while (parts < 16 && b1 * (unsigned)parts * 2u <= grid_warps) parts *= 2;
        unsigned next = ITEM_NONE, items = 0;
        if (n_c) {
            next = wf_cull_batches<1, BLOCK, true>(W, sc_, cur, p0, p0 + n_c, 0u, 0u, genC, parts, 0u, ITEM_NONE, budget, P.preloaded ? s_cullc : s_cull, s_list);
            items = (n_c + 31u) / 32u * (unsigned)parts;
        }
        if (n_v) wf_cull_batches<1, BLOCK, false>(W, sc_, cur, 0u, n_v, n_g, p0, gen_base, parts, items, next, budget, s_cull, s_list);
    }
}

template <int R, int BLOCK, int MINB>
__global__ void __launch_bounds__(BLOCK, MINB) wf_cull(const __grid_constant__ WaveParams W) {
    TraceScope trace(W.trace);
    const RenderParams& P = W.base;
    extern __shared__ float4 smem_f4[];
    float4* s_cull = smem_f4;
    uint32_t* s_list = reinterpret_cast<uint32_t*>(smem_f4 + P.cull_cap);
    float4* s_cullc = reinterpret_cast<float4*>(s_list + Culler<R, BLOCK>::LIST_WORDS * BLOCK);
    if (W.st->mode != MODE_RUN) return;
    const unsigned n_g = W.st->cnt[W.cur][0], n_p = W.st->cnt[W.cur][1];
    if (n_g + n_p == 0) return;
    const unsigned long long gen_base = W.st->gen_base[W.cur];
    if (P.preloaded) {
        preload_scene(P.sc, s_cull, BLOCK);
        if (n_p && P.common_origin)
            for (int i = threadIdx.x; i < P.sc.n_cull; i += BLOCK)
                s_cullc[i] = Culler<R, BLOCK, true>::common_record(s_cull[i], P.cam.origin.x, P.cam.origin.y, P.cam.origin.z);
    }
    __syncthreads();
    wf_cull_body<R, BLOCK>(W, grid_scope(), W.cur, n_g, n_p, gen_base, s_cull, s_cullc, s_list);
}

#include "rt_cull_tc.cuh"

__device__ __forceinline__ unsigned wf_cand_region(const WaveParams& W, unsigned total_warps) {
    return ((W.pair_cap + total_warps * 32u - 1u) / (total_warps * 32u)) * 32u;
}

template <bool GEN>
__device__ __forceinline__ void wf_refine_body(const WaveParams& W, const DevScene* scp, Scope sc_, int cur) {
    const RenderParams& P = W.base;
    const unsigned npairs = min(W.st->npairs, W.pair_cap);
    const unsigned lane = threadIdx.x & 31u;
    if (sc_.bid == 0 && threadIdx.x == 0) {
        W.st->batch = 0;
        W.st->cnt[cur ^ 1][0] = 0;
        W.st->cnt[cur ^ 1][1] = 0;
        atomicAdd(&P.counters[DC_CANDIDATES], (unsigned long long)(npairs - min(npairs, W.st->pad)));
        W.st->pad = 0;
    }
    const unsigned total_warps = sc_.nblk * (blockDim.x >> 5);
    const unsigned warp_id = sc_.bid * (blockDim.x >> 5) + (threadIdx.x >> 5);
    const size_t region = (size_t)warp_id * wf_cand_region(W, total_warps);
    unsigned cnt = 0;
    const unsigned stride = sc_.nblk * blockDim.x;
    const unsigned i_first = sc_.bid * blockDim.x + threadIdx.x;
    uint2 pr_next = i_first < npairs ? W.pairs[i_first] : make_uint2(PAIR_NULL, 0u);
    for (unsigned i0 = i_first - lane; i0 < npairs; i0 += stride) {
        const uint2 pr = pr_next;
        const unsigned i_next = i0 + lane + stride;
        pr_next = i_next < npairs ? W.pairs[i_next] : make_uint2(PAIR_NULL, 0u);
        bool cand = false;
        double t = CUDART_INF;
        if (pr.x != PAIR_NULL) {
            const float4* qc = cur ? W.queue[1] : W.queue[0];
            const float4 a = qc[3 * (size_t)pr.x], b = qc[3 * (size_t)pr.x + 1];
            const unsigned long long seen = __ldcg(&W.best_t[pr.x]);
            if (!GEN) {
                t = refine_candidate(P.sc.ex_c0r, P.sc.ex_c1, P.sc.ex_t0t1, P.sc.flags, (int)pr.y, a.x, a.y, a.z, b.x, b.y, b.z,
                                     a.w, 0.001, (double)FLT_MAX);
            } else {
                uint32_t pixq = 0, smpq = 0, bq = 0;
                if (__ldg(&P.sc.prim_type[pr.y]) == PRIM_MEDIUM) {
                    const uint32_t sd = __float_as_uint(qc[3 * (size_t)pr.x + 2].w);
                    pixq = rng_pixel(P, __float_as_uint(b.w));
                    smpq = sd >> 8;
                    bq = (uint32_t)(P.max_depth - (int)(sd & 255u) + 1);
                }
                t = refine_leaf<true>(scp, (int)pr.y, a.x, a.y, a.z, b.x, b.y, b.z, a.w, 0.001, (double)FLT_MAX, true, P.key, pixq, smpq, bq);
            }
            const unsigned long long tb = (unsigned long long)__double_as_longlong(t);
            if (t < CUDART_INF && tb <= seen) {
                atomicMin(&W.best_t[pr.x], tb);
                cand = true;
            }
        }
        const unsigned m = __ballot_sync(0xffffffffu, cand);
        if (cand) {
            const size_t slot = region + cnt + __popc(m & ((1u << lane) - 1u));
            W.cands[slot] = pr;
            W.cand_t[slot] = t;
        }
        cnt += __popc(m);
    }
    if (lane == 0) W.cand_count[warp_id] = cnt;
}
template <bool GEN>
__global__ void __launch_bounds__(256) wf_refine(const __grid_constant__ WaveParams W) {
    if (W.st->mode != MODE_RUN) return;
    TraceScope trace(W.trace);
    wf_refine_body<GEN>(W, &W.base.sc, grid_scope(), W.cur);
}

__device__ __forceinline__ void wf_tiebreak_body(const WaveParams& W, Scope sc_) {
    const RenderParams& P = W.base;
    const unsigned lane = threadIdx.x & 31u;
    const unsigned total_warps = sc_.nblk * (blockDim.x >> 5);
    const unsigned warp_id = sc_.bid * (blockDim.x >> 5) + (threadIdx.x >> 5);
    const size_t region = (size_t)warp_id * wf_cand_region(W, total_warps);
    const unsigned cnt = W.cand_count[warp_id];
    for (unsigned j = lane; j < cnt; j += 32) {
        const uint2 pr = W.cands[region + j];
        if ((unsigned long long)__double_as_longlong(W.cand_t[region + j]) == W.best_t[pr.x])
            atomicMin(&W.best_key[pr.x], (((unsigned long long)__ldg(&P.sc.tie_hi[pr.y])) << 32) | pr.y);
    }
}
__global__ void __launch_bounds__(256) wf_tiebreak(const __grid_constant__ WaveParams W) {
    if (W.st->mode != MODE_RUN) return;
    TraceScope trace(W.trace);
    wf_tiebreak_body(W, grid_scope());
}

template <bool GEN>
__device__ __noinline__ void exact_closest_hit(const DevScene* sc, float ox, float oy, float oz, float dx, float dy, float dz,
                                               float tm, uint2 key, uint32_t pixel, uint32_t sample, uint32_t bounce, double* out_t,
                                               int* out_k) {
    double best = CUDART_INF;
    int bk = -1;
    unsigned btie = 0xffffffffu;
    for (int k = 0; k < sc->n; ++k) {
        double t = refine_leaf<GEN>(sc, k, ox, oy, oz, dx, dy, dz, tm, 0.001, (double)FLT_MAX, true, key, pixel, sample, bounce);
        if (t < CUDART_INF) {
            unsigned tie = __ldg(&sc->tie_hi[k]);
            if (t < best || (t == best && tie < btie)) { best = t; bk = k; btie = tie; }
        }
    }
    *out_t = best;
    *out_k = bk;
}

template <bool GEN>
__device__ __forceinline__ unsigned wf_shade_body(const WaveParams& W, const DevScene* scp, Scope sc_, int cur, unsigned* s_ctr) {
    const RenderParams& P = W.base;
    const unsigned n_g = W.st->cnt[cur][0], n_p = W.st->cnt[cur][1], n = n_g + n_p;
    const unsigned lane = threadIdx.x & 31u;
    const float4* qc = cur ? W.queue[1] : W.queue[0];
    float4* qn = cur ? W.queue[0] : W.queue[1];
    if (sc_.bid == 0 && threadIdx.x == 0) W.st->npairs = 0;
    unsigned n_direct = 0;
    const unsigned stride = sc_.nblk * blockDim.x;
    for (unsigned idx0 = sc_.bid * blockDim.x + threadIdx.x - lane; idx0 < n; idx0 += stride) {
        const bool have = idx0 + lane < n;
        const unsigned idx = wf_entry(idx0 + lane, n_g, n_p, (unsigned)W.capacity);
        bool cont = false;
        float4 a, b, c;
        if (have) {
            a = qc[3 * (size_t)idx]; b = qc[3 * (size_t)idx + 1]; c = qc[3 * (size_t)idx + 2];
            unsigned long long key = W.best_key[idx];
            const uint32_t slot = __float_as_uint(b.w), sd = __float_as_uint(c.w);
            const uint32_t pix = rng_pixel(P, slot);
            const uint32_t smp = sd >> 8;
            const int depth = (int)(sd & 255u);
            const uint32_t bounce = (uint32_t)(P.max_depth - depth + 1);
            int k = (int)(unsigned)key;
            double td = __longlong_as_double((long long)W.best_t[idx]);
            W.best_key[idx] = BEST_KEY_MISS;
            W.best_t[idx] = BEST_T_INIT;
            if (key == BEST_KEY_OVERFLOW) {
                exact_closest_hit<GEN>(scp, a.x, a.y, a.z, b.x, b.y, b.z, a.w, P.key, pix, smp, bounce, &td, &k);
                key = k < 0 ? BEST_KEY_MISS : 1ull;
            } else {
                for (int kd = P.sc.n_list; kd < P.sc.n; ++kd) {
                    ++n_direct;
                    const double t = refine_leaf<GEN>(scp, kd, a.x, a.y, a.z, b.x, b.y, b.z, a.w, 0.001, (double)FLT_MAX, true, P.key, pix,
                                                      smp, bounce);
                    const unsigned long long kk = (((unsigned long long)__ldg(&P.sc.tie_hi[kd])) << 32) | (unsigned)kd;
                    if (t < td || (t < CUDART_INF && t == td && kk < key)) {
                        td = t;
                        key = kk;
                        k = kd;
                    }
                }
            }
            const bool hit = key != BEST_KEY_MISS;
            if (P.path_pixel) path_log_ray(P, slot, (int)bounce - 1, a, b, hit ? k : -1, hit ? td : CUDART_INF);
            if (!hit) {
                atomicAdd(&s_ctr[DC_TERM_MISS], 1u);
                if (P.path_pixel) path_log_end(P, slot, (int)bounce, TERM_MISS);
            } else {
                float3 o = f3(a.x, a.y, a.z), d = f3(b.x, b.y, b.z);
                float3 att, em;
                int reason = TERM_NONE;
                float tmv = a.w;
                ScatterRng rng{P.key, pix, smp, bounce, nullptr, nullptr};
                cont = shade_hit<GEN>(P.sc, scp, k, (float)td, o, d, tmv, depth > 0, rng, att, em, reason);
                if (em.x != 0.f || em.y != 0.f || em.z != 0.f) {
                    float* dst = P.sum + (size_t)slot * 3;
                    atomicAdd(dst + 0, c.x * em.x);
                    atomicAdd(dst + 1, c.y * em.y);
                    atomicAdd(dst + 2, c.z * em.z);
                }
                if (cont) {
                    a = make_float4(o.x, o.y, o.z, tmv);
                    b = make_float4(d.x, d.y, d.z, b.w);
                    c = make_float4(c.x * att.x, c.y * att.y, c.z * att.z, __uint_as_float((smp << 8) | (uint32_t)(depth - 1)));
                } else {
                    atomicAdd(&s_ctr[reason == TERM_LIGHT ? DC_TERM_LIGHT
                                     : reason == TERM_ABSORB ? DC_TERM_ABSORB : DC_TERM_DEPTH], 1u);
                    if (P.path_pixel) path_log_end(P, slot, (int)bounce, reason);
                }
            }
        }
        const unsigned mc = __ballot_sync(0xffffffffu, cont);
        if (mc) {
            unsigned base = 0u;
            if (lane == 0) base = atomicAdd(&W.st->cnt[cur ^ 1][0], (unsigned)__popc(mc));
            base = __shfl_sync(0xffffffffu, base, 0);
            if (cont) {
                float4* q = qn + 3 * (size_t)(base + __popc(mc & ((1u << lane) - 1u)));
                q[0] = a; q[1] = b; q[2] = c;
            }
        }
    }
    if (n_direct) atomicAdd(&s_ctr[DC_DIRECT], n_direct);
    return 0u;
}

template <bool GEN>
__global__ void __launch_bounds__(256, GEN ? 1 : 0) wf_shade(const __grid_constant__ WaveParams W) {
    if (W.st->mode != MODE_RUN) return;
    TraceScope trace(W.trace);
    const RenderParams& P = W.base;
    __shared__ unsigned s_ctr[DC_COUNT];
    if (threadIdx.x < DC_COUNT) s_ctr[threadIdx.x] = 0;
    __syncthreads();
    wf_shade_body<GEN>(W, &W.base.sc, grid_scope(), W.cur, s_ctr);
    __syncthreads();
    if (threadIdx.x < DC_COUNT && s_ctr[threadIdx.x]) atomicAdd(&P.counters[threadIdx.x], (unsigned long long)s_ctr[threadIdx.x]);
    if (threadIdx.x == 0) {
        __threadfence();
        if (atomicAdd(&W.st->done, 1u) == gridDim.x - 1) {
            __threadfence();
            W.st->done = 0;
            const unsigned n_cont = *(volatile unsigned*)&W.st->cnt[W.cur ^ 1][0];
            const unsigned want = (unsigned)W.capacity - n_cont;
            unsigned n_fresh = 0;
            unsigned long long base = 0ull;
            if (!W.st->exhausted && want) {
                base = atomicAdd(P.work_counter, (unsigned long long)want);
                if (base < P.total_work) n_fresh = (unsigned)min((unsigned long long)want, P.total_work - base);
                if (base + want >= P.total_work) W.st->exhausted = 1u;
            }
            W.st->cnt[W.cur ^ 1][1] = n_fresh;
            W.st->gen_base[W.cur ^ 1] = base;
            if (n_fresh) atomicAdd(&P.counters[DC_SAMPLES], (unsigned long long)n_fresh);
            if (n_cont + n_fresh == 0) W.st->mode = MODE_DONE;
            __threadfence();
            publish_status(W, n_cont + n_fresh, n_fresh, W.st->exhausted, W.st->mode, W.iter);
        }
    }
}

struct TraceParamsB {
    DevScene sc;
    int n;
    const float* origins;
    const float* dirs;
    const float* times;
    double tmin, tmax;
    double* out_t;
    int* out_id;
    unsigned long long* stats;
};

struct BvhHit {
    double t;
    int k;
    unsigned tie;
    unsigned n_leaf, n_node;
};
template <bool GEN>
__device__ __forceinline__ BvhHit bvh_closest(const DevScene* sc, float ox, float oy, float oz, float dx, float dy, float dz, float time,
                                              double tmin, double tmax, bool has_ctx, uint2 key, uint32_t pixel, uint32_t sample,
                                              uint32_t bounce) {
    BvhHit H{CUDART_INF, -1, 0xffffffffu, 0u, 0u};
    const float ix = 1.0f / dx, iy = 1.0f / dy, iz = 1.0f / dz;
    const float e = 2.4e-7f * fmaxf(fmaxf(fabsf(ox), fabsf(oy)), fabsf(oz));
    const float tlo = (float)tmin * (1.0f - 1e-6f);
    float thi = tmax >= (double)FLT_MAX ? FLT_MAX : __double2float_ru(tmax);
    int stack[48];
    int sp = 0, node = 0;
    for (;;) {
        if (node >= 0) {
            const float4 A = __ldg(&sc->bvh[4 * node]), B = __ldg(&sc->bvh[4 * node + 1]), C = __ldg(&sc->bvh[4 * node + 2]);
            const int4 D = __ldg(reinterpret_cast<const int4*>(&sc->bvh[4 * node + 3]));
            H.n_node += 2;
            float a0 = ((A.x - e) - ox) * ix, a1 = ((A.w + e) - ox) * ix, b0 = ((A.y - e) - oy) * iy, b1 = ((B.x + e) - oy) * iy,
                  c0 = ((A.z - e) - oz) * iz, c1 = ((B.y + e) - oz) * iz;
            float ln = fmaxf(fmaxf(fminf(a0, a1), fminf(b0, b1)), fmaxf(fminf(c0, c1), tlo));
            float lf = fminf(fminf(fmaxf(a0, a1), fmaxf(b0, b1)), fminf(fmaxf(c0, c1), thi));
            a0 = ((B.z - e) - ox) * ix; a1 = ((C.y + e) - ox) * ix; b0 = ((B.w - e) - oy) * iy; b1 = ((C.z + e) - oy) * iy;
            c0 = ((C.x - e) - oz) * iz; c1 = ((C.w + e) - oz) * iz;
            float rn = fmaxf(fmaxf(fminf(a0, a1), fminf(b0, b1)), fmaxf(fminf(c0, c1), tlo));
            float rf = fminf(fminf(fmaxf(a0, a1), fmaxf(b0, b1)), fminf(fmaxf(c0, c1), thi));
            const bool hl = ln <= lf * 1.0000005f + 1e-30f, hr = rn <= rf * 1.0000005f + 1e-30f;
            if (hl && hr) {
                const bool left_first = ln <= rn;
                stack[sp++] = left_first ? D.y : D.x;
                node = left_first ? D.x : D.y;
                continue;
            }
            if (hl) { node = D.x; continue; }
            if (hr) { node = D.y; continue; }
        } else {
            const int k = ~node;
            H.n_leaf++;
            const double t = refine_leaf<GEN>(sc, k, ox, oy, oz, dx, dy, dz, time, tmin, tmax, has_ctx, key, pixel, sample, bounce);
            if (t < CUDART_INF) {
                const unsigned tie = __ldg(&sc->tie_hi[k]);
                if (t < H.t || (t == H.t && tie < H.tie)) {
                    H.t = t; H.k = k; H.tie = tie;
                    thi = fminf(thi, __double2float_ru(t));
                }
            }
        }
        if (sp == 0) break;
        node = stack[--sp];
    }
    return H;
}

template <bool GEN>
__global__ void __launch_bounds__(128, GEN ? 1 : 0) wf_bvh(const __grid_constant__ WaveParams W) {
    if (W.st->mode != MODE_RUN) return;
    TraceScope trace(W.trace);
    const RenderParams& P = W.base;
    __shared__ unsigned s_ctr[DC_COUNT];
    if (threadIdx.x < DC_COUNT) s_ctr[threadIdx.x] = 0;
    __syncthreads();
    const int cur = W.cur;
    const unsigned n_g = W.st->cnt[cur][0], n_p = W.st->cnt[cur][1], n = n_g + n_p, p0 = (unsigned)W.capacity - n_p;
    const unsigned long long gen_base = W.st->gen_base[cur];
    float4* qc = cur ? W.queue[1] : W.queue[0];
    unsigned n_leaf = 0, n_node = 0;
    for (unsigned v = blockIdx.x * blockDim.x + threadIdx.x; v < n; v += gridDim.x * blockDim.x) {
        float4 a, b, c;
        unsigned idx;
        if (v >= n_g) {
            idx = p0 + (v - n_g);
            make_path(P, gen_base + (v - n_g), a, b, c);
            float4* q = qc + 3 * (size_t)idx;
            q[0] = a; q[1] = b; q[2] = c;
        } else {
            idx = v;
            a = qc[3 * (size_t)idx]; b = qc[3 * (size_t)idx + 1]; c = qc[3 * (size_t)idx + 2];
        }
        const uint32_t sd = __float_as_uint(c.w);
        const BvhHit H = bvh_closest<GEN>(&W.base.sc, a.x, a.y, a.z, b.x, b.y, b.z, a.w, 0.001, (double)FLT_MAX, true, P.key,
                                          rng_pixel(P, __float_as_uint(b.w)), sd >> 8, (uint32_t)(P.max_depth - (int)(sd & 255u) + 1));
        n_leaf += H.n_leaf; n_node += H.n_node;
        if (H.k >= 0) {
            W.best_t[idx] = (unsigned long long)__double_as_longlong(H.t);
            W.best_key[idx] = ((unsigned long long)H.tie << 32) | (unsigned)H.k;
        }
    }
    atomicAdd(&s_ctr[DC_CANDIDATES], n_leaf);
    atomicAdd(&s_ctr[DC_BVH_NODES], n_node);
    __syncthreads();
    if (threadIdx.x < DC_COUNT && s_ctr[threadIdx.x]) atomicAdd(&P.counters[threadIdx.x], (unsigned long long)s_ctr[threadIdx.x]);
    if (blockIdx.x == 0 && threadIdx.x == 0) {
        atomicAdd(&P.counters[DC_RAYS], (unsigned long long)n);
        W.st->batch = 0;
        W.st->npairs = 0;
        W.st->cnt[cur ^ 1][0] = 0;
        W.st->cnt[cur ^ 1][1] = 0;
    }
}

template <bool GEN>
__global__ void __launch_bounds__(128) trace_bvh_kernel(const __grid_constant__ TraceParamsB P) {
    const int idx = blockIdx.x * blockDim.x + threadIdx.x;
    if (idx >= P.n) return;
    const float ox = P.origins[3 * idx], oy = P.origins[3 * idx + 1], oz = P.origins[3 * idx + 2];
    const float dx = P.dirs[3 * idx], dy = P.dirs[3 * idx + 1], dz = P.dirs[3 * idx + 2];
    const float tm = P.times ? P.times[idx] : 0.f;
    BvhHit H = bvh_closest<GEN>(&P.sc, ox, oy, oz, dx, dy, dz, tm, P.tmin, P.tmax, false, make_uint2(0u, 0u), 0u, 0u, 0u);
    for (int k = P.sc.n_list; k < P.sc.n; ++k) {
        const double t = refine_leaf<GEN>(&P.sc, k, ox, oy, oz, dx, dy, dz, tm, P.tmin, P.tmax, false, make_uint2(0u, 0u), 0u, 0u, 0u);
        const unsigned tie = __ldg(&P.sc.tie_hi[k]);
        if (t < H.t || (t < CUDART_INF && t == H.t && tie < H.tie)) { H.t = t; H.k = k; H.tie = tie; }
    }
    P.out_t[idx] = H.t;
    P.out_id[idx] = H.k >= 0 ? __ldg(&P.sc.orig_id[H.k]) : -1;
    if (P.stats) {
        atomicAdd(&P.stats[0], (unsigned long long)H.n_leaf);
        atomicAdd(&P.stats[1], (unsigned long long)H.n_node);
    }
}

template <bool GEN>
__device__ __forceinline__ void wf_solo_paths(const WaveParams& W, const DevScene* scp, const float4* qc, unsigned n, unsigned* claim,
                                              const float4* s_cull, unsigned* s_ctr) {
    const RenderParams& P = W.base;
    const unsigned lane = threadIdx.x & 31u;
    const unsigned lpp = W.tail_lpp;
    const unsigned sub = lane & (lpp - 1u), lead = lane & ~(lpp - 1u);
    bool active = false;
    float4 a = make_float4(0.f, 0.f, 0.f, 0.f), b = a, c = a;
    uint32_t slot = 0u, pix = 0u;
    unsigned n_rays = 0, n_cand = 0, n_direct = 0;
    for (;;) {
        unsigned i = 0xffffffffu;
        if (!active && sub == 0u) i = atomicAdd(claim, 1u);
        i = __shfl_sync(0xffffffffu, i, (int)lead);
        if (!active && i < n) {
            a = qc[3 * (size_t)i]; b = qc[3 * (size_t)i + 1]; c = qc[3 * (size_t)i + 2];
            slot = __float_as_uint(b.w);
            pix = rng_pixel(P, slot);
            active = true;
        }
        if (!__any_sync(0xffffffffu, active)) break;
        const uint32_t sd = __float_as_uint(c.w), smp = sd >> 8;
        const int depth = (int)(sd & 255u);
        const uint32_t bounce = (uint32_t)(P.max_depth - depth + 1);
        Culler<1, 32, false> K;
        K.set_ray(0, a.x, a.y, a.z, b.x, b.y, b.z);
        if (active && sub == 0u) ++n_rays;
        unsigned long long bt = BEST_T_INIT, bkey = BEST_KEY_MISS;
        for (int base = 0; base < P.sc.n; base += 64 * (int)lpp) {
            unsigned long long mask = 0ull;
            if (active) {
                const int jn = min(64, (P.sc.n - base + (int)lpp - 1) / (int)lpp);
#pragma unroll 4
                for (int j = 0; j < jn; ++j) {
                    const int s = base + (int)lpp * j + (int)sub;
                    bool pass = s < P.sc.n;
                    if (s < P.sc.n_list) {
                        const float4 S = P.preloaded ? s_cull[s] : __ldg(&P.sc.cull_a[s]);
                        pass = (int)K.key_bits(S, 0) >= 0;
                    }
                    mask |= (unsigned long long)(pass ? 1u : 0u) << j;
                }
            }
            while (__any_sync(0xffffffffu, mask != 0ull)) {
                if (mask) {
                    const int s = base + (int)lpp * (__ffsll((long long)mask) - 1) + (int)sub;
                    mask &= mask - 1ull;
                    if (s < P.sc.n_list) ++n_cand; else ++n_direct;
                    const double t = refine_leaf<GEN>(scp, s, a.x, a.y, a.z, b.x, b.y, b.z, a.w, 0.001, (double)FLT_MAX, true, P.key, pix, smp,
                                                      bounce);
                    const unsigned long long tb = (unsigned long long)__double_as_longlong(t);
                    const unsigned long long kk = (((unsigned long long)__ldg(&P.sc.tie_hi[s])) << 32) | (unsigned)s;
                    if (t < CUDART_INF && (tb < bt || (tb == bt && kk < bkey))) { bt = tb; bkey = kk; }
                }
            }
        }
        for (unsigned dlt = lpp >> 1; dlt; dlt >>= 1) {
            const unsigned long long ot = __shfl_xor_sync(0xffffffffu, bt, (int)dlt), ok = __shfl_xor_sync(0xffffffffu, bkey, (int)dlt);
            if (ot < bt || (ot == bt && ok < bkey)) { bt = ot; bkey = ok; }
        }
        if (active) {
            const bool hit = bkey != BEST_KEY_MISS;
            const int k = (int)(unsigned)bkey;
            const double td = __longlong_as_double((long long)bt);
            if (P.path_pixel && sub == 0u) path_log_ray(P, slot, (int)bounce - 1, a, b, hit ? k : -1, hit ? td : CUDART_INF);
            int reason = TERM_MISS;
            bool cont = false;
            if (hit) {
                float3 o = f3(a.x, a.y, a.z), d = f3(b.x, b.y, b.z);
                float3 att, em;
                float tmv = a.w;
                ScatterRng rng{P.key, pix, smp, bounce, nullptr, nullptr};
                reason = TERM_NONE;
                cont = shade_hit<GEN>(P.sc, scp, k, (float)td, o, d, tmv, depth > 0, rng, att, em, reason);
                if (sub == 0u && (em.x != 0.f || em.y != 0.f || em.z != 0.f)) {
                    float* dst = P.sum + (size_t)slot * 3;
                    atomicAdd(dst + 0, c.x * em.x);
                    atomicAdd(dst + 1, c.y * em.y);
                    atomicAdd(dst + 2, c.z * em.z);
                }
                if (cont) {
                    a = make_float4(o.x, o.y, o.z, tmv);
                    b = make_float4(d.x, d.y, d.z, b.w);
                    c = make_float4(c.x * att.x, c.y * att.y, c.z * att.z, __uint_as_float((smp << 8) | (uint32_t)(depth - 1)));
                }
            }
            if (!cont) {
                if (sub == 0u) {
                    atomicAdd(&s_ctr[reason == TERM_MISS ? DC_TERM_MISS : reason == TERM_LIGHT ? DC_TERM_LIGHT
                                     : reason == TERM_ABSORB ? DC_TERM_ABSORB : DC_TERM_DEPTH], 1u);
                    if (P.path_pixel) path_log_end(P, slot, (int)bounce, reason);
                }
                active = false;
            }
        }
    }
    if (n_rays) atomicAdd(&s_ctr[DC_RAYS], n_rays);
    if (n_cand) atomicAdd(&s_ctr[DC_CANDIDATES], n_cand);
    if (n_direct) atomicAdd(&s_ctr[DC_DIRECT], n_direct);
}

constexpr int kPairsPerEntry = 8;
template <int BLOCK, bool GEN, int TR>
__global__ void __launch_bounds__(BLOCK, GEN ? 1 : 2) wf_tail(const __grid_constant__ WaveParams W) {
    const RenderParams& P = W.base;
    extern __shared__ float4 smem_f4[];
    float4* s_cull = smem_f4;
    uint32_t* s_list = reinterpret_cast<uint32_t*>(smem_f4 + P.cull_cap);
    __shared__ unsigned s_ctr[DC_COUNT];
    __shared__ WaveState s_st;
    if (W.st->mode == MODE_DONE) return;
    TraceScope trace(W.trace);
    int cur = W.cur;
    const unsigned n_all = W.st->cnt[cur][0];
    const unsigned K = ((n_all + gridDim.x - 1) / gridDim.x + 31u) / 32u * 32u;
    const unsigned first = blockIdx.x * K;
    if (first < n_all) {
        if (threadIdx.x < DC_COUNT) s_ctr[threadIdx.x] = 0;
        if (threadIdx.x == 0) {
            s_st.cnt[cur][0] = min(K, n_all - first);
            s_st.cnt[cur ^ 1][0] = 0;
            s_st.cnt[0][1] = s_st.cnt[1][1] = 0;
            s_st.gen_base[0] = s_st.gen_base[1] = 0ull;
            s_st.batch = 0;
            s_st.npairs = 0;
            s_st.exhausted = 1;
            s_st.done = 0;
            s_st.mode = MODE_RUN;
            s_st.pad = 0;
        }
        const unsigned warps = BLOCK / 32;
        WaveParams L = W;
        L.queue[0] = W.queue[0] + 3 * (size_t)first;
        L.queue[1] = W.queue[1] + 3 * (size_t)first;
        L.best_t = W.best_t + first;
        L.best_key = W.best_key + first;
        L.pairs = W.pairs + (size_t)first * kPairsPerEntry;
        L.pair_cap = min(K, (unsigned)W.capacity - first) * kPairsPerEntry;
        const size_t cand_slice = (size_t)wf_cand_region(L, warps) * warps;
        L.cands = W.cands + (size_t)blockIdx.x * cand_slice;
        L.cand_t = W.cand_t + (size_t)blockIdx.x * cand_slice;
        L.cand_count = W.cand_count + blockIdx.x * warps;
        L.st = &s_st;
        L.status = nullptr;
        L.capacity = (int)K;
        L.claims_per_warp = 0;
        L.resident_warps = 0;
        if (P.preloaded) preload_scene(P.sc, s_cull, BLOCK);
        const Scope solo{0u, 1u};
        for (;;) {
            __syncthreads();
            const unsigned n = *(volatile unsigned*)&s_st.cnt[cur][0];
#ifdef RT_TAIL_DIAG
            const bool diag = (blockIdx.x == 0 || blockIdx.x == gridDim.x / 2) && threadIdx.x == 0;
            unsigned long long dt0 = global_timer_ns();
#endif
            if (n <= W.tail_solo) {
                if (n) wf_solo_paths<GEN>(L, &W.base.sc, cur ? L.queue[1] : L.queue[0], n, &s_st.done, s_cull, s_ctr);
#ifdef RT_TAIL_DIAG
                __syncthreads();
                if (diag) printf("tail cta %u solo n %u: %llu ns\n", blockIdx.x, n, global_timer_ns() - dt0);
#endif
                break;
            }
            wf_cull_body<TR, BLOCK>(L, solo, cur, n, 0u, 0ull, s_cull, nullptr, s_list);
            __syncthreads();
#ifdef RT_TAIL_DIAG
            unsigned long long dt1 = global_timer_ns();
            const unsigned np_ = s_st.npairs;
#endif
            wf_refine_body<GEN>(L, &W.base.sc, solo, cur);
            __syncthreads();
#ifdef RT_TAIL_DIAG
            unsigned long long dt2 = global_timer_ns();
#endif
            wf_tiebreak_body(L, solo);
            __syncthreads();
#ifdef RT_TAIL_DIAG
            unsigned long long dt3 = global_timer_ns();
#endif
            wf_shade_body<GEN>(L, &W.base.sc, solo, cur, s_ctr);
#ifdef RT_TAIL_DIAG
            __syncthreads();
            if (diag) printf("tail cta %u n %u pairs %u: cull %llu refine %llu tie %llu shade %llu ns\n", blockIdx.x, n, np_, dt1 - dt0, dt2 - dt1, dt3 - dt2, global_timer_ns() - dt3);
#endif
            cur ^= 1;
        }
        __syncthreads();
        if (threadIdx.x < DC_COUNT && s_ctr[threadIdx.x]) atomicAdd(&P.counters[threadIdx.x], (unsigned long long)s_ctr[threadIdx.x]);
    }
    if (threadIdx.x == 0) {
        __threadfence();
        if (atomicAdd(&W.st->done, 1u) == gridDim.x - 1) {
            W.st->done = 0;
            W.st->cnt[0][0] = W.st->cnt[0][1] = W.st->cnt[1][0] = W.st->cnt[1][1] = 0;
            W.st->mode = MODE_DONE;
            __threadfence();
            publish_status(W, 0u, 0u, 1u, MODE_DONE, W.iter);
        }
    }
}


struct MegaShade {
    float4 o_t;
    float4 d_c;
    float4 att_r;
    float4 em;
};
template <bool GEN>
__device__ __noinline__ MegaShade mega_shade_one(const DevScene* scp, int k, float t, float ox, float oy, float oz, float dx, float dy,
                                                 float dz, float time, int allow_scatter, uint2 key, uint32_t pix, uint32_t smp,
                                                 uint32_t bounce) {
    float3 o = f3(ox, oy, oz), d = f3(dx, dy, dz), att, em;
    int reason = TERM_NONE;
    ScatterRng rng{key, pix, smp, bounce, nullptr, nullptr};
    const bool cont = shade_hit<GEN>(*scp, scp, k, t, o, d, time, allow_scatter != 0, rng, att, em, reason);
    MegaShade m;
    m.o_t = make_float4(o.x, o.y, o.z, time);
    m.d_c = make_float4(d.x, d.y, d.z, cont ? 1.f : 0.f);
    m.att_r = make_float4(att.x, att.y, att.z, (float)reason);
    m.em = make_float4(em.x, em.y, em.z, 0.f);
    return m;
}

template <int R, int BLOCK, int MINB, bool GEN>
__global__ void __launch_bounds__(BLOCK, MINB) mega_kernel(const __grid_constant__ RenderParams P) {
    extern __shared__ float4 smem_f4[];
    float4* s_cull = smem_f4;
    uint32_t* s_list = reinterpret_cast<uint32_t*>(smem_f4 + P.cull_cap);
    __shared__ unsigned s_ctr[DC_COUNT];
    if (threadIdx.x < DC_COUNT) s_ctr[threadIdx.x] = 0;
    if (P.preloaded) preload_scene(P.sc, s_cull, BLOCK);
    __syncthreads();

    Culler<R, BLOCK> K;
    RefineSink<R, BLOCK, GEN> I;
    I.tmin = 0.001;
    I.tmax = (double)FLT_MAX;
    I.ncand = 0;
    I.sc = &P.sc;
    I.has_ctx = true;
    I.key = P.key;

    float ar[R], ag[R], ab[R];
    uint32_t slot[R];
    uint32_t (&pix)[R] = I.pix, (&smp)[R] = I.smp;
    int depth[R];
    bool alive[R];
    RT_FOR_R { alive[r] = false; I.ox[r] = I.oy[r] = I.oz[r] = I.tm[r] = 0.f; I.dx[r] = 1.f; I.dy[r] = I.dz[r] = 0.f; pix[r] = smp[r] = slot[r] = 0u; I.bounce[r] = 0u; }
    unsigned n_rays = 0, n_samples = 0, n_direct = 0;
    const unsigned lane = threadIdx.x & 31u;
    const unsigned pshard = (unsigned)P.nx * (unsigned)P.rows_in_shard;

    for (;;) {
        RT_FOR_R {
            unsigned need = __ballot_sync(0xffffffffu, !alive[r]);
            if (need) {
                int leader = __ffs(need) - 1;
                unsigned long long base = 0;
                if ((int)lane == leader) base = atomicAdd(P.work_counter, (unsigned long long)__popc(need));
                base = __shfl_sync(0xffffffffu, base, leader);
                unsigned long long w = base + __popc(need & ((1u << lane) - 1u));
                if (!alive[r] && w < P.total_work) {
                    unsigned s_local = (unsigned)(w / pshard);
                    unsigned q = (unsigned)(w - (unsigned long long)s_local * pshard);
                    int row_local = (int)(q / (unsigned)P.nx);
                    int i = (int)(q - (unsigned)row_local * (unsigned)P.nx);
                    int j = P.row_offset + row_local * P.row_stride;
                    pix[r] = (uint32_t)j * (uint32_t)P.nx + (uint32_t)i;
                    smp[r] = (uint32_t)(P.sample_begin + (int)s_local);
                    slot[r] = pix[r];
                    if (P.path_pixel) {
                        pix[r] = (uint32_t)__ldg(&P.path_pixel[w]);
                        smp[r] = (uint32_t)__ldg(&P.path_sample[w]);
                        j = (int)(pix[r] / (uint32_t)P.nx);
                        i = (int)(pix[r] - (uint32_t)j * (uint32_t)P.nx);
                        slot[r] = (uint32_t)w;
                    }
                    float3 o, d;
                    generate_ray(P.cam, P.nx, P.ny, i, j, pix[r], smp[r], P.key, o, d, I.tm[r], nullptr);
                    I.ox[r] = o.x; I.oy[r] = o.y; I.oz[r] = o.z;
                    I.dx[r] = d.x; I.dy[r] = d.y; I.dz[r] = d.z;
                    ar[r] = ag[r] = ab[r] = 1.0f;
                    depth[r] = P.max_depth;
                    alive[r] = true;
                    n_samples++;
                }
            }
        }
        bool any_alive = false;
        RT_FOR_R any_alive |= alive[r];
        if (P.preloaded) {
            if (!__any_sync(0xffffffffu, any_alive)) break;
        } else {
            if (!__syncthreads_or(any_alive)) break;
        }

        unsigned live = 0;
        RT_FOR_R {
            if (alive[r]) { K.set_ray(r, I.ox[r], I.oy[r], I.oz[r], I.dx[r], I.dy[r], I.dz[r]); n_rays++; live |= 1u << r; }
            else K.kill(r);
            I.bounce[r] = (uint32_t)(P.max_depth - depth[r] + 1);
        }
        I.begin();
        K.run(P.sc, s_cull, P.cull_cap, P.preloaded != 0, s_list, I);
        n_direct += I.direct(live);

        RT_FOR_R {
            if (alive[r]) {
                if (P.path_pixel)
                    path_log_ray(P, slot[r], (int)I.bounce[r] - 1, make_float4(I.ox[r], I.oy[r], I.oz[r], I.tm[r]),
                                 make_float4(I.dx[r], I.dy[r], I.dz[r], 0.f), I.best_k[r], I.best_t[r]);
                if (I.best_k[r] < 0) {
                    alive[r] = false;
                    atomicAdd(&s_ctr[DC_TERM_MISS], 1u);
                    if (P.path_pixel) path_log_end(P, slot[r], (int)I.bounce[r], TERM_MISS);
                } else {
                    const MegaShade ms = mega_shade_one<GEN>(&P.sc, I.best_k[r], (float)I.best_t[r], I.ox[r], I.oy[r], I.oz[r], I.dx[r], I.dy[r],
                                                             I.dz[r], I.tm[r], depth[r] > 0 ? 1 : 0, P.key, pix[r], smp[r], I.bounce[r]);
                    const float3 o = f3(ms.o_t.x, ms.o_t.y, ms.o_t.z), d = f3(ms.d_c.x, ms.d_c.y, ms.d_c.z);
                    const float3 att = f3(ms.att_r.x, ms.att_r.y, ms.att_r.z), em = f3(ms.em.x, ms.em.y, ms.em.z);
                    const bool cont = ms.d_c.w != 0.f;
                    const int reason = (int)ms.att_r.w;
                    I.tm[r] = ms.o_t.w;
                    if (em.x != 0.f || em.y != 0.f || em.z != 0.f) {
                        float* dst = P.sum + (size_t)slot[r] * 3;
                        atomicAdd(dst + 0, ar[r] * em.x);
                        atomicAdd(dst + 1, ag[r] * em.y);
                        atomicAdd(dst + 2, ab[r] * em.z);
                    }
                    if (cont) {
                        ar[r] *= att.x; ag[r] *= att.y; ab[r] *= att.z;
                        I.ox[r] = o.x; I.oy[r] = o.y; I.oz[r] = o.z;
                        I.dx[r] = d.x; I.dy[r] = d.y; I.dz[r] = d.z;
                        depth[r]--;
                    } else {
                        alive[r] = false;
                        atomicAdd(&s_ctr[reason == TERM_LIGHT ? DC_TERM_LIGHT
                                         : reason == TERM_ABSORB ? DC_TERM_ABSORB : DC_TERM_DEPTH], 1u);
                        if (P.path_pixel) path_log_end(P, slot[r], (int)I.bounce[r], reason);
                    }
                }
            }
        }
    }

    atomicAdd(&s_ctr[DC_RAYS], n_rays);
    atomicAdd(&s_ctr[DC_SAMPLES], n_samples);
    atomicAdd(&s_ctr[DC_CANDIDATES], I.ncand);
    atomicAdd(&s_ctr[DC_DIRECT], n_direct);
    __syncthreads();
    if (threadIdx.x < DC_COUNT && s_ctr[threadIdx.x]) atomicAdd(&P.counters[threadIdx.x], (unsigned long long)s_ctr[threadIdx.x]);
}

struct TraceParams {
    DevScene sc;
    int n;
    const float* origins;
    const float* dirs;
    const float* times;
    double tmin, tmax;
    double* out_t;
    int* out_id;
    int cull_cap, preloaded;
};

template <int R, int BLOCK, bool GEN>
__global__ void __launch_bounds__(BLOCK) trace_kernel(const __grid_constant__ TraceParams P) {
    extern __shared__ float4 smem_f4[];
    float4* s_cull = smem_f4;
    uint32_t* s_list = reinterpret_cast<uint32_t*>(smem_f4 + P.cull_cap);
    if (P.preloaded) preload_scene(P.sc, s_cull, BLOCK);
    __syncthreads();
    Culler<R, BLOCK> K;
    RefineSink<R, BLOCK, GEN> I;
    I.tmin = P.tmin;
    I.tmax = P.tmax;
    I.ncand = 0;
    I.sc = &P.sc;
    I.has_ctx = false;
    for (long long base = (long long)blockIdx.x * BLOCK * R; base < P.n; base += (long long)gridDim.x * BLOCK * R) {
        unsigned live = 0;
        RT_FOR_R {
            long long idx = base + (long long)r * BLOCK + threadIdx.x;
            if (idx < P.n) {
                I.ox[r] = P.origins[3 * idx]; I.oy[r] = P.origins[3 * idx + 1]; I.oz[r] = P.origins[3 * idx + 2];
                I.dx[r] = P.dirs[3 * idx]; I.dy[r] = P.dirs[3 * idx + 1]; I.dz[r] = P.dirs[3 * idx + 2];
                I.tm[r] = P.times ? P.times[idx] : 0.f;
                K.set_ray(r, I.ox[r], I.oy[r], I.oz[r], I.dx[r], I.dy[r], I.dz[r]);
                live |= 1u << r;
            } else {
                I.ox[r] = I.oy[r] = I.oz[r] = I.tm[r] = 0.f;
                I.dx[r] = 1.f; I.dy[r] = 0.f; I.dz[r] = 0.f;
                K.kill(r);
            }
        }
        I.begin();
        K.run(P.sc, s_cull, P.cull_cap, P.preloaded != 0, s_list, I);
        I.direct(live);
        RT_FOR_R {
            long long idx = base + (long long)r * BLOCK + threadIdx.x;
            if (idx < P.n) {
                P.out_t[idx] = I.best_t[r];
                P.out_id[idx] = (I.best_k[r] >= 0) ? __ldg(&P.sc.orig_id[I.best_k[r]]) : -1;
            }
        }
    }
}

__global__ void __launch_bounds__(128) cull_check_kernel(const __grid_constant__ DevScene sc, int n, const float* origins, const float* dirs,
                                                         const float* times, double tmin, double tmax,
                                                         unsigned long long* out) {
    const int idx = blockIdx.x * blockDim.x + threadIdx.x;
    unsigned long long lost = 0, surv = 0, cand = 0;
    if (idx < n) {
        const float ox = origins[3 * idx], oy = origins[3 * idx + 1], oz = origins[3 * idx + 2];
        const float dx = dirs[3 * idx], dy = dirs[3 * idx + 1], dz = dirs[3 * idx + 2];
        const float tm = times ? times[idx] : 0.f;
        Culler<1, 128> K;
        K.set_ray(0, ox, oy, oz, dx, dy, dz);
        K.pin();
        for (int k = 0; k < sc.n_list; ++k) {
            const bool culled = (K.key_bits(__ldg(&sc.cull_a[k]), 0) >> 31) != 0u;
            const double t = sc.generic ? refine_leaf<true>(&sc, k, ox, oy, oz, dx, dy, dz, tm, tmin, tmax, false, make_uint2(0u, 0u), 0u, 0u, 0u)
                                        : refine_leaf<false>(&sc, k, ox, oy, oz, dx, dy, dz, tm, tmin, tmax, false, make_uint2(0u, 0u), 0u, 0u, 0u);
            surv += culled ? 0u : 1u;
            if (t < CUDART_INF) {
                cand++;
                lost += culled ? 1u : 0u;
            }
        }
    }
    if (lost) atomicAdd(&out[0], lost);
    if (surv) atomicAdd(&out[1], surv);
    if (cand) atomicAdd(&out[2], cand);
}

__global__ void sampler_kernel(int kind, int n, uint2 key, float* out) {
    const int i = blockIdx.x * blockDim.x + threadIdx.x;
    if (i >= n) return;
    if (kind == 0) {
        const float3 p = rand_in_unit_sphere(key, (uint32_t)i, 0u, 1u, 1u);
        out[3 * i] = p.x; out[3 * i + 1] = p.y; out[3 * i + 2] = p.z;
    } else {
        const float2 p = rand_in_unit_disk(key, (uint32_t)i, 0u, 1u);
        out[2 * i] = p.x; out[2 * i + 1] = p.y;
    }
}

__global__ void genrays_kernel(DevCamera cam, int n, int nx, int ny, const int* ij, const int* s, uint2 key, float* out_o,
                               float* out_d, float* out_t, float* out_rnd) {
    int idx = blockIdx.x * blockDim.x + threadIdx.x;
    if (idx >= n) return;
    int i = ij[2 * idx], j = ij[2 * idx + 1];
    float3 o, d;
    float tm;
    float rnd[5];
    generate_ray(cam, nx, ny, i, j, (uint32_t)j * (uint32_t)nx + (uint32_t)i, (uint32_t)s[idx], key, o, d, tm, rnd);
    out_o[3 * idx] = o.x; out_o[3 * idx + 1] = o.y; out_o[3 * idx + 2] = o.z;
    out_d[3 * idx] = d.x; out_d[3 * idx + 1] = d.y; out_d[3 * idx + 2] = d.z;
    out_t[idx] = tm;
    if (out_rnd)
        for (int k = 0; k < 5; ++k) out_rnd[5 * idx + k] = rnd[k];
}

__global__ void shade_kernel(const __grid_constant__ DevScene sc, int n, const float* origins, const float* dirs, const float* times,
                             const int* hit_id, const double* hit_t, const float* ball, const float* u01v, float* out_o,
                             float* out_d, float* out_att, float* out_em, int* out_flags) {
    int idx = blockIdx.x * blockDim.x + threadIdx.x;
    if (idx >= n) return;
    float3 o = f3(origins[3 * idx], origins[3 * idx + 1], origins[3 * idx + 2]);
    float3 d = f3(dirs[3 * idx], dirs[3 * idx + 1], dirs[3 * idx + 2]);
    float3 att = f3(0.f, 0.f, 0.f), em = f3(0.f, 0.f, 0.f);
    int flag = -1;
    int id = hit_id[idx];
    if (id >= 0 && id < sc.n) {
        int k = sc.cull_of_orig[id];
        int reason = TERM_NONE;
        ScatterRng rng{make_uint2(0u, 0u), 0u, 0u, 0u, ball + 3 * idx, u01v + idx};
        float tmv = times ? times[idx] : 0.f;
        bool cont = sc.generic ? shade_hit<true>(sc, &sc, k, (float)hit_t[idx], o, d, tmv, true, rng, att, em, reason)
                               : shade_hit<false>(sc, &sc, k, (float)hit_t[idx], o, d, tmv, true, rng, att, em, reason);
        flag = cont ? 1 : 0;
        if (!cont) {
            o = f3(0.f, 0.f, 0.f); d = o; att = o;
        }
// ... 69 lines not shown
```

Measured before the change: 1.607 billion.

## Merge hit t and key into 128-bit record, drop tiebreak pass via CAS

Replaces the separate best_t/best_key arrays and the candidate buffers with one 16-byte HitRec per entry. Refine now merges (t, key) atomically with a 128-bit compare-and-swap loop, so the tiebreak kernel and its candidate staging are removed and each wave iteration launches one kernel fewer. Shade also prefetches the next entry's queue and hit record into L1. The cost is CAS retry loops under contention and a dependence on 128-bit global atomics, which need recent hardware.

```diff
diff --git a/raytrace_clj_b200/csrc/rt_api.cu b/raytrace_clj_b200/csrc/rt_api.cu
--- a/raytrace_clj_b200/csrc/rt_api.cu
+++ b/raytrace_clj_b200/csrc/rt_api.cu
@@ -45,11 +45,8 @@
     unsigned long long* d_counters = nullptr;
     struct WaveLane {
         float4* queue = nullptr;
-        unsigned long long* best = nullptr;
+        HitRec* best = nullptr;
         uint2* pairs = nullptr;
-        uint2* cands = nullptr;
-        double* cand_t = nullptr;
-        unsigned* cand_count = nullptr;
         WaveState* state = nullptr;
         LaneStatus* h_status = nullptr;
         LaneStatus* d_status = nullptr;
@@ -147,7 +144,7 @@
     std::atomic<uint64_t> n_launches{0};
     std::mutex err_mu;
     bool profile = false;
-    double stage_ms[4] = {0, 0, 0, 0};
+    double stage_ms[3] = {0, 0, 0};
     double reduce_ms = 0.0;
     std::vector<bool> peer_ok;
     NcclApi nccl;
@@ -202,10 +199,7 @@
     if (L.queue) cudaFree(L.queue);
     if (L.best) cudaFree(L.best);
     if (L.pairs) cudaFree(L.pairs);
-    if (L.cands) cudaFree(L.cands);
-    if (L.cand_t) cudaFree(L.cand_t);
-    if (L.cand_count) cudaFree(L.cand_count);
-    L.queue = nullptr; L.best = nullptr; L.pairs = nullptr; L.cands = nullptr; L.cand_t = nullptr; L.cand_count = nullptr;
+    L.queue = nullptr; L.best = nullptr; L.pairs = nullptr;
     L.entries = 0;
 }
 
@@ -245,12 +239,8 @@
     if (L.entries >= entries) return RT_OK;
     free_lane(L);
     RT_CUDA(ctx, cudaMalloc(&L.queue, entries * 2 * 3 * sizeof(float4)));
-    RT_CUDA(ctx, cudaMalloc(&L.best, entries * 2 * sizeof(unsigned long long)));
+    RT_CUDA(ctx, cudaMalloc(&L.best, entries * sizeof(HitRec)));
     RT_CUDA(ctx, cudaMalloc(&L.pairs, entries * kPairsPerEntry * sizeof(uint2)));
-    const size_t cand_slots = entries * kPairsPerEntry + (size_t)d.sm_count * 8 * 8 * 32;
-    RT_CUDA(ctx, cudaMalloc(&L.cands, cand_slots * sizeof(uint2)));
-    RT_CUDA(ctx, cudaMalloc(&L.cand_t, cand_slots * sizeof(double)));
-    RT_CUDA(ctx, cudaMalloc(&L.cand_count, (size_t)d.sm_count * 8 * 8 * sizeof(unsigned)));
     L.entries = entries;
     L.best_clean = false;
     return RT_OK;
@@ -395,12 +385,8 @@
         W[l].base = P;
         W[l].queue[0] = L.queue;
         W[l].queue[1] = L.queue + 3 * capacity;
-        W[l].best_t = L.best;
-        W[l].best_key = L.best + L.entries;
+        W[l].best = L.best;
         W[l].pairs = L.pairs;
-        W[l].cands = L.cands;
-        W[l].cand_t = L.cand_t;
-        W[l].cand_count = L.cand_count;
         W[l].st = L.state;
         W[l].capacity = (int)capacity;
         W[l].pair_cap = (unsigned)std::min<size_t>(capacity * kPairsPerEntry, 0xfffffff0u);
@@ -453,7 +439,7 @@
         I.count[l] = count0[l];
         first += count0[l];
         if (!L.best_clean) {
-            wf_fill_best<<<d.sm_count * 4, 256, 0, stream>>>(L.best, L.best + L.entries, L.entries);
+            wf_fill_best<<<d.sm_count * 4, 256, 0, stream>>>(L.best, L.entries);
             ctx->n_launches += 1;
         }
         L.best_clean = false;
@@ -482,7 +468,7 @@
             all_done = false;
             DeviceBuffers::WaveLane& L = d.lanes[l];
             while (!tailed[l] && enq[l] - seen[l] < depth) {
-                cudaEvent_t e[5] = {nullptr, nullptr, nullptr, nullptr, nullptr};
+                cudaEvent_t e[4] = {nullptr, nullptr, nullptr, nullptr};
                 if (ctx->profile)
                     for (auto& x : e) { RT_CUDA(ctx, cudaEventCreate(&x)); evs.push_back(x); }
                 if (ctx->profile) cudaEventRecord(e[0], st[l]);
@@ -491,11 +477,11 @@
                 if (bvh) {
                     W[l].trace = trace_slot("bvh", l, iter_no[l]);
                     k_bvh<<<light_grid, 128, 0, st[l]>>>(W[l]);
-                    if (ctx->profile) { cudaEventRecord(e[1], st[l]); cudaEventRecord(e[2], st[l]); cudaEventRecord(e[3], st[l]); }
+                    if (ctx->profile) { cudaEventRecord(e[1], st[l]); cudaEventRecord(e[2], st[l]); }
                     W[l].trace = trace_slot("shade", l, iter_no[l]);
                     k_shade<<<light_grid, light_block, 0, st[l]>>>(W[l]);
-                    if (ctx->profile) cudaEventRecord(e[4], st[l]);
-                    ctx->n_launches -= 2;
+                    if (ctx->profile) cudaEventRecord(e[3], st[l]);
+                    ctx->n_launches -= 1;
                 } else if (claims) {
                     W[l].trace = trace_slot("cull", l, iter_no[l]);
                     if (debug_sync) {
@@ -519,9 +505,6 @@
                     W[l].trace = trace_slot("refine", l, iter_no[l]);
                     k_refine<<<light_grid, light_block, 0, L.stage_stream>>>(W[l]);
                     if ((rc = dbg("wf_refine", l, enq[l]))) return rc;
-                    W[l].trace = trace_slot("tiebreak", l, iter_no[l]);
-                    wf_tiebreak<<<light_grid, light_block, 0, L.stage_stream>>>(W[l]);
-                    if ((rc = dbg("wf_tiebreak", l, enq[l]))) return rc;
                     W[l].trace = trace_slot("shade", l, iter_no[l]);
                     k_shade<<<light_grid, light_block, 0, L.stage_stream>>>(W[l]);
                     if ((rc = dbg("wf_shade", l, enq[l]))) return rc;
@@ -538,17 +521,14 @@
                     W[l].trace = trace_slot("refine", l, iter_no[l]);
                     k_refine<<<light_grid, light_block, 0, st[l]>>>(W[l]);
                     if (ctx->profile) cudaEventRecord(e[2], st[l]);
-                    W[l].trace = trace_slot("tiebreak", l, iter_no[l]);
-                    wf_tiebreak<<<light_grid, light_block, 0, st[l]>>>(W[l]);
-                    if (ctx->profile) cudaEventRecord(e[3], st[l]);
                     W[l].trace = trace_slot("shade", l, iter_no[l]);
                     k_shade<<<light_grid, light_block, 0, st[l]>>>(W[l]);
-                    if (ctx->profile) cudaEventRecord(e[4], st[l]);
+                    if (ctx->profile) cudaEventRecord(e[3], st[l]);
                 }
                 RT_CUDA(ctx, cudaGetLastError());
                 W[l].cur ^= 1;
                 ++iter_no[l];
-                ctx->n_launches += 4;
+                ctx->n_launches += 3;
                 ++enq[l];
                 progressed = true;
             }
@@ -599,8 +579,8 @@
     for (int l = 0; l < n_lanes; ++l) d.lanes[l].best_clean = true;
     if (ctx->profile) {
         RT_CUDA(ctx, cudaStreamSynchronize(stream));
-        for (size_t i = 0; i + 4 < evs.size(); i += 5)
-            for (int sgi = 0; sgi < 4; ++sgi) {
+        for (size_t i = 0; i + 3 < evs.size(); i += 4)
+            for (int sgi = 0; sgi < 3; ++sgi) {
                 float ms = 0.f;
                 if (cudaEventElapsedTime(&ms, evs[i + sgi], evs[i + sgi + 1]) == cudaSuccess) ctx->stage_ms[sgi] += ms;
             }
@@ -1958,16 +1938,12 @@
         W.base.max_depth = 1;
         W.queue[0] = L.queue;
         W.queue[1] = L.queue + 3 * L.entries;
-        W.best_t = L.best;
-        W.best_key = L.best + L.entries;
+        W.best = L.best;
         W.pairs = L.pairs;
-        W.cands = L.cands;
-        W.cand_t = L.cand_t;
-        W.cand_count = L.cand_count;
         W.st = L.state;
         W.capacity = (int)L.entries;
         W.pair_cap = (unsigned)std::min<size_t>(L.entries * kPairsPerEntry, 0xfffffff0u);
-        wf_fill_best<<<d.sm_count * 4, 256, 0, d.stream>>>(L.best, L.best + L.entries, L.entries);
+        wf_fill_best<<<d.sm_count * 4, 256, 0, d.stream>>>(L.best, L.entries);
 #ifdef RT_TC_CHECK
         RT_CUDA(ctx, cudaMemsetAsync(L.pairs, 0xDD, (size_t)W.pair_cap * sizeof(uint2), d.stream));
 #endif
@@ -2160,8 +2136,8 @@
     out[RT_CTR_KERNEL_LAUNCHES] = ctx->n_launches.load();
     out[RT_CTR_CULL_NS] = (uint64_t)(ctx->stage_ms[0] * 1e6);
     out[RT_CTR_REFINE_NS] = (uint64_t)(ctx->stage_ms[1] * 1e6);
-    out[RT_CTR_TIEBREAK_NS] = (uint64_t)(ctx->stage_ms[2] * 1e6);
-    out[RT_CTR_SHADE_NS] = (uint64_t)(ctx->stage_ms[3] * 1e6);
+    out[RT_CTR_TIEBREAK_NS] = 0;
+    out[RT_CTR_SHADE_NS] = (uint64_t)(ctx->stage_ms[2] * 1e6);
     out[RT_CTR_REDUCE_NS] = (uint64_t)(ctx->reduce_ms * 1e6);
     return RT_OK;
 }
diff --git a/raytrace_clj_b200/csrc/rt_cull_tc.cuh b/raytrace_clj_b200/csrc/rt_cull_tc.cuh
--- a/raytrace_clj_b200/csrc/rt_cull_tc.cuh
+++ b/raytrace_clj_b200/csrc/rt_cull_tc.cuh
@@ -262,7 +262,7 @@
         const unsigned w = E.pos + __popc(bal & ((1u << lane) - 1u));
         TC_CHECK(entry < (unsigned)W.capacity && k < (unsigned)W.base.sc.n_list, "pair", entry, k);
         if (w < E.end) W.pairs[w] = make_uint2(entry, k);
-        else W.best_key[entry] = BEST_KEY_OVERFLOW;
+        else hit_store(&W.best[entry], HIT_OVERFLOW);
     }
     E.pos = min(E.pos + total, E.end);
 }
@@ -287,7 +287,7 @@
             if (!tc_confirm(S, r0, r1, (unsigned)j * tc::TILE_N + cb * 64u + q, kk)) continue;
             const unsigned w = atomicAdd(&W.st->npairs, 1u);
             if (w < W.pair_cap) W.pairs[w] = make_uint2(entry, (unsigned)kk);
-            else W.best_key[entry] = BEST_KEY_OVERFLOW;
+            else hit_store(&W.best[entry], HIT_OVERFLOW);
         }
 }
 
@@ -599,7 +599,7 @@
     unsigned long long lost = 0, surv = 0, cand = 0;
     if (idx < n) {
         const float4 a = W.queue[0][3 * (size_t)idx], b = W.queue[0][3 * (size_t)idx + 1];
-        const bool overflow = W.best_key[idx] == BEST_KEY_OVERFLOW;
+        const bool overflow = hit_is_overflow(W.best[idx]);
         for (int k = 0; k < sc.n_list; ++k) {
             const bool kept = overflow || ((mask[(size_t)idx * words + (k >> 5)] >> (k & 31)) & 1u);
             const double t = sc.generic ? refine_leaf<true>(&W.base.sc, k, a.x, a.y, a.z, b.x, b.y, b.z, a.w, tmin, tmax, false, make_uint2(0u, 0u), 0u, 0u, 0u)
diff --git a/raytrace_clj_b200/csrc/rt_kernels.cuh b/raytrace_clj_b200/csrc/rt_kernels.cuh
--- a/raytrace_clj_b200/csrc/rt_kernels.cuh
+++ b/raytrace_clj_b200/csrc/rt_kernels.cuh
@@ -355,15 +355,50 @@
     }
 };
 
+struct alignas(16) HitRec {
+    unsigned long long t, key;
+};
+constexpr unsigned long long BEST_T_INIT = 0x7ff0000000000000ull;
+constexpr unsigned long long BEST_KEY_MISS = ~0ull;
+__device__ constexpr HitRec HIT_NONE{BEST_T_INIT, BEST_KEY_MISS};
+__device__ constexpr HitRec HIT_OVERFLOW{0ull, 0ull};
+__device__ __forceinline__ bool hit_less(const HitRec& a, const HitRec& b) {
+    return a.t < b.t || (a.t == b.t && a.key < b.key);
+}
+__device__ __forceinline__ bool hit_is_overflow(const HitRec& h) { return (h.t | h.key) == 0ull; }
+__device__ __forceinline__ HitRec hit_load_cg(const HitRec* p) {
+    const ulonglong2 v = __ldcg(reinterpret_cast<const ulonglong2*>(p));
+    return HitRec{v.x, v.y};
+}
+__device__ __forceinline__ void hit_store(HitRec* p, const HitRec& h) {
+    *reinterpret_cast<ulonglong2*>(p) = make_ulonglong2(h.t, h.key);
+}
+__device__ __forceinline__ HitRec hit_cas(HitRec* p, const HitRec& cmp, const HitRec& val) {
+    HitRec old;
+    asm volatile("{\n\t.reg .b128 c, v, d;\n\t"
+                 "mov.b128 c, {%2, %3};\n\t"
+                 "mov.b128 v, {%4, %5};\n\t"
+                 "atom.global.cas.b128 d, [%6], c, v;\n\t"
+                 "mov.b128 {%0, %1}, d;\n\t}"
+                 : "=l"(old.t), "=l"(old.key)
+                 : "l"(cmp.t), "l"(cmp.key), "l"(val.t), "l"(val.key), "l"(p)
+                 : "memory");
+    return old;
+}
+__device__ __forceinline__ void prefetch_l1(const void* p) { asm volatile("prefetch.global.L1 [%0];" ::"l"(p)); }
+__device__ __forceinline__ void hit_merge(HitRec* p, const HitRec& h, HitRec seen) {
+    while (hit_less(h, seen)) {
+        const HitRec old = hit_cas(p, seen, h);
+        if (old.t == seen.t && old.key == seen.key) return;
+        seen = old;
+    }
+}
+
 struct WaveParams {
     RenderParams base;
     float4* queue[2];
-    unsigned long long* best_t;
-    unsigned long long* best_key;
+    HitRec* best;
     uint2* pairs;
-    uint2* cands;
-    double* cand_t;
-    unsigned* cand_count;
     WaveState* st;
     int capacity;
     unsigned pair_cap;
@@ -390,9 +425,6 @@
     W.status->seq = seq;
 }
 
-constexpr unsigned long long BEST_T_INIT = 0x7ff0000000000000ull;
-constexpr unsigned long long BEST_KEY_MISS = ~0ull;
-constexpr unsigned long long BEST_KEY_OVERFLOW = 0ull;
 constexpr unsigned PAIR_NULL = 0xffffffffu;
 
 __device__ __forceinline__ unsigned warp_claim(unsigned* counter, bool pred, unsigned lane) {
@@ -459,11 +491,8 @@
     *I.work_counter = I.total0;
     atomicAdd(&I.counters[DC_SAMPLES], I.total0);
 }
-__global__ void wf_fill_best(unsigned long long* best_t, unsigned long long* best_key, size_t n) {
-    for (size_t i = blockIdx.x * (size_t)blockDim.x + threadIdx.x; i < n; i += (size_t)gridDim.x * blockDim.x) {
-        best_t[i] = 0x7ff0000000000000ull;
-        best_key[i] = ~0ull;
-    }
+__global__ void wf_fill_best(HitRec* best, size_t n) {
+    for (size_t i = blockIdx.x * (size_t)blockDim.x + threadIdx.x; i < n; i += (size_t)gridDim.x * blockDim.x) hit_store(&best[i], HIT_NONE);
 }
 
 template <int R, int BLOCK>
@@ -475,7 +504,7 @@
     unsigned long long live;
     uint2* pairs;
     unsigned pair_cap;
-    unsigned long long* best_key;
+    HitRec* best;
     WaveState* st;
 
     __device__ __forceinline__ void flush(const uint32_t* list, unsigned long long nz, int count, int kbase) {
@@ -508,7 +537,7 @@
                 pairs[w] = make_uint2(entry(v), (unsigned)(kbase + k));
             } else {
                 if (w < pair_cap) pairs[w] = make_uint2(PAIR_NULL, 0u);
-                if (v < n) best_key[entry(v)] = BEST_KEY_OVERFLOW;
+                if (v < n) hit_store(&best[entry(v)], HIT_OVERFLOW);
             }
             ++w;
         }
@@ -538,7 +567,7 @@
     sink.p0 = p0;
     sink.pairs = W.pairs;
     sink.pair_cap = W.pair_cap;
-    sink.best_key = W.best_key;
+    sink.best = W.best;
     sink.st = W.st;
     unsigned item = sc_.bid * warps + warp;
     const unsigned uniform_end = (n_items + warps - 1) / warps * warps;
@@ -651,10 +680,6 @@
 
 #include "rt_cull_tc.cuh"
 
-__device__ __forceinline__ unsigned wf_cand_region(const WaveParams& W, unsigned total_warps) {
-    return ((W.pair_cap + total_warps * 32u - 1u) / (total_warps * 32u)) * 32u;
-}
-
 template <bool GEN>
 __device__ __forceinline__ void wf_refine_body(const WaveParams& W, const DevScene* scp, Scope sc_, int cur) {
     const RenderParams& P = W.base;
@@ -667,10 +692,6 @@
         atomicAdd(&P.counters[DC_CANDIDATES], (unsigned long long)(npairs - min(npairs, W.st->pad)));
         W.st->pad = 0;
     }
-    const unsigned total_warps = sc_.nblk * (blockDim.x >> 5);
-    const unsigned warp_id = sc_.bid * (blockDim.x >> 5) + (threadIdx.x >> 5);
-    const size_t region = (size_t)warp_id * wf_cand_region(W, total_warps);
-    unsigned cnt = 0;
     const unsigned stride = sc_.nblk * blockDim.x;
     const unsigned i_first = sc_.bid * blockDim.x + threadIdx.x;
     uint2 pr_next = i_first < npairs ? W.pairs[i_first] : make_uint2(PAIR_NULL, 0u);
@@ -678,12 +699,11 @@
         const uint2 pr = pr_next;
         const unsigned i_next = i0 + lane + stride;
         pr_next = i_next < npairs ? W.pairs[i_next] : make_uint2(PAIR_NULL, 0u);
-        bool cand = false;
-        double t = CUDART_INF;
         if (pr.x != PAIR_NULL) {
             const float4* qc = cur ? W.queue[1] : W.queue[0];
             const float4 a = qc[3 * (size_t)pr.x], b = qc[3 * (size_t)pr.x + 1];
-            const unsigned long long seen = __ldcg(&W.best_t[pr.x]);
+            const HitRec seen = hit_load_cg(&W.best[pr.x]);
+            double t;
             if (!GEN) {
                 t = refine_candidate(P.sc.ex_c0r, P.sc.ex_c1, P.sc.ex_t0t1, P.sc.flags, (int)pr.y, a.x, a.y, a.z, b.x, b.y, b.z,
                                      a.w, 0.001, (double)FLT_MAX);
@@ -698,45 +718,16 @@
                 t = refine_leaf<true>(scp, (int)pr.y, a.x, a.y, a.z, b.x, b.y, b.z, a.w, 0.001, (double)FLT_MAX, true, P.key, pixq, smpq, bq);
             }
             const unsigned long long tb = (unsigned long long)__double_as_longlong(t);
-            if (t < CUDART_INF && tb <= seen) {
-                atomicMin(&W.best_t[pr.x], tb);
-                cand = true;
-            }
-        }
-        const unsigned m = __ballot_sync(0xffffffffu, cand);
-        if (cand) {
-            const size_t slot = region + cnt + __popc(m & ((1u << lane) - 1u));
-            W.cands[slot] = pr;
-            W.cand_t[slot] = t;
-        }
-        cnt += __popc(m);
-    }
-    if (lane == 0) W.cand_count[warp_id] = cnt;
+            if (t < CUDART_INF && tb <= seen.t)
+                hit_merge(&W.best[pr.x], HitRec{tb, (((unsigned long long)__ldg(&P.sc.tie_hi[pr.y])) << 32) | pr.y}, seen);
+        }
+    }
 }
 template <bool GEN>
 __global__ void __launch_bounds__(256) wf_refine(const __grid_constant__ WaveParams W) {
     if (W.st->mode != MODE_RUN) return;
     TraceScope trace(W.trace);
     wf_refine_body<GEN>(W, &W.base.sc, grid_scope(), W.cur);
-}
-
-__device__ __forceinline__ void wf_tiebreak_body(const WaveParams& W, Scope sc_) {
-    const RenderParams& P = W.base;
-    const unsigned lane = threadIdx.x & 31u;
-    const unsigned total_warps = sc_.nblk * (blockDim.x >> 5);
-    const unsigned warp_id = sc_.bid * (blockDim.x >> 5) + (threadIdx.x >> 5);
-    const size_t region = (size_t)warp_id * wf_cand_region(W, total_warps);
-    const unsigned cnt = W.cand_count[warp_id];
-    for (unsigned j = lane; j < cnt; j += 32) {
-        const uint2 pr = W.cands[region + j];
-        if ((unsigned long long)__double_as_longlong(W.cand_t[region + j]) == W.best_t[pr.x])
-            atomicMin(&W.best_key[pr.x], (((unsigned long long)__ldg(&P.sc.tie_hi[pr.y])) << 32) | pr.y);
-    }
-}
-__global__ void __launch_bounds__(256) wf_tiebreak(const __grid_constant__ WaveParams W) {
-    if (W.st->mode != MODE_RUN) return;
-    TraceScope trace(W.trace);
-    wf_tiebreak_body(W, grid_scope());
 }
 
 template <bool GEN>
@@ -774,17 +765,23 @@
         float4 a, b, c;
         if (have) {
             a = qc[3 * (size_t)idx]; b = qc[3 * (size_t)idx + 1]; c = qc[3 * (size_t)idx + 2];
-            unsigned long long key = W.best_key[idx];
+            const HitRec h = W.best[idx];
+            if (idx0 + lane + stride < n) {
+                const unsigned e = wf_entry(idx0 + lane + stride, n_g, n_p, (unsigned)W.capacity);
+                prefetch_l1(qc + 3 * (size_t)e);
+                prefetch_l1(qc + 3 * (size_t)e + 2);
+                prefetch_l1(&W.best[e]);
+            }
+            unsigned long long key = h.key;
             const uint32_t slot = __float_as_uint(b.w), sd = __float_as_uint(c.w);
             const uint32_t pix = rng_pixel(P, slot);
             const uint32_t smp = sd >> 8;
             const int depth = (int)(sd & 255u);
             const uint32_t bounce = (uint32_t)(P.max_depth - depth + 1);
             int k = (int)(unsigned)key;
-            double td = __longlong_as_double((long long)W.best_t[idx]);
-            W.best_key[idx] = BEST_KEY_MISS;
-            W.best_t[idx] = BEST_T_INIT;
-            if (key == BEST_KEY_OVERFLOW) {
+            double td = __longlong_as_double((long long)h.t);
+            hit_store(&W.best[idx], HIT_NONE);
+            if (hit_is_overflow(h)) {
                 exact_closest_hit<GEN>(scp, a.x, a.y, a.z, b.x, b.y, b.z, a.w, P.key, pix, smp, bounce, &td, &k);
                 key = k < 0 ? BEST_KEY_MISS : 1ull;
             } else {
@@ -977,10 +974,7 @@
         const BvhHit H = bvh_closest<GEN>(&W.base.sc, a.x, a.y, a.z, b.x, b.y, b.z, a.w, 0.001, (double)FLT_MAX, true, P.key,
                                           rng_pixel(P, __float_as_uint(b.w)), sd >> 8, (uint32_t)(P.max_depth - (int)(sd & 255u) + 1));
         n_leaf += H.n_leaf; n_node += H.n_node;
-        if (H.k >= 0) {
-            W.best_t[idx] = (unsigned long long)__double_as_longlong(H.t);
-            W.best_key[idx] = ((unsigned long long)H.tie << 32) | (unsigned)H.k;
-        }
+        if (H.k >= 0) hit_store(&W.best[idx], HitRec{(unsigned long long)__double_as_longlong(H.t), ((unsigned long long)H.tie << 32) | (unsigned)H.k});
     }
     atomicAdd(&s_ctr[DC_CANDIDATES], n_leaf);
     atomicAdd(&s_ctr[DC_BVH_NODES], n_node);
@@ -1147,18 +1141,12 @@
             s_st.mode = MODE_RUN;
             s_st.pad = 0;
         }
-        const unsigned warps = BLOCK / 32;
         WaveParams L = W;
         L.queue[0] = W.queue[0] + 3 * (size_t)first;
         L.queue[1] = W.queue[1] + 3 * (size_t)first;
-        L.best_t = W.best_t + first;
-        L.best_key = W.best_key + first;
+        L.best = W.best + first;
         L.pairs = W.pairs + (size_t)first * kPairsPerEntry;
         L.pair_cap = min(K, (unsigned)W.capacity - first) * kPairsPerEntry;
-        const size_t cand_slice = (size_t)wf_cand_region(L, warps) * warps;
-        L.cands = W.cands + (size_t)blockIdx.x * cand_slice;
-        L.cand_t = W.cand_t + (size_t)blockIdx.x * cand_slice;
-        L.cand_count = W.cand_count + blockIdx.x * warps;
         L.st = &s_st;
         L.status = nullptr;
         L.capacity = (int)K;
@@ -1192,15 +1180,10 @@
 #ifdef RT_TAIL_DIAG
             unsigned long long dt2 = global_timer_ns();
 #endif
-            wf_tiebreak_body(L, solo);
-            __syncthreads();
-#ifdef RT_TAIL_DIAG
-            unsigned long long dt3 = global_timer_ns();
-#endif
             wf_shade_body<GEN>(L, &W.base.sc, solo, cur, s_ctr);
 #ifdef RT_TAIL_DIAG
             __syncthreads();
-            if (diag) printf("tail cta %u n %u pairs %u: cull %llu refine %llu tie %llu shade %llu ns\n", blockIdx.x, n, np_, dt1 - dt0, dt2 - dt1, dt3 - dt2, global_timer_ns() - dt3);
+            if (diag) printf("tail cta %u n %u pairs %u: cull %llu refine %llu shade %llu ns\n", blockIdx.x, n, np_, dt1 - dt0, dt2 - dt1, global_timer_ns() - dt2);
 #endif
             cur ^= 1;
         }
```

New measurement: 1.635 billion (median of 6 runs). 1.02x the previous value.
